# tencent-ailab/pika

Hardware: NVIDIA H100
Metric: utterances/sec RNN-T train step (T=1000,U=150,V=6k) (higher is better)
Workload: dtype bf16

## Files before the change

### include/pika_b200.h

```cpp
#ifndef PIKA_B200_H
#define PIKA_B200_H
#include <stdint.h>

#ifdef __cplusplus
extern "C" {
#endif

#define PK_F32 0
#define PK_BF16 1

const char* pk_last_error(void);
int pk_version(void);
long long pk_launch_count(void);

#define PK_GEMM_MAX_PAIRS 9
#define PK_SEL_ZERO 0
#define PK_SEL_ZB0 1
#define PK_SEL_ZB1 2
#define PK_SEL_KZ 3
#define PK_ACT_NONE 0
#define PK_ACT_RELU 1
#define PK_AUX_NONE 0
#define PK_AUX_ADD 1
#define PK_AUX_MASK_NZ 2

typedef struct {
    const void* ptr;
    int64_t dim[4];
    int64_t stride[3];
} pk_view4;

typedef struct {
    int n_pairs;
    pk_view4 a[PK_GEMM_MAX_PAIRS];
    pk_view4 b[PK_GEMM_MAX_PAIRS];
    int a_row_off[PK_GEMM_MAX_PAIRS];
    int b_row_off[PK_GEMM_MAX_PAIRS];
    int a_mn_major, b_mn_major;
    int a_sel2, a_sel3, b_sel2, b_sel3;
    int kz_count;
    pk_view4 c;
    int c_dtype;
    int c_accumulate;
    float alpha;
    const float* bias;
    int act;
    float drop_p;
    uint32_t drop_seed;
    int aux_mode;
    const void* aux;
    int aux_dtype;
    int64_t aux_stride[3];
    float aux_scale;
    int block_n;
    int k_splits;
    float* row_lse;
} pk_gemm_desc;

int pk_gemm_bf16(const pk_gemm_desc* desc, void* stream);
int pk_gemm_row_lse_parts(long long M, long long N, int block_n);

long long pk_rnnt_loss_workspace_bytes(int B, int T, int U1);
long long pk_rnnt_loss_colsum_workspace_bytes(int B, int T, int U1, int ldv);
int pk_rnnt_loss_fwd_bwd(const void* logits, int dtype, const int* labels, const int* frame_lens,
                         const int* label_lens, int B, int T, int U1, int V, int ldv, int ld_labels,
                         const float* grad_scale, float* costs, void* dlogits, float* dlogits_colsum, void* workspace,
                         long long workspace_bytes, void* stream);
int pk_rnnt_loss_fwd_bwd_lse(const void* logits, int dtype, const int* labels, const int* frame_lens,
                             const int* label_lens, int B, int T, int U1, int V, int ldv, int ld_labels,
                             const float* grad_scale, float* costs, void* dlogits, float* dlogits_colsum, void* workspace,
                             long long workspace_bytes, const float* row_lse, int n_parts, void* stream);

int pk_cast_split(const void* src, int src_dtype, long long ld_src, void* hi, void* lo, long long ld_dst,
                  long long rows, int cols, int cols_pad, float scale, void* stream);
int pk_attention_lse_stride(int T);
long long pk_attention_keep_bits_bytes(int B, int T, int heads);
int pk_attention_fwd(const void* q, const void* k, const void* v, long long ld_qkv, void* out, long long ld_out, float* lse,
                     int B, int T, int heads, int dh, float alpha, float drop_p, uint32_t seed, void* stream);
int pk_attention_bwd(const void* q, const void* k, const void* v, long long ld_qkv, const void* out, long long ld_out,
                     const void* dout, long long ld_dout, const float* lse, float* dsum_ws, void* dq, void* dk, void* dv,
                     long long ld_dqkv, int B, int T, int heads, int dh, float alpha, float drop_p, uint32_t seed, void* stream);
int pk_attention_fwd_bits(const void* q, const void* k, const void* v, long long ld_qkv, void* out, long long ld_out, float* lse,
                          int B, int T, int heads, int dh, float alpha, float drop_p, uint32_t seed, uint32_t* keep_bits, void* stream);
int pk_attention_bwd_bits(const void* q, const void* k, const void* v, long long ld_qkv, const void* out, long long ld_out,
                          const void* dout, long long ld_dout, const float* lse, float* dsum_ws, void* dq, void* dk, void* dv,
                          long long ld_dqkv, int B, int T, int heads, int dh, float alpha, float drop_p, const uint32_t* keep_bits,
                          void* stream);
long long pk_colstats_ws_floats(int C);
int pk_bn_fwd(const void* x, void* y, int dtype, long long rows, int C, const float* w, const float* b, float eps,
              int train, float momentum, float* run_mean, float* run_var, float* mean, float* rstd, float* stats_ws,
              void* stream);
int pk_bn_bwd(const void* dy, const void* x, void* dx, int dtype, long long rows, int C, const float* w,
              const float* mean, const float* rstd, int train, int relu_mask, float* dw, float* db, float* ws ,
              void* stream);
int pk_colsum(const void* x, int dtype, long long rows, int C, float* out, float* ws, void* stream);
int pk_layernorm_fwd(const void* x, void* y, int dtype, long long rows, int C, const float* w, const float* b, float eps,
                     float* mean, float* rstd, void* stream);
int pk_layernorm_bwd(const void* dy, const void* x, void* dx, int dtype, long long rows, int C, const float* w,
                     const float* mean, const float* rstd, float* dw, float* db, void* stream);
int pk_softmax_fwd(const float* S, long long ld_s, void* P, void* Pd, int dtype, long long ld_p, long long rows, int n,
                   float drop_p, uint32_t seed, void* stream);
int pk_softmax_masked_fwd(const float* S, long long ld_s, void* P, void* Pd, int dtype, long long ld_p, long long rows, int n,
                          int q_len, int heads, int causal, const uint8_t* key_pad, float drop_p, uint32_t seed, void* stream);
int pk_softmax_bwd(const float* dPd, long long ld_d, const void* P, long long ld_p, void* dS, int dtype, long long rows,
                   int n, float drop_p, uint32_t seed, void* stream);
#define PK_RELPOS_MAX 1024
int pk_softmax_masked_relpos_fwd(const float* S, long long ld_s, const float* QR, long long ld_r, void* P, void* Pd, int dtype,
                                 long long ld_p, long long rows, int n, int q_len, int heads, int causal, const uint8_t* key_pad,
                                 int max_rel, float* Pb, float drop_p, uint32_t seed, void* stream);
int pk_softmax_relpos_bwd(const float* dPd, long long ld_d, const float* G, long long ld_r, const void* P, long long ld_p, void* dS,
                          int dtype, long long rows, int n, int q_len, int heads, int max_rel, float* dSb, float drop_p,
                          uint32_t seed, void* stream);
int pk_dropout(const void* x, void* y, int dtype, long long n, float p, uint32_t seed, void* stream);
int pk_mask_nz(const void* dy, const void* y, void* dx, int dtype, long long n, float scale, void* stream);
int pk_add(const void* a, const void* b, void* o, int dtype, long long n, void* stream);
int pk_log_softmax(const void* x, int dtype, long long ld, float* y, long long rows, int n, float scale, void* stream);
int pk_joint_gate_fwd(const void* ex, const void* py, void* h, int dtype, int B, int T, int U1, int H, int ld_h, void* stream);
int pk_joint_gate_bwd(const void* ex, const void* py, const void* dh, void* dex, void* dpy, int dtype, int B, int T, int U1,
                      int H, void* stream);
int pk_lstm_cell_fwd(const float* gx, long long ld_gx, const float* gh, long long ld_gh, const float* c_prev, float* c_out,
                     void* h_out, int dtype, long long ld_h, float* gates_save, int B, int H, void* stream);
int pk_lstm_cell_bwd(const void* dh_out, long long ld_dho, const float* dh_rec, const float* dc_next, const float* gates,
                     const float* c, const float* c_prev, void* dgates, int dtype, float* dc_prev, int B, int H, void* stream);
int pk_embedding_fwd(const long long* idx, const float* table, int E, void* out, int dtype, int ld_out, long long n, void* stream);
int pk_embedding_bwd(const long long* idx, const void* dout, int dtype, int ld, int E, float* dtable, long long n,
                     long long padding_idx, void* stream);

int pk_absmax(const float* x, long long n, float* out, int* nan_flag, void* stream);
int pk_sgd_nesterov_clip(float* p, const float* g, float* buf, long long n, float lr, float momentum, float max_norm,
                         const float* absmax, const int* nan_flag, int first, void* stream);
int pk_bmuf_delta(const float* glob, const float* local, float* delta, long long n, void* stream);
int pk_bmuf_update(float* glob, float* local, float* delta_prev, const float* delta_sum, long long n, int world,
                   float block_momentum, float block_lr, void* stream);
int pk_adam_clip(float* p, const float* g, float* exp_avg, float* exp_avg_sq, float* p_out2, long long n, double lr,
                 double beta1, double beta2, double eps, double bias_correction1, double bias_correction2_sqrt,
                 float max_norm, const float* absmax, const int* nan_flag, void* stream);
int pk_bmuf_adam_update(float* glob, float* local, float* delta_prev, float* exp_avg_g, float* exp_avg_sq_g, float* msg,
                        long long n, int world, double block_momentum, double block_lr, double beta1_tau, double beta1_rho,
                        double beta2_tau, double beta2_rho, void* stream);

long long pk_frontend_workspace_bytes(int B, int n_max, int t_max, int n_mel, int D);
int pk_frontend_fwd(const short* pcm, long long ld_pcm, const int* n_samples, const float* rate, const int* new_len,
                    const float* target_db, const int* n_frames, int B, int n_max, int t_max, int n_mel, int lctx,
                    int rctx, const float* window, const float* twiddle, const float* mel_w, const int* mel_lo,
                    const int* mel_hi, float preemph, int cmn, const float* offset, const float* scale, int f0, int fs,
                    int t0, int ts, void* out, int out_dtype, short* wave_i16_out, void* workspace,
                    long long workspace_bytes, int* err_flag, float dither, unsigned int dither_seed, void* stream);
int pk_fbank(const float* wave, long long ld_wave, const int* n_frames, int B, int t_max, int n_mel, const float* window,
             const float* twiddle, const float* mel_w, const int* mel_lo, const int* mel_hi, float preemph, float* feats,
             float dither, unsigned int dither_seed, void* stream);

long long pk_frontend_noise_rir_workspace_bytes(int B, int n_max, int t_max, int n_mel, int D, int rir_max_len);
int pk_frontend_fwd_noise_rir(const short* pcm, long long ld_pcm, const int* n_samples, const float* rate, const int* new_len,
                              const float* target_db, const int* n_frames, int B, int n_max, int t_max, int n_mel, int lctx,
                              int rctx, const float* window, const float* twiddle, const float* mel_w, const int* mel_lo,
                              const int* mel_hi, float preemph, int cmn, const float* offset, const float* scale, int f0, int fs,
                              int t0, int ts, void* out, int out_dtype, short* wave_i16_out, void* workspace,
                              long long workspace_bytes, int* err_flag, float dither, unsigned int dither_seed, void* stream,
                              const short* noise, const int* noise_idx, const long long* noise_off, const double* snr,
                              const double* noise_rms_db, const short* rir, const long long* rir_off, const int* rir_len,
                              const int* rir_idx, int rir_max_len);

long long pk_conv_same_f64_workspace_bytes(int B, int n_max, int m_max);
int pk_conv_same_f64(const double* x, long long ld_x, const int* n_len, const double* h, long long ld_h, const int* m_len, int B,
                     int n_max, int m_max, double* y, long long ld_y, void* workspace, long long workspace_bytes, void* stream);

int pk_beam_prepare(const int* next_ys, const int* step_ctx, int* t_idx, const void* enc, int dtype, int Tenc, int H, void* enc_hid,
                    const float* embed, int E, void* x_emb, int ld_x, int K, int blk, int rows, void* stream);
int pk_beam_lstm_cell(const float* gates, const int* next_ys, const int* step_ctx, int blk, void* h, int dtype, float* c, int rows, int H,
                      void* stream);
int pk_beam_step_end(int* step_ctx, const int* not_done, int max_steps, void* stream);
int pk_beam_gate(const float* a, void* h, int dtype, int rows, int H, void* stream);
int pk_row_lse(const void* x, int dtype, long long ld, float* lse, long long rows, int n, float scale, void* stream);
int pk_beam_advance(const float* logits, int ldv, const float* row_lse, float sm_scale, const int* t_idx, const int* num_frames, const int* max_len, float* scores,
                    int* next_ys, int* prev_ks, int* hyp_tok, int* hyp_len, float* fin_score, int* fin_step, int* fin_k,
                    int* fin_count, int* eos_top, int* done, int* not_done_total, int B, int K, int V, int L, int cap,
                    const int* step_ctx, int blk, int n_best, int beam_prune, void* stream);
int pk_beam_reorder(const int* prev_ks, const int* step_ctx, const void* h_in, const float* c_in, const int* t_in, void* h_out, float* c_out,
                    int* t_out, int dtype, int K, int H, int layers, int rows, void* stream);
typedef struct {
    const int* arc_off;
    const int* arc_ilabel;
    const double* arc_weight;
    const int* arc_next;
    const double* finals;
    int backoff_id, n_disambig;
    int disambig_ids[4];
} pk_lm_fst;
int pk_beam_advance_lm(const float* logits, int ldv, const float* row_lse, float sm_scale, const int* t_idx, const int* num_frames, const int* max_len, float* scores,
                       int* next_ys, int* prev_ks, int* hyp_tok, int* hyp_len, float* fin_score, int* fin_step, int* fin_k,
                       int* fin_count, int* eos_top, int* done, int* not_done_total, int B, int K, int V, int L, int cap,
                       const int* step_ctx, int blk, int n_best, int beam_prune, const pk_lm_fst* fst, double lm_scale, double nonblk_reward,
                       int* set_state, double* set_cost, int* set_n, float* lm_scores, int max_states, int* err_flag, void* stream);

typedef struct {
    const int* next_ys;
    const int* step_ctx;
    const int* hyp_tok;
    const int* hyp_len;
    int* slot;
    void* pool;
    long long n_entries;
    int blk, rows, S1, layers, D, dtype, init;
} pk_beam_xf_state;
int pk_beam_xf_taps(const pk_beam_xf_state* st, int layer, const float* embed, int E, const void* x_cur, void* taps, int ldc, void* stream);
int pk_beam_xf_attn(const pk_beam_xf_state* st, int layer, const void* qkv, int heads, const float* rel, int max_rel, void* out, void* stream);
int pk_beam_xf_select(const pk_beam_xf_state* st, const void* x, void* h, int H, void* stream);
int pk_beam_xf_slots(const pk_beam_xf_state* st, const int* prev_ks, int K, void* stream);

long long pk_lstm_seq_workspace_bytes(int H);
int pk_lstm_seq_fwd_ex(const float* gx, const void* w_hh_bf16, void* out, int out_dtype, int ldo, float* gates_save, float* cs,
                       const int* lens, int B, int U, int H, int n_dir, int reverse, void* ws, void* stream);
int pk_lstm_seq_bwd_ex(const void* dout, int dtype, int ldo, const float* gates_save, const float* cs, const void* w_hh_bf16,
                       void* dG_bf16, const int* lens, int B, int U, int H, int n_dir, int reverse, void* ws, void* stream);

int pk_gather_rows(const void* src, const int* idx, void* dst, int dtype, long long rows, int C, void* stream);
int pk_scatter_add_rows(const void* src, const int* idx, float* dst, int dtype, long long rows, int C, void* stream);
int pk_ce_grad(const void* z, int dtype, long long ld, const int* tok, const float* coef, float scale, void* dz,
               long long rows, int n, void* stream);

#ifdef __cplusplus
}
#endif
#endif
```

### pika_b200/_lib.py

```python
import ctypes
import os
import re

_HERE = os.path.dirname(os.path.abspath(__file__))
LIB_PATH = os.path.join(_HERE, "libpika_b200.so")
HEADER_PATH = os.path.join(os.path.dirname(_HERE), "include", "pika_b200.h")


class PikaError(RuntimeError):
    pass


def _read_header(path):
    with open(path) as f:
        src = re.sub(r"/\*.*?\*/", " ", f.read(), flags=re.S)
    defines = {k: int(v) for k, v in re.findall(r"^\s*#define\s+(\w+)\s+(-?\d+)\s*$", src, flags=re.M)}
    src = re.sub(r"^\s*#.*$", " ", src, flags=re.M)
    src = re.sub(r"typedef\s+struct\s*\{.*?\}\s*\w+\s*;", " ", src, flags=re.S)
    src = re.sub(r'extern\s+"C"\s*\{|\}', " ", src)
    protos = []
    for decl in filter(None, (" ".join(d.split()) for d in src.split(";"))):
        m = re.fullmatch(r"(.+?)\s*\b(pk_\w+)\s*\((.*)\)", decl)
        if m is None:
            raise ImportError("pika_b200: %s: cannot read the declaration %r" % (path, decl))
        params = m.group(3).strip()
        protos.append((m.group(1), m.group(2), [] if params in ("", "void") else [p.strip() for p in params.split(",")]))
    return defines, protos


_DEFINES, _PROTOTYPES = _read_header(HEADER_PATH)
PK_F32, PK_BF16 = _DEFINES["PK_F32"], _DEFINES["PK_BF16"]
SEL_ZERO, SEL_ZB0, SEL_ZB1, SEL_KZ = (_DEFINES["PK_SEL_" + s] for s in ("ZERO", "ZB0", "ZB1", "KZ"))
ACT_NONE, ACT_RELU = _DEFINES["PK_ACT_NONE"], _DEFINES["PK_ACT_RELU"]
AUX_NONE, AUX_ADD, AUX_MASK_NZ = _DEFINES["PK_AUX_NONE"], _DEFINES["PK_AUX_ADD"], _DEFINES["PK_AUX_MASK_NZ"]
MAX_PAIRS = _DEFINES["PK_GEMM_MAX_PAIRS"]


class View4(ctypes.Structure):
    _fields_ = [("ptr", ctypes.c_void_p), ("dim", ctypes.c_int64 * 4), ("stride", ctypes.c_int64 * 3)]


class GemmDesc(ctypes.Structure):
    _fields_ = [
        ("n_pairs", ctypes.c_int),
        ("a", View4 * MAX_PAIRS),
        ("b", View4 * MAX_PAIRS),
        ("a_row_off", ctypes.c_int * MAX_PAIRS),
        ("b_row_off", ctypes.c_int * MAX_PAIRS),
        ("a_mn_major", ctypes.c_int), ("b_mn_major", ctypes.c_int),
        ("a_sel2", ctypes.c_int), ("a_sel3", ctypes.c_int), ("b_sel2", ctypes.c_int), ("b_sel3", ctypes.c_int),
        ("kz_count", ctypes.c_int),
        ("c", View4),
        ("c_dtype", ctypes.c_int),
        ("c_accumulate", ctypes.c_int),
        ("alpha", ctypes.c_float),
        ("bias", ctypes.c_void_p),
        ("act", ctypes.c_int),
        ("drop_p", ctypes.c_float),
        ("drop_seed", ctypes.c_uint32),
        ("aux_mode", ctypes.c_int),
        ("aux", ctypes.c_void_p),
        ("aux_dtype", ctypes.c_int),
        ("aux_stride", ctypes.c_int64 * 3),
        ("aux_scale", ctypes.c_float),
        ("block_n", ctypes.c_int),
        ("k_splits", ctypes.c_int),
        ("row_lse", ctypes.c_void_p),
    ]


class LmFst(ctypes.Structure):
    _fields_ = [("arc_off", ctypes.c_void_p), ("arc_ilabel", ctypes.c_void_p), ("arc_weight", ctypes.c_void_p),
                ("arc_next", ctypes.c_void_p), ("finals", ctypes.c_void_p), ("backoff_id", ctypes.c_int),
                ("n_disambig", ctypes.c_int), ("disambig_ids", ctypes.c_int * 4)]


class BeamXfState(ctypes.Structure):
    _fields_ = [("next_ys", ctypes.c_void_p), ("step_ctx", ctypes.c_void_p), ("hyp_tok", ctypes.c_void_p), ("hyp_len", ctypes.c_void_p),
                ("slot", ctypes.c_void_p), ("pool", ctypes.c_void_p), ("n_entries", ctypes.c_longlong), ("blk", ctypes.c_int),
                ("rows", ctypes.c_int), ("S1", ctypes.c_int), ("layers", ctypes.c_int), ("D", ctypes.c_int), ("dtype", ctypes.c_int),
                ("init", ctypes.c_int)]


STRUCTS = {"pk_view4": View4, "pk_gemm_desc": GemmDesc, "pk_lm_fst": LmFst, "pk_beam_xf_state": BeamXfState}
_SCALARS = {"int": ctypes.c_int, "long long": ctypes.c_longlong, "float": ctypes.c_float, "double": ctypes.c_double,
            "uint32_t": ctypes.c_uint32, "unsigned int": ctypes.c_uint32}
_RESULTS = {"int": ctypes.c_int, "long long": ctypes.c_longlong, "const char*": ctypes.c_char_p}


def _param_type(decl, fn):
    words = re.findall(r"\w+|\*", decl)[:-1]
    if "*" in words:
        base = " ".join(w for w in words if w not in ("const", "*"))
        if base in STRUCTS:
            return ctypes.POINTER(STRUCTS[base])
        if not base.startswith("pk_"):
            return ctypes.c_void_p
    elif " ".join(words) in _SCALARS:
        return _SCALARS[" ".join(words)]
    raise ImportError("pika_b200: %s: no ctypes type for the parameter %r of %s" % (HEADER_PATH, decl, fn))


class _CDLL(ctypes.CDLL):
    _func_flags_ = 0


def _bind(lib):
    for ret, name, params in _PROTOTYPES:
        if not hasattr(lib, name):
            raise ImportError("pika_b200: %s declares %s, which %s does not export" % (HEADER_PATH, name, LIB_PATH))
        ret = re.sub(r"\s*\*", "*", ret)
        if ret not in _RESULTS:
            raise ImportError("pika_b200: %s: no ctypes type for the return type %r of %s" % (HEADER_PATH, ret, name))
        fn = getattr(lib, name)
        fn.restype = _RESULTS[ret]
        fn.argtypes = [_param_type(p, name) for p in params]
    return lib


if not os.path.exists(LIB_PATH):
    raise ImportError(
        "pika_b200: %s is missing -- build it with `python -c 'import __graft_entry__ as g; g.build()'` "
        "(there is no CPU fallback)" % LIB_PATH)

lib = _bind(_CDLL(LIB_PATH))


def check(rc, what=""):
    if rc != 0:
        raise PikaError("%s failed (rc=%d): %s" % (what, rc, lib.pk_last_error().decode()))


def launch_count():
    return int(lib.pk_launch_count())
```

### pika_b200/csrc/elementwise.cu

```cuda
#include "../../include/pika_b200.h"
#include "common.cuh"

namespace pk {
void count_launch();

template <typename T> struct V8 {};
template <> struct V8<__nv_bfloat16> {
    struct Raw { uint4 q; };
    PK_DEVICE static Raw load_raw(const __nv_bfloat16* p) { return Raw{*reinterpret_cast<const uint4*>(p)}; }
    PK_DEVICE static void unpack(const Raw& r, float (&f)[8]) {
        f[0] = bf16lo(r.q.x); f[1] = bf16hi(r.q.x); f[2] = bf16lo(r.q.y); f[3] = bf16hi(r.q.y);
        f[4] = bf16lo(r.q.z); f[5] = bf16hi(r.q.z); f[6] = bf16lo(r.q.w); f[7] = bf16hi(r.q.w);
    }
    PK_DEVICE static void load(const __nv_bfloat16* p, float (&f)[8]) {
        const uint4 q = *reinterpret_cast<const uint4*>(p);
        f[0] = bf16lo(q.x); f[1] = bf16hi(q.x); f[2] = bf16lo(q.y); f[3] = bf16hi(q.y);
        f[4] = bf16lo(q.z); f[5] = bf16hi(q.z); f[6] = bf16lo(q.w); f[7] = bf16hi(q.w);
    }
    PK_DEVICE static void store(__nv_bfloat16* p, const float (&f)[8]) {
        *reinterpret_cast<uint4*>(p) =
            make_uint4(pack_bf16x2(f[0], f[1]), pack_bf16x2(f[2], f[3]), pack_bf16x2(f[4], f[5]), pack_bf16x2(f[6], f[7]));
    }
};
template <> struct V8<float> {
// ... 647 lines not shown
        V8<T>::load(x + i * 8, f);
#pragma unroll
        for (int e = 0; e < 8; ++e) f[e] = drop_keep((uint64_t)(i * 8 + e), seed, thresh) ? f[e] * scale : 0.f;
        V8<T>::store(y + i * 8, f);
    }
    for (long long i = nv * 8 + (long long)blockIdx.x * blockDim.x + threadIdx.x; i < n; i += (long long)gridDim.x * blockDim.x) {
        const float v = to_f32<T>(x[i]);
        y[i] = from_f32<T>(drop_keep((uint64_t)i, seed, thresh) ? v * scale : 0.f);
    }
}
template <typename T>
__global__ void __launch_bounds__(256) mask_nz_kernel(const T* __restrict__ dy, const T* __restrict__ y, T* __restrict__ dx, long long n, float scale) {
    const long long nv = n / 8;
    constexpr int UR = 2;
    for (long long i0 = ((long long)blockIdx.x * blockDim.x + threadIdx.x) * UR; i0 < nv; i0 += (long long)gridDim.x * blockDim.x * UR) {
        float g[UR][8], f[UR][8];
#pragma unroll
        for (int k = 0; k < UR; ++k)
            if (i0 + k < nv) { V8<T>::load(dy + (i0 + k) * 8, g[k]); V8<T>::load(y + (i0 + k) * 8, f[k]); }
#pragma unroll
        for (int k = 0; k < UR; ++k)
            if (i0 + k < nv) {
#pragma unroll
                for (int e = 0; e < 8; ++e) g[k][e] = f[k][e] != 0.f ? g[k][e] * scale : 0.f;
                V8<T>::store(dx + (i0 + k) * 8, g[k]);
            }
    }
    for (long long i = nv * 8 + (long long)blockIdx.x * blockDim.x + threadIdx.x; i < n; i += (long long)gridDim.x * blockDim.x)
        dx[i] = from_f32<T>(to_f32<T>(y[i]) != 0.f ? to_f32<T>(dy[i]) * scale : 0.f);
}
template <typename T>
__global__ void __launch_bounds__(256) add_kernel(const T* __restrict__ a, const T* __restrict__ b, T* __restrict__ o, long long n) {
    const long long nv = n / 8;
    for (long long i = (long long)blockIdx.x * blockDim.x + threadIdx.x; i < nv; i += (long long)gridDim.x * blockDim.x) {
        float f[8], g[8];
        V8<T>::load(a + i * 8, f);
        V8<T>::load(b + i * 8, g);
#pragma unroll
        for (int e = 0; e < 8; ++e) f[e] += g[e];
        V8<T>::store(o + i * 8, f);
    }
    for (long long i = nv * 8 + (long long)blockIdx.x * blockDim.x + threadIdx.x; i < n; i += (long long)gridDim.x * blockDim.x)
        o[i] = from_f32<T>(to_f32<T>(a[i]) + to_f32<T>(b[i]));
}
template <typename T>
__global__ void __launch_bounds__(256) log_softmax_kernel(const T* __restrict__ x, long long ld, float* __restrict__ y, long long rows,
                                                          int n, float scale, float* __restrict__ lse = nullptr) {
    const int lane = threadIdx.x & 31;
    const long long warp = (long long)blockIdx.x * (blockDim.x >> 5) + (threadIdx.x >> 5);
    const long long nw = (long long)gridDim.x * (blockDim.x >> 5);
    for (long long r = warp; r < rows; r += nw) {
        const T* xr = x + r * ld;
        float m = -INFINITY;
        for (int c = lane; c < n; c += 32) m = fmaxf(m, to_f32<T>(xr[c]) * scale);
        m = warp_max(m);
        float s = 0.f;
        for (int c = lane; c < n; c += 32) s += expf(to_f32<T>(xr[c]) * scale - m);
        const float l = m + logf(warp_sum(s));
        if (y) for (int c = lane; c < n; c += 32) y[r * n + c] = to_f32<T>(xr[c]) * scale - l;
        if (lse && lane == 0) lse[r] = l;
    }
}

PK_DEVICE float sigmoidf_(float x) { return 1.f / (1.f + __expf(-x)); }
template <typename T> PK_DEVICE float jt_tanh(float x);
template <> PK_DEVICE float jt_tanh<float>(float x) { return tanhf(x); }
template <> PK_DEVICE float jt_tanh<__nv_bfloat16>(float x) {
    float y;
    asm("tanh.approx.f32 %0, %1;" : "=f"(y) : "f"(x));
    return y;
}
template <typename T> PK_DEVICE float jt_sigmoid(float x);
template <> PK_DEVICE float jt_sigmoid<float>(float x) { return 1.f / (1.f + expf(-x)); }
template <> PK_DEVICE float jt_sigmoid<__nv_bfloat16>(float x) { return fmaf(jt_tanh<__nv_bfloat16>(0.5f * x), 0.5f, 0.5f); }

template <typename T>
__global__ void __launch_bounds__(128) joint_gate_fwd_kernel(const T* __restrict__ ex, const T* __restrict__ py, T* __restrict__ h,
                                                             int B, int Tt, int U1, int H, int ld_h) {
    const int bt = blockIdx.x;
    const int b = bt / Tt;
    for (int c0 = threadIdx.x * 8; c0 < H; c0 += blockDim.x * 8) {
        float e1[8], eg[8];
        V8<T>::load(ex + (long long)bt * 2 * H + c0, e1);
        V8<T>::load(ex + (long long)bt * 2 * H + H + c0, eg);
        for (int u = 0; u < U1; ++u) {
            float p1[8], pg[8], o[8];
            const T* pr = py + ((long long)b * U1 + u) * 2 * H;
            V8<T>::load(pr + c0, p1);
            V8<T>::load(pr + H + c0, pg);
#pragma unroll
            for (int e = 0; e < 8; ++e) o[e] = jt_tanh<T>(e1[e] + p1[e]) * jt_sigmoid<T>(eg[e] + pg[e]);
            V8<T>::store(h + ((long long)bt * U1 + u) * ld_h + c0, o);
        }
    }
    if (ld_h > H) {
        for (int u = threadIdx.x; u < U1; u += blockDim.x) {
            const float one[8] = {1.f, 0.f, 0.f, 0.f, 0.f, 0.f, 0.f, 0.f};
            V8<T>::store(h + ((long long)bt * U1 + u) * ld_h + H, one);
        }
    }
}
template <typename T, int UI>
__global__ void __launch_bounds__(128) joint_gate_fwd_sliced_kernel(const T* __restrict__ ex, const T* __restrict__ py, T* __restrict__ h,
                                                                    int B, int Tt, int U1, int H, int ld_h) {
    extern __shared__ __align__(16) uint8_t jg_smem[];
    T* s_py = reinterpret_cast<T*>(jg_smem);
    const int slices = H / 32;
    const int b = blockIdx.x / slices, cs = blockIdx.x - b * slices;
    const int tid = threadIdx.x, warp = tid >> 5, lane = tid & 31;
    const int ct = lane & 3, ul = (lane >> 2) + 8 * warp;
    const int c0 = cs * 32 + ct * 8;
    for (int i = tid; i < U1 * 8; i += 128) {
        const int u = i >> 3, v = i & 7;
        float f[8];
        V8<T>::load(py + ((long long)b * U1 + u) * 2 * H + (v >> 2) * H + cs * 32 + (v & 3) * 8, f);
        V8<T>::store(s_py + ((long long)(v * U1) + u) * 8, f);
    }
    __syncthreads();
    const T* s_p1 = s_py + (long long)(ct * U1) * 8;
    const T* s_pg = s_py + (long long)((4 + ct) * U1) * 8;
    const T* ex_b = ex + (long long)b * Tt * 2 * H + c0;
    typename V8<T>::Raw e1n = V8<T>::load_raw(ex_b), egn = V8<T>::load_raw(ex_b + H);
    for (int t = 0; t < Tt; ++t) {
        float e1[8], eg[8];
        V8<T>::unpack(e1n, e1);
        V8<T>::unpack(egn, eg);
        if (t + 1 < Tt) {
            e1n = V8<T>::load_raw(ex_b + (long long)(t + 1) * 2 * H);
            egn = V8<T>::load_raw(ex_b + (long long)(t + 1) * 2 * H + H);
        }
        T* hrow = h + ((long long)(b * Tt + t) * U1) * ld_h + c0;
#pragma unroll
        for (int i = 0; i < UI; ++i) {
            const int u = ul + 32 * i;
            if (u < U1) {
                float p1[8], pg[8], o[8];
                V8<T>::load(s_p1 + u * 8, p1);
                V8<T>::load(s_pg + u * 8, pg);
#pragma unroll
                for (int e = 0; e < 8; ++e) o[e] = jt_tanh<T>(e1[e] + p1[e]) * jt_sigmoid<T>(eg[e] + pg[e]);
                V8<T>::store(hrow + (long long)u * ld_h, o);
            }
        }
        if (ld_h > H && cs == 0 && ct == 0) {
            const float one[8] = {1.f, 0.f, 0.f, 0.f, 0.f, 0.f, 0.f, 0.f};
#pragma unroll
            for (int i = 0; i < UI; ++i) {
                const int u = ul + 32 * i;
                if (u < U1) V8<T>::store(h + ((long long)(b * Tt + t) * U1 + u) * ld_h + H, one);
            }
        }
    }
}
template <typename T>
__global__ void __launch_bounds__(128) joint_gate_bwd_ex_kernel(const T* __restrict__ ex, const T* __restrict__ py,
                                                                const T* __restrict__ dh, T* __restrict__ dex, int B, int Tt,
                                                                int U1, int H) {
    const int bt = blockIdx.x;
    const int b = bt / Tt;
    for (int c0 = threadIdx.x * 8; c0 < H; c0 += blockDim.x * 8) {
        float e1[8], eg[8], a1[8] = {0, 0, 0, 0, 0, 0, 0, 0}, ag[8] = {0, 0, 0, 0, 0, 0, 0, 0};
        V8<T>::load(ex + (long long)bt * 2 * H + c0, e1);
        V8<T>::load(ex + (long long)bt * 2 * H + H + c0, eg);
        for (int u = 0; u < U1; ++u) {
            float p1[8], pg[8], d[8];
            const T* pr = py + ((long long)b * U1 + u) * 2 * H;
            V8<T>::load(pr + c0, p1);
            V8<T>::load(pr + H + c0, pg);
            V8<T>::load(dh + ((long long)bt * U1 + u) * H + c0, d);
#pragma unroll
            for (int e = 0; e < 8; ++e) {
                const float a = jt_tanh<T>(e1[e] + p1[e]), g = jt_sigmoid<T>(eg[e] + pg[e]);
                a1[e] += d[e] * g * (1.f - a * a);
                ag[e] += d[e] * a * g * (1.f - g);
            }
        }
        V8<T>::store(dex + (long long)bt * 2 * H + c0, a1);
        V8<T>::store(dex + (long long)bt * 2 * H + H + c0, ag);
    }
}
template <typename T>
__global__ void __launch_bounds__(128) joint_gate_bwd_py_kernel(const T* __restrict__ ex, const T* __restrict__ py,
                                                                const T* __restrict__ dh, T* __restrict__ dpy, int B, int Tt,
                                                                int U1, int H) {
    const int bu = blockIdx.x;
    const int b = bu / U1, u = bu - b * U1;
    for (int c0 = threadIdx.x * 8; c0 < H; c0 += blockDim.x * 8) {
        float p1[8], pg[8], a1[8] = {0, 0, 0, 0, 0, 0, 0, 0}, ag[8] = {0, 0, 0, 0, 0, 0, 0, 0};
        V8<T>::load(py + (long long)bu * 2 * H + c0, p1);
        V8<T>::load(py + (long long)bu * 2 * H + H + c0, pg);
        for (int t = 0; t < Tt; ++t) {
            float e1[8], eg[8], d[8];
            const long long bt = (long long)b * Tt + t;
            V8<T>::load(ex + bt * 2 * H + c0, e1);
            V8<T>::load(ex + bt * 2 * H + H + c0, eg);
            V8<T>::load(dh + (bt * U1 + u) * H + c0, d);
#pragma unroll
            for (int e = 0; e < 8; ++e) {
                const float a = jt_tanh<T>(e1[e] + p1[e]), g = jt_sigmoid<T>(eg[e] + pg[e]);
                a1[e] += d[e] * g * (1.f - a * a);
                ag[e] += d[e] * a * g * (1.f - g);
            }
        }
        V8<T>::store(dpy + (long long)bu * 2 * H + c0, a1);
        V8<T>::store(dpy + (long long)bu * 2 * H + H + c0, ag);
    }
}

template <typename T, int UI>
__global__ void __launch_bounds__(128) joint_gate_bwd_fused_kernel(const T* __restrict__ ex, const T* __restrict__ py, const T* __restrict__ dh,
                                                                   T* __restrict__ dex, T* __restrict__ dpy, int B, int Tt, int U1, int H) {
    extern __shared__ __align__(16) uint8_t jg_smem[];
    T* s_py = reinterpret_cast<T*>(jg_smem);
    const int slices = H / 32;
    const int b = blockIdx.x / slices, cs = blockIdx.x - b * slices;
    const int tid = threadIdx.x, ct = tid >> 5, lane = tid & 31;
    const int c0 = cs * 32 + ct * 8;
    for (int i = tid; i < U1 * 8; i += 128) {
        const int u = i >> 3, v = i & 7;
        float f[8];
        V8<T>::load(py + ((long long)b * U1 + u) * 2 * H + (v >> 2) * H + cs * 32 + (v & 3) * 8, f);
        V8<T>::store(s_py + ((long long)(v * U1) + u) * 8, f);
    }
    float a1u[UI][8], agu[UI][8];
#pragma unroll
    for (int i = 0; i < UI; ++i)
#pragma unroll
        for (int e = 0; e < 8; ++e) { a1u[i][e] = 0.f; agu[i][e] = 0.f; }
    __syncthreads();
    const T* s_p1 = s_py + (long long)(ct * U1) * 8;
    const T* s_pg = s_py + (long long)((4 + ct) * U1) * 8;
    const T* dh_b = dh + (long long)b * Tt * U1 * H + c0;
    const T* ex_b = ex + (long long)b * Tt * 2 * H + c0;
    typename V8<T>::Raw dn[UI], e1n, egn;
#pragma unroll
    for (int i = 0; i < UI; ++i) {
        const int u = lane + 32 * i;
        if (u < U1) dn[i] = V8<T>::load_raw(dh_b + (long long)u * H);
    }
    e1n = V8<T>::load_raw(ex_b);
    egn = V8<T>::load_raw(ex_b + H);
    for (int t = 0; t < Tt; ++t) {
        float e1[8], eg[8];
        typename V8<T>::Raw dc[UI];
        V8<T>::unpack(e1n, e1);
        V8<T>::unpack(egn, eg);
#pragma unroll
        for (int i = 0; i < UI; ++i) dc[i] = dn[i];
        if (t + 1 < Tt) {
#pragma unroll
            for (int i = 0; i < UI; ++i) {
                const int u = lane + 32 * i;
                if (u < U1) dn[i] = V8<T>::load_raw(dh_b + ((long long)(t + 1) * U1 + u) * H);
            }
            e1n = V8<T>::load_raw(ex_b + (long long)(t + 1) * 2 * H);
            egn = V8<T>::load_raw(ex_b + (long long)(t + 1) * 2 * H + H);
        }
        float v[16];
#pragma unroll
        for (int e = 0; e < 16; ++e) v[e] = 0.f;
#pragma unroll
        for (int i = 0; i < UI; ++i) {
            const int u = lane + 32 * i;
            if (u < U1) {
                float p1[8], pg[8], d[8];
                V8<T>::unpack(dc[i], d);
                V8<T>::load(s_p1 + u * 8, p1);
                V8<T>::load(s_pg + u * 8, pg);
#pragma unroll
                for (int e = 0; e < 8; ++e) {
                    const float a = jt_tanh<T>(e1[e] + p1[e]), g = jt_sigmoid<T>(eg[e] + pg[e]);
                    const float dg = d[e] * g;
                    const float t1 = dg * (1.f - a * a), tg = dg * a * (1.f - g);
                    a1u[i][e] += t1; agu[i][e] += tg;
                    v[e] += t1; v[8 + e] += tg;
                }
            }
        }
        float w8[8], w4[4], w2[2];
        const bool h16 = lane & 16, h8 = lane & 8, h4 = lane & 4, h2 = lane & 2;
#pragma unroll
        for (int i = 0; i < 8; ++i) {
            const float keep = h16 ? v[i + 8] : v[i], send = h16 ? v[i] : v[i + 8];
            w8[i] = keep + __shfl_xor_sync(0xffffffffu, send, 16);
        }
#pragma unroll
        for (int i = 0; i < 4; ++i) {
            const float keep = h8 ? w8[i + 4] : w8[i], send = h8 ? w8[i] : w8[i + 4];
            w4[i] = keep + __shfl_xor_sync(0xffffffffu, send, 8);
        }
#pragma unroll
        for (int i = 0; i < 2; ++i) {
            const float keep = h4 ? w4[i + 2] : w4[i], send = h4 ? w4[i] : w4[i + 2];
            w2[i] = keep + __shfl_xor_sync(0xffffffffu, send, 4);
        }
        float w1 = (h2 ? w2[1] : w2[0]) + __shfl_xor_sync(0xffffffffu, h2 ? w2[0] : w2[1], 2);
        w1 += __shfl_xor_sync(0xffffffffu, w1, 1);
        if ((lane & 1) == 0) {
            const int j = lane >> 1;
            dex[((long long)b * Tt + t) * 2 * H + (j >> 3) * H + c0 + (j & 7)] = from_f32<T>(w1);
        }
    }
#pragma unroll
    for (int i = 0; i < UI; ++i) {
        const int u = lane + 32 * i;
        if (u < U1) {
            V8<T>::store(dpy + ((long long)b * U1 + u) * 2 * H + c0, a1u[i]);
            V8<T>::store(dpy + ((long long)b * U1 + u) * 2 * H + H + c0, agu[i]);
        }
    }
}

template <typename T>
__global__ void lstm_cell_fwd_kernel(const float* __restrict__ gx, long long ld_gx, const float* __restrict__ gh, long long ld_gh,
                                     const float* __restrict__ c_prev, float* __restrict__ c_out, T* __restrict__ h_out,
                                     long long ld_h, float* __restrict__ gates_save, int B, int H) {
    const int i = blockIdx.x * blockDim.x + threadIdx.x;
    if (i >= B * H) return;
    const int b = i / H, j = i - b * H;
    const float* a = gx + (long long)b * ld_gx;
    float gi = a[j], gf = a[H + j], gg = a[2 * H + j], go = a[3 * H + j];
    if (gh) {
        const float* r = gh + (long long)b * ld_gh;
        gi += r[j]; gf += r[H + j]; gg += r[2 * H + j]; go += r[3 * H + j];
    }
    gi = sigmoidf_(gi); gf = sigmoidf_(gf); gg = tanhf(gg); go = sigmoidf_(go);
    const float cp = c_prev ? c_prev[i] : 0.f;
    const float c = gf * cp + gi * gg;
    c_out[i] = c;
    h_out[(long long)b * ld_h + j] = from_f32<T>(go * tanhf(c));
    if (gates_save) {
        float* g = gates_save + (long long)b * 4 * H;
        g[j] = gi; g[H + j] = gf; g[2 * H + j] = gg; g[3 * H + j] = go;
    }
}
template <typename T>
__global__ void lstm_cell_bwd_kernel(const T* __restrict__ dh_out, long long ld_dho, const float* __restrict__ dh_rec,
                                     const float* __restrict__ dc_next, const float* __restrict__ gates, const float* __restrict__ c,
                                     const float* __restrict__ c_prev, T* __restrict__ dgates, float* __restrict__ dc_prev, int B,
                                     int H) {
    const int i = blockIdx.x * blockDim.x + threadIdx.x;
    if (i >= B * H) return;
    const int b = i / H, j = i - b * H;
    const float* g = gates + (long long)b * 4 * H;
    const float gi = g[j], gf = g[H + j], gg = g[2 * H + j], go = g[3 * H + j];
    float dh = dh_out ? to_f32<T>(dh_out[(long long)b * ld_dho + j]) : 0.f;
    if (dh_rec) dh += dh_rec[i];
    const float tc = tanhf(c[i]);
    float dc = dh * go * (1.f - tc * tc);
    if (dc_next) dc += dc_next[i];
    const float cp = c_prev ? c_prev[i] : 0.f;
    T* d = dgates + (long long)b * 4 * H;
    d[j] = from_f32<T>(dc * gg * gi * (1.f - gi));
    d[H + j] = from_f32<T>(dc * cp * gf * (1.f - gf));
    d[2 * H + j] = from_f32<T>(dc * gi * (1.f - gg * gg));
    d[3 * H + j] = from_f32<T>(dh * tc * go * (1.f - go));
    dc_prev[i] = dc * gf;
}

template <typename T>
__global__ void embedding_fwd_kernel(const long long* __restrict__ idx, const float* __restrict__ table, int E, T* __restrict__ out,
                                     int ld_out, long long n) {
    for (long long i = (long long)blockIdx.x * blockDim.x + threadIdx.x; i < n * ld_out; i += (long long)gridDim.x * blockDim.x) {
        const long long r = i / ld_out;
        const int c = (int)(i - r * ld_out);
        out[i] = from_f32<T>(c < E ? table[idx[r] * E + c] : 0.f);
    }
}
template <typename T>
__global__ void embedding_bwd_kernel(const long long* __restrict__ idx, const T* __restrict__ dout, int ld, int E,
                                     float* __restrict__ dtable, long long n, long long padding_idx) {
    for (long long i = (long long)blockIdx.x * blockDim.x + threadIdx.x; i < n * E; i += (long long)gridDim.x * blockDim.x) {
        const long long r = i / E;
        const int c = (int)(i - r * E);
        if (idx[r] != padding_idx) atomicAdd(&dtable[idx[r] * E + c], to_f32<T>(dout[r * ld + c]));
    }
}


template <typename T>
__global__ void gather_rows_kernel(const T* __restrict__ src, const int* __restrict__ idx, T* __restrict__ dst, long long rows, int C) {
    const long long r = blockIdx.x;
    if (r >= rows) return;
    const T* s = src + (long long)idx[r] * C;
    for (int c = threadIdx.x * 8; c < C; c += blockDim.x * 8) {
        float f[8];
        V8<T>::load(s + c, f);
        V8<T>::store(dst + r * C + c, f);
    }
}
template <typename T>
__global__ void scatter_add_rows_kernel(const T* __restrict__ src, const int* __restrict__ idx, float* __restrict__ dst, long long rows, int C) {
    const long long r = blockIdx.x;
    if (r >= rows) return;
    float* d = dst + (long long)idx[r] * C;
    for (int c = threadIdx.x; c < C; c += blockDim.x) atomicAdd(&d[c], to_f32<T>(src[r * C + c]));
}
template <typename T>
__global__ void __launch_bounds__(256) ce_grad_kernel(const T* __restrict__ z, long long ld, const int* __restrict__ tok,
                                                      const float* __restrict__ coef, float scale, T* __restrict__ dz, long long rows, int n) {
    const int lane = threadIdx.x & 31;
    const long long warp = (long long)blockIdx.x * (blockDim.x >> 5) + (threadIdx.x >> 5);
    const long long nw = (long long)gridDim.x * (blockDim.x >> 5);
    for (long long r = warp; r < rows; r += nw) {
        const T* zr = z + r * ld;
        T* dr = dz + r * ld;
// ... 86 lines not shown
                         const float* mean, const float* rstd, int train, int relu_mask, float* dw, float* db, float* ws,
                         void* stream) {
    PK_CHECK_ARG(C % 8 == 0 && rows > 0, "C must be a multiple of 8 and rows > 0");
    PK_CHECK_ARG(aligned16(dy) && aligned16(x) && aligned16(dx) && aligned16(ws), "pk_bn_bwd: dy, x, dx, ws must be 16-byte aligned");
    cudaStream_t st = STREAM(stream);
    PK_DISPATCH_T(dtype, { int rc = run_colstats<T, 1>((const T*)dy, (const T*)x, rows, C, mean, rstd, ws, db, dw, st); if (rc) return rc; });
    PK_DISPATCH_T(dtype, (bn_bwd_apply_kernel<T><<<col_grid(rows, C), 128, 0, st>>>((const T*)dy, (const T*)x, (T*)dx, rows, C, mean, rstd, w,
                                                                       train ? db : nullptr, train ? dw : nullptr, relu_mask)));
    DONE();
}

extern "C" int pk_colsum(const void* x, int dtype, long long rows, int C, float* out, float* ws, void* stream) {
    PK_CHECK_ARG(C % 8 == 0 && rows > 0, "C must be a multiple of 8 and rows > 0");
    PK_CHECK_ARG(aligned16(x) && aligned16(ws), "pk_colsum: x, ws must be 16-byte aligned");
    cudaStream_t st = STREAM(stream);
    PK_DISPATCH_T(dtype, { int rc = run_colstats<T, 0>((const T*)x, nullptr, rows, C, nullptr, nullptr, ws, out, nullptr, st); if (rc) return rc; });
    return 0;
}

extern "C" int pk_layernorm_fwd(const void* x, void* y, int dtype, long long rows, int C, const float* w, const float* b, float eps,
                                float* mean, float* rstd, void* stream) {
    PK_CHECK_ARG(C % 8 == 0 && rows > 0 && C <= 1024, "C must be a multiple of 8, <= 1024, and rows > 0");
    PK_CHECK_ARG(aligned16(x) && aligned16(y), "pk_layernorm_fwd: x, y must be 16-byte aligned");
    const int grid = grid_for(rows, 8);
    PK_DISPATCH_T(dtype, (ln_fwd_kernel<T><<<grid, 256, 0, STREAM(stream)>>>((const T*)x, (T*)y, rows, C, w, b, eps, mean, rstd)));
    DONE();
}
extern "C" int pk_layernorm_bwd(const void* dy, const void* x, void* dx, int dtype, long long rows, int C, const float* w,
                                const float* mean, const float* rstd, float* dw, float* db, void* stream) {
    PK_CHECK_ARG(C % 8 == 0 && rows > 0 && C <= 1024, "C must be a multiple of 8, <= 1024, and rows > 0");
    PK_CHECK_ARG(aligned16(dy) && aligned16(x) && aligned16(dx), "pk_layernorm_bwd: dy, x, dx must be 16-byte aligned");
    cudaStream_t st = STREAM(stream);
    PK_CHECK_CUDA(cudaMemsetAsync(dw, 0, sizeof(float) * C, st));
    PK_CHECK_CUDA(cudaMemsetAsync(db, 0, sizeof(float) * C, st));
    const int grid = grid_for(rows, 8, 2);
    PK_DISPATCH_T(dtype, (ln_bwd_kernel<T><<<grid, 256, 2 * C * sizeof(float), st>>>((const T*)dy, (const T*)x, (T*)dx, rows, C, w, mean,
                                                                                     rstd, dw, db)));
    DONE();
}

extern "C" int pk_softmax_fwd(const float* S, long long ld_s, void* P, void* Pd, int dtype, long long ld_p, long long rows, int n,
                              float drop_p, uint32_t seed, void* stream) {
    PK_CHECK_ARG(rows > 0 && n > 0 && ld_p >= n && ld_s >= ld_p && ld_p <= 2048 && ld_p % 8 == 0 && ld_s % 8 == 0, "softmax rows: ld % 8 == 0, <= 2048 wide");
    const int grid = grid_for(rows, 8);
    const uint32_t th = drop_thresh16_of(drop_p);
    const float sc = drop_scale16_of(th);
    if (ld_p <= 1024) { PK_DISPATCH_T(dtype, (softmax_fwd_kernel<T, 4><<<grid, 256, 0, STREAM(stream)>>>(S, ld_s, (T*)P, (T*)Pd, ld_p, rows, n, th, sc, seed))); }
    else { PK_DISPATCH_T(dtype, (softmax_fwd_kernel<T, 8><<<grid, 256, 0, STREAM(stream)>>>(S, ld_s, (T*)P, (T*)Pd, ld_p, rows, n, th, sc, seed))); }
    DONE();
}
extern "C" int pk_softmax_masked_fwd(const float* S, long long ld_s, void* P, void* Pd, int dtype, long long ld_p, long long rows, int n,
                                     int q_len, int heads, int causal, const uint8_t* key_pad, float drop_p, uint32_t seed, void* stream) {
    PK_CHECK_ARG(rows > 0 && n > 0 && ld_p >= n && ld_s >= ld_p && ld_p <= 2048 && ld_p % 8 == 0 && ld_s % 8 == 0, "softmax rows: ld % 8 == 0, <= 2048 wide");
    PK_CHECK_ARG(q_len > 0 && heads > 0 && rows % ((long long)heads * q_len) == 0, "masked softmax: rows = sequences * heads * q_len");
    PK_CHECK_ARG(causal || key_pad, "masked softmax without a mask: use pk_softmax_fwd");
    const int grid = grid_for(rows, 8);
    const uint32_t th = drop_thresh16_of(drop_p);
    const float sc = drop_scale16_of(th);
    if (ld_p <= 1024) { PK_DISPATCH_T(dtype, (softmax_fwd_kernel<T, 4><<<grid, 256, 0, STREAM(stream)>>>(S, ld_s, (T*)P, (T*)Pd, ld_p, rows, n, th, sc, seed, q_len, heads, causal, key_pad))); }
    else { PK_DISPATCH_T(dtype, (softmax_fwd_kernel<T, 8><<<grid, 256, 0, STREAM(stream)>>>(S, ld_s, (T*)P, (T*)Pd, ld_p, rows, n, th, sc, seed, q_len, heads, causal, key_pad))); }
    DONE();
}
extern "C" int pk_softmax_bwd(const float* dPd, long long ld_d, const void* P, long long ld_p, void* dS, int dtype, long long rows,
                              int n, float drop_p, uint32_t seed, void* stream) {
    PK_CHECK_ARG(rows > 0 && n > 0 && ld_p >= n && ld_d >= ld_p && ld_p <= 2048 && ld_p % 8 == 0 && ld_d % 8 == 0, "softmax rows: ld % 8 == 0, <= 2048 wide");
    const int grid = grid_for(rows, 8);
    const uint32_t th = drop_thresh16_of(drop_p);
    const float sc = drop_scale16_of(th);
    if (ld_p <= 1024) { PK_DISPATCH_T(dtype, (softmax_bwd_kernel<T, 4><<<grid, 256, 0, STREAM(stream)>>>(dPd, ld_d, (const T*)P, ld_p, (T*)dS, rows, n, th, sc, seed))); }
    else { PK_DISPATCH_T(dtype, (softmax_bwd_kernel<T, 8><<<grid, 256, 0, STREAM(stream)>>>(dPd, ld_d, (const T*)P, ld_p, (T*)dS, rows, n, th, sc, seed))); }
    DONE();
}
#define PK_RELPOS_CHECKS(ld_x, ld_p)                                                                                                  \
    PK_CHECK_ARG(rows > 0 && n > 0 && ld_p >= n && ld_x >= ld_p && ld_p <= 2048 && ld_p % 8 == 0 && ld_x % 8 == 0,                     \
                 "relative-position softmax rows: n <= ld_p <= 2048, pitches multiples of 8");                                         \
    PK_CHECK_ARG(q_len == n && heads > 0 && rows % ((long long)heads * q_len) == 0,                                                     \
                 "relative-position softmax: self-attention rows = sequences * heads * n");                                             \
    PK_CHECK_ARG(max_rel >= 1 && max_rel <= PK_RELPOS_MAX && ld_r >= 2 * max_rel + 1 && ld_r % 8 == 0,                               \
                 "relative positions: 1 <= max_rel <= 1024, ld_r >= 2*max_rel + 1 and a multiple of 8")
extern "C" int pk_softmax_masked_relpos_fwd(const float* S, long long ld_s, const float* QR, long long ld_r, void* P, void* Pd, int dtype,
                                            long long ld_p, long long rows, int n, int q_len, int heads, int causal, const uint8_t* key_pad,
                                            int max_rel, float* Pb, float drop_p, uint32_t seed, void* stream) {
    PK_RELPOS_CHECKS(ld_s, ld_p);
    const int grid = grid_for(rows, 8);
    const uint32_t th = drop_thresh16_of(drop_p);
    const float sc = drop_scale16_of(th);
    if (ld_p <= 1024) { PK_DISPATCH_T(dtype, (softmax_relpos_fwd_kernel<T, 4><<<grid, 256, 0, STREAM(stream)>>>(S, ld_s, QR, ld_r, (T*)P, (T*)Pd, ld_p, rows, n, th, sc, seed, q_len, heads, causal, key_pad, max_rel, Pb))); }
    else { PK_DISPATCH_T(dtype, (softmax_relpos_fwd_kernel<T, 8><<<grid, 256, 0, STREAM(stream)>>>(S, ld_s, QR, ld_r, (T*)P, (T*)Pd, ld_p, rows, n, th, sc, seed, q_len, heads, causal, key_pad, max_rel, Pb))); }
    DONE();
}
extern "C" int pk_softmax_relpos_bwd(const float* dPd, long long ld_d, const float* G, long long ld_r, const void* P, long long ld_p, void* dS,
                                     int dtype, long long rows, int n, int q_len, int heads, int max_rel, float* dSb, float drop_p,
                                     uint32_t seed, void* stream) {
    PK_RELPOS_CHECKS(ld_d, ld_p);
    const int grid = grid_for(rows, 8);
    const uint32_t th = drop_thresh16_of(drop_p);
    const float sc = drop_scale16_of(th);
    if (ld_p <= 1024) { PK_DISPATCH_T(dtype, (softmax_relpos_bwd_kernel<T, 4><<<grid, 256, 0, STREAM(stream)>>>(dPd, ld_d, G, ld_r, (const T*)P, ld_p, (T*)dS, rows, n, th, sc, seed, q_len, heads, max_rel, dSb))); }
    else { PK_DISPATCH_T(dtype, (softmax_relpos_bwd_kernel<T, 8><<<grid, 256, 0, STREAM(stream)>>>(dPd, ld_d, G, ld_r, (const T*)P, ld_p, (T*)dS, rows, n, th, sc, seed, q_len, heads, max_rel, dSb))); }
    DONE();
}
#undef PK_RELPOS_CHECKS

extern "C" int pk_dropout(const void* x, void* y, int dtype, long long n, float p, uint32_t seed, void* stream) {
    const int grid = grid_for(n, 256 * 8);
    const uint32_t th = drop_thresh_of(p);
    PK_CHECK_ARG(th != 0, "p must be > 0");
    PK_CHECK_ARG((reinterpret_cast<uintptr_t>(x) & 15) == 0 && (reinterpret_cast<uintptr_t>(y) & 15) == 0, "pk_dropout: pointers must be 16-byte aligned");
    PK_DISPATCH_T(dtype, (dropout_kernel<T><<<grid, 256, 0, STREAM(stream)>>>((const T*)x, (T*)y, n, th, 1.f / (1.f - p), seed)));
    DONE();
}
extern "C" int pk_mask_nz(const void* dy, const void* y, void* dx, int dtype, long long n, float scale, void* stream) {
    const int grid = grid_for(n, 256 * 16);
    PK_CHECK_ARG(((reinterpret_cast<uintptr_t>(dy) | reinterpret_cast<uintptr_t>(y) | reinterpret_cast<uintptr_t>(dx)) & 15) == 0, "pk_mask_nz: pointers must be 16-byte aligned");
    PK_DISPATCH_T(dtype, (mask_nz_kernel<T><<<grid, 256, 0, STREAM(stream)>>>((const T*)dy, (const T*)y, (T*)dx, n, scale)));
    DONE();
}
extern "C" int pk_add(const void* a, const void* b, void* o, int dtype, long long n, void* stream) {
    const int grid = grid_for(n, 256 * 8);
    PK_CHECK_ARG(((reinterpret_cast<uintptr_t>(a) | reinterpret_cast<uintptr_t>(b) | reinterpret_cast<uintptr_t>(o)) & 15) == 0, "pk_add: pointers must be 16-byte aligned");
    PK_DISPATCH_T(dtype, (add_kernel<T><<<grid, 256, 0, STREAM(stream)>>>((const T*)a, (const T*)b, (T*)o, n)));
    DONE();
}
extern "C" int pk_log_softmax(const void* x, int dtype, long long ld, float* y, long long rows, int n, float scale, void* stream) {
    const int grid = grid_for(rows, 8);
    PK_DISPATCH_T(dtype, (log_softmax_kernel<T><<<grid, 256, 0, STREAM(stream)>>>((const T*)x, ld, y, rows, n, scale)));
    DONE();
}
extern "C" int pk_row_lse(const void* x, int dtype, long long ld, float* lse, long long rows, int n, float scale, void* stream) {
    const int grid = grid_for(rows, 8);
    PK_DISPATCH_T(dtype, (log_softmax_kernel<T><<<grid, 256, 0, STREAM(stream)>>>((const T*)x, ld, nullptr, rows, n, scale, lse)));
    DONE();
}

template <typename T, int UI>
static void launch_gate_fwd_sliced(const void* ex, const void* py, void* h, int B, int T_, int U1, int H, int ld_h, cudaStream_t st) {
    joint_gate_fwd_sliced_kernel<T, UI><<<B * (H / 32), 128, U1 * 64 * (int)sizeof(T), st>>>((const T*)ex, (const T*)py, (T*)h, B, T_, U1, H, ld_h);
}
extern "C" int pk_joint_gate_fwd(const void* ex, const void* py, void* h, int dtype, int B, int T_, int U1, int H, int ld_h, void* stream) {
    PK_CHECK_ARG(H % 8 == 0 && ld_h % 8 == 0 && ld_h >= H, "H, ld_h must be multiples of 8");
    const int ui = (U1 + 31) / 32;
    if (H % 32 == 0 && ui <= 5 && T_ >= 8) {
        cudaStream_t st = STREAM(stream);
#define PK_GATE_CASE(N) case N: { PK_DISPATCH_T(dtype, (launch_gate_fwd_sliced<T, N>(ex, py, h, B, T_, U1, H, ld_h, st))); } break;
        switch (ui) { PK_GATE_CASE(1) PK_GATE_CASE(2) PK_GATE_CASE(3) PK_GATE_CASE(4) PK_GATE_CASE(5) }
#undef PK_GATE_CASE
        DONE();
    }
    PK_DISPATCH_T(dtype, (joint_gate_fwd_kernel<T><<<B * T_, 128, 0, STREAM(stream)>>>((const T*)ex, (const T*)py, (T*)h, B, T_, U1, H, ld_h)));
    DONE();
}

template <typename T, int UI>
static void launch_gate_bwd_fused(const void* ex, const void* py, const void* dh, void* dex, void* dpy, int B, int T_, int U1, int H, cudaStream_t st) {
    const int smem = U1 * 64 * (int)sizeof(T);
    joint_gate_bwd_fused_kernel<T, UI><<<B * (H / 32), 128, smem, st>>>((const T*)ex, (const T*)py, (const T*)dh, (T*)dex, (T*)dpy, B, T_, U1, H);
}
extern "C" int pk_joint_gate_bwd(const void* ex, const void* py, const void* dh, void* dex, void* dpy, int dtype, int B, int T_, int U1,
                                 int H, void* stream) {
    PK_CHECK_ARG(H % 8 == 0, "H must be a multiple of 8");
    const int ui = (U1 + 31) / 32;
    if (H % 32 == 0 && ui <= 5) {
        cudaStream_t st = STREAM(stream);
#define PK_GATE_CASE(N) case N: { PK_DISPATCH_T(dtype, (launch_gate_bwd_fused<T, N>(ex, py, dh, dex, dpy, B, T_, U1, H, st))); } break;
        switch (ui) { PK_GATE_CASE(1) PK_GATE_CASE(2) PK_GATE_CASE(3) PK_GATE_CASE(4) PK_GATE_CASE(5) }
#undef PK_GATE_CASE
        DONE();
    }
    PK_DISPATCH_T(dtype, (joint_gate_bwd_ex_kernel<T><<<B * T_, 128, 0, STREAM(stream)>>>((const T*)ex, (const T*)py, (const T*)dh, (T*)dex, B, T_, U1, H)));
    PK_CHECK_LAUNCH(); count_launch();
    PK_DISPATCH_T(dtype, (joint_gate_bwd_py_kernel<T><<<B * U1, 128, 0, STREAM(stream)>>>((const T*)ex, (const T*)py, (const T*)dh, (T*)dpy, B, T_, U1, H)));
    DONE();
}

extern "C" int pk_lstm_cell_fwd(const float* gx, long long ld_gx, const float* gh, long long ld_gh, const float* c_prev, float* c_out,
                                void* h_out, int dtype, long long ld_h, float* gates_save, int B, int H, void* stream) {
    PK_DISPATCH_T(dtype, (lstm_cell_fwd_kernel<T><<<(B * H + 255) / 256, 256, 0, STREAM(stream)>>>(gx, ld_gx, gh, ld_gh, c_prev, c_out,
                                                                                                (T*)h_out, ld_h, gates_save, B, H)));
    DONE();
}
extern "C" int pk_lstm_cell_bwd(const void* dh_out, long long ld_dho, const float* dh_rec, const float* dc_next, const float* gates,
                                const float* c, const float* c_prev, void* dgates, int dtype, float* dc_prev, int B, int H,
                                void* stream) {
    PK_DISPATCH_T(dtype, (lstm_cell_bwd_kernel<T><<<(B * H + 255) / 256, 256, 0, STREAM(stream)>>>((const T*)dh_out, ld_dho, dh_rec, dc_next,
                                                                                                gates, c, c_prev, (T*)dgates, dc_prev, B, H)));
    DONE();
}

extern "C" int pk_embedding_fwd(const long long* idx, const float* table, int E, void* out, int dtype, int ld_out, long long n,
                                void* stream) {
    const int grid = grid_for(n * ld_out, 256);
    PK_DISPATCH_T(dtype, (embedding_fwd_kernel<T><<<grid, 256, 0, STREAM(stream)>>>(idx, table, E, (T*)out, ld_out, n)));
    DONE();
}
extern "C" int pk_embedding_bwd(const long long* idx, const void* dout, int dtype, int ld, int E, float* dtable, long long n,
                                long long padding_idx, void* stream) {
    const int grid = grid_for(n * E, 256);
    PK_DISPATCH_T(dtype, (embedding_bwd_kernel<T><<<grid, 256, 0, STREAM(stream)>>>(idx, (const T*)dout, ld, E, dtable, n, padding_idx)));
    DONE();
}

extern "C" int pk_gather_rows(const void* src, const int* idx, void* dst, int dtype, long long rows, int C, void* stream) {
    PK_CHECK_ARG(C % 8 == 0 && rows > 0, "C must be a multiple of 8 and rows > 0");
    PK_CHECK_ARG(aligned16(src) && aligned16(dst), "pk_gather_rows: src, dst must be 16-byte aligned");
    PK_DISPATCH_T(dtype, (gather_rows_kernel<T><<<(unsigned)rows, 128, 0, STREAM(stream)>>>((const T*)src, idx, (T*)dst, rows, C)));
    DONE();
}
extern "C" int pk_scatter_add_rows(const void* src, const int* idx, float* dst, int dtype, long long rows, int C, void* stream) {
    PK_CHECK_ARG(rows > 0, "rows must be > 0");
    PK_DISPATCH_T(dtype, (scatter_add_rows_kernel<T><<<(unsigned)rows, 256, 0, STREAM(stream)>>>((const T*)src, idx, dst, rows, C)));
    DONE();
}
extern "C" int pk_ce_grad(const void* z, int dtype, long long ld, const int* tok, const float* coef, float scale, void* dz,
                          long long rows, int n, void* stream) {
    PK_CHECK_ARG(rows > 0 && n > 0 && ld >= n, "bad shape");
    const int grid = grid_for(rows, 8);
    PK_DISPATCH_T(dtype, (ce_grad_kernel<T><<<grid, 256, 0, STREAM(stream)>>>((const T*)z, ld, tok, coef, scale, (T*)dz, rows, n)));
    DONE();
}
```

### pika_b200/csrc/gemm.cu

```cuda
#include <cstdarg>
#include <cstdio>
#include <cstring>

#include "../../include/pika_b200.h"
#include "common.cuh"

namespace pk {

constexpr int BM = 128;
constexpr int BK = 64;
constexpr int A_STAGE_BYTES = BM * BK * 2;
constexpr int C_STAGE_BYTES = 64 * 128;
constexpr int CONSUMERS = 2;

struct GemmParams {
    CUtensorMap a[PK_GEMM_MAX_PAIRS];
    CUtensorMap b[PK_GEMM_MAX_PAIRS];
    CUtensorMap c;
    int a_off[PK_GEMM_MAX_PAIRS];
    int b_off[PK_GEMM_MAX_PAIRS];
    int n_pairs, kz_count, num_k_blocks;
    int k_splits, iters_per_split;
    int M, N, tiles_m, tiles_n, zb0, zb1;
    int a_sel2, a_sel3, b_sel2, b_sel3;
    int c_is_f32, c_accumulate;
    float alpha;
    const float* bias;
    int act;
    uint32_t drop_thresh;
    float drop_scale;
    uint32_t drop_seed;
    int aux_mode, aux_is_f32;
    const void* aux;
    long long aux_sm, aux_s0, aux_s1;
    float aux_scale;
    float* row_lse;
    uint64_t pol_a, pol_b, pol_c;
};

template <int BN, bool EPI_WARPS> struct GemmCfg {
    static constexpr int B_STAGE_BYTES = BN * BK * 2;
    static constexpr int STAGE_BYTES = A_STAGE_BYTES + B_STAGE_BYTES;
    static constexpr int STAGES = BN == 256 ? (EPI_WARPS ? 3 : 4) : (BN == 128 ? 6 : 8);
    static constexpr int C_OFF = STAGES * STAGE_BYTES;
    static constexpr int C_BYTES = EPI_WARPS ? BM * BN * 2 : CONSUMERS * 2 * C_STAGE_BYTES;
    static constexpr int BIAS_OFF = C_OFF + C_BYTES;
    static constexpr int BAR_OFF = BIAS_OFF + (EPI_WARPS ? BN * 4 : 0);
    static constexpr int SMEM_BYTES = BAR_OFF + 256 + 1024;
    static constexpr int THREADS = 128 + CONSUMERS * 128;
    static_assert(SMEM_BYTES <= 232448, "shared memory budget");
};

PK_DEVICE int pick_sel(int sel, int zb0, int zb1, int kz) {
    return sel == PK_SEL_ZB0 ? zb0 : (sel == PK_SEL_ZB1 ? zb1 : (sel == PK_SEL_KZ ? kz : 0));
}

struct UnitCoord { int mb, nb, zb0, zb1, split; };
PK_DEVICE UnitCoord decode_unit(const GemmParams& p, int unit) {
    UnitCoord u;
    const int tiles_per_z = p.tiles_m * p.tiles_n;
    const int out_tiles = tiles_per_z * p.zb0 * p.zb1;
    u.split = unit / out_tiles;
    const int tile = unit - u.split * out_tiles;
    const int z = tile / tiles_per_z;
    const int r = tile - z * tiles_per_z;
    u.mb = r / p.tiles_n; u.nb = r - u.mb * p.tiles_n;
    u.zb1 = z / p.zb0; u.zb0 = z - u.zb1 * p.zb0;
    return u;
}

template <int BN, bool A_MN, bool B_MN> PK_DEVICE void wgmma_tile(float (&acc)[BN / 2], uint64_t a, uint64_t b, uint32_t accumulate) {
    if constexpr (BN == 64) wgmma_ss_n64<A_MN, B_MN>(acc, a, b, accumulate);
    else if constexpr (BN == 128) wgmma_ss_n128<A_MN, B_MN>(acc, a, b, accumulate);
    else wgmma_ss_n256<A_MN, B_MN>(acc, a, b, accumulate);
}

enum { EPI_PLAIN = 0, EPI_LSE = 1, EPI_FULL = 2 };
template <bool CF32, int EPI> constexpr bool epi_warps() { return !CF32 && EPI != EPI_FULL; }

template <bool A_MN, bool B_MN, int BN, bool CF32, int EPI>
__global__ void __launch_bounds__(GemmCfg<BN, epi_warps<CF32, EPI>()>::THREADS, 1) gemm_wgmma_kernel(const __grid_constant__ GemmParams p) {
    constexpr bool EW = epi_warps<CF32, EPI>();
    static_assert(EPI != EPI_LSE || (EW && BN == 256), "the row log-sum-exp epilogue works on bf16 256-wide tiles");
    using Cfg = GemmCfg<BN, EW>;
    extern __shared__ uint8_t smem_raw[];
    uint8_t* smem = reinterpret_cast<uint8_t*>((reinterpret_cast<uintptr_t>(smem_raw) + 1023) & ~uintptr_t(1023));
    uint64_t* full_bar = reinterpret_cast<uint64_t*>(smem + Cfg::BAR_OFF);
    uint64_t* empty_bar = full_bar + Cfg::STAGES;
    uint64_t* c_full = empty_bar + Cfg::STAGES;
    uint64_t* c_empty = c_full + 1;
    const uint32_t ctile = smem_u32(smem + Cfg::C_OFF);
    const uint32_t sbias = smem_u32(smem + Cfg::BIAS_OFF);

    const int warp = threadIdx.x >> 5;
    const int lane = threadIdx.x & 31;
    const int worker = (int)blockIdx.x, n_workers = (int)gridDim.x;

    if (threadIdx.x == 0) {
        for (int i = 0; i < p.n_pairs; ++i) {
            tma_prefetch_desc(&p.a[i]);
            tma_prefetch_desc(&p.b[i]);
        }
        tma_prefetch_desc(&p.c);
        for (int s = 0; s < Cfg::STAGES; ++s) {
            mbar_init(&full_bar[s], 1);
            mbar_init(&empty_bar[s], CONSUMERS);
        }
        if (EW) {
            mbar_init(c_full, CONSUMERS * 4);
            mbar_init(c_empty, 3);
        }
        mbar_fence_init();
    }
    __syncthreads();

    const int out_tiles = p.tiles_m * p.tiles_n * p.zb0 * p.zb1;
    const int num_units = out_tiles * p.k_splits;
    const int k_iters_total = p.n_pairs * p.kz_count * p.num_k_blocks;

    if (warp < 4) {
        setmaxnreg_dec<40>();
    }
    if (warp == 0) {
        const uint32_t lead = elect_one_u32();
        int stage = 0;
        uint32_t phase = 0;
        const int kzb = p.kz_count * p.num_k_blocks;
        for (int unit = worker; unit < num_units; unit += n_workers) {
            const UnitCoord u = decode_unit(p, unit);
            const int m0 = u.mb * BM, n0 = u.nb * BN;
            const int i0 = u.split * p.iters_per_split, i1 = min(k_iters_total, i0 + p.iters_per_split);
            int pr = i0 / kzb;
            int rem = i0 - pr * kzb;
            int kz = rem / p.num_k_blocks, kb = rem - kz * p.num_k_blocks;
            int a2 = pick_sel(p.a_sel2, u.zb0, u.zb1, kz), a3 = pick_sel(p.a_sel3, u.zb0, u.zb1, kz);
            int b2 = pick_sel(p.b_sel2, u.zb0, u.zb1, kz), b3 = pick_sel(p.b_sel3, u.zb0, u.zb1, kz);
            const CUtensorMap* ma = &p.a[pr];
            const CUtensorMap* mbp = &p.b[pr];
            int a_off = p.a_off[pr], b_off = p.b_off[pr];
            for (int i = i0; i < i1; ++i) {
                mbar_wait(&empty_bar[stage], phase ^ 1);
                uint8_t* sa = smem + stage * Cfg::STAGE_BYTES;
                uint8_t* sb = sa + A_STAGE_BYTES;
                mbar_arrive_expect_tx_p(&full_bar[stage], Cfg::STAGE_BYTES, lead);
                const int k0 = kb * BK;
                if (A_MN) {
#pragma unroll
                    for (int c = 0; c < BM / 64; ++c)
                        tma_load_4d_hint_p(sa + c * (64 * BK * 2), ma, &full_bar[stage], m0 + c * 64, k0 + a_off, a2, a3, p.pol_a, lead);
                } else {
                    tma_load_4d_hint_p(sa, ma, &full_bar[stage], k0, m0 + a_off, a2, a3, p.pol_a, lead);
                }
                if (B_MN) {
#pragma unroll
                    for (int c = 0; c < BN / 64; ++c)
                        tma_load_4d_hint_p(sb + c * (64 * BK * 2), mbp, &full_bar[stage], n0 + c * 64, k0 + b_off, b2, b3, p.pol_b, lead);
                } else {
                    tma_load_4d_hint_p(sb, mbp, &full_bar[stage], k0, n0 + b_off, b2, b3, p.pol_b, lead);
                }
                if (++stage == Cfg::STAGES) { stage = 0; phase ^= 1; }
                if (++kb == p.num_k_blocks) {
                    kb = 0;
                    if (++kz == p.kz_count) {
                        kz = 0;
                        if (++pr < p.n_pairs) { ma = &p.a[pr]; mbp = &p.b[pr]; a_off = p.a_off[pr]; b_off = p.b_off[pr]; }
                    }
                    a2 = pick_sel(p.a_sel2, u.zb0, u.zb1, kz); a3 = pick_sel(p.a_sel3, u.zb0, u.zb1, kz);
                    b2 = pick_sel(p.b_sel2, u.zb0, u.zb1, kz); b3 = pick_sel(p.b_sel3, u.zb0, u.zb1, kz);
                }
            }
        }
    }
    if (EW && warp >= 1 && warp < 4) {
        const int et = threadIdx.x - 32;
        const uint32_t store_pred = (threadIdx.x == 32) ? 1u : 0u;
        uint32_t cph = 0;
        for (int unit = worker; unit < num_units; unit += n_workers, cph ^= 1) {
            const UnitCoord u = decode_unit(p, unit);
            const int m0 = u.mb * BM, n0 = u.nb * BN;
            for (int c = et; c < BN; c += 96) sts_f32(sbias + c * 4, (p.bias != nullptr && n0 + c < p.N) ? __ldg(p.bias + n0 + c) : 0.f);
            __syncwarp();
            if (lane == 0) mbar_arrive(c_empty);
            mbar_wait(c_full, cph);
#pragma unroll
            for (int ch = 0; ch < BN / 64; ++ch)
#pragma unroll
                for (int h = 0; h < 2; ++h)
                    if (n0 + ch * 64 < p.N && m0 + h * 64 < p.M)
                        tma_store_4d_hint_p(&p.c, smem + Cfg::C_OFF + ch * (BM * 128) + h * (64 * 128), n0 + ch * 64, m0 + h * 64, u.zb0, u.zb1,
                                            p.pol_c, store_pred);
            tma_store_commit_p(store_pred);
            tma_store_wait_read_p<0>(store_pred);
        }
        if (store_pred) tma_store_wait<0>();
    }
    if (warp >= 4) {
    setmaxnreg_inc<232>();
    const int wg = (threadIdx.x >> 7) - 1;
    const int et = threadIdx.x & 127;
    const int w4 = et >> 5;
    const uint32_t store_pred = (et == 0) ? 1u : 0u;
    const int bar_stage = 1 + wg;
    constexpr int GW = CF32 ? 4 : 8;
    constexpr int CH = 8 * GW;
    constexpr int ES = CF32 ? 4 : 2;
    uint8_t* cst = smem + Cfg::C_OFF + wg * 2 * C_STAGE_BYTES;
    const float relu_floor = (p.act == PK_ACT_RELU) ? 0.f : -INFINITY;
    const uint32_t base16 = (smem_u32(smem) >> 4) & 0x3FFF;
    const uint64_t a_desc0 = (A_MN ? make_smem_desc_sw128(0, 64 * BK * 2, 1024) : make_smem_desc_sw128(0, 16, 1024)) + base16 + ((wg * 8192) >> 4);
    const uint64_t b_desc0 = (B_MN ? make_smem_desc_sw128(0, 64 * BK * 2, 1024) : make_smem_desc_sw128(0, 16, 1024)) + base16 + (A_STAGE_BYTES >> 4);
    constexpr uint32_t A_K16 = (A_MN ? 2048 : 32) >> 4, B_K16 = (B_MN ? 2048 : 32) >> 4;
    const int r0 = w4 * 16 + (lane >> 2);
    const int cq = (lane & 3) * 2;

    float acc[BN / 2];
    int stage = 0;
    uint32_t phase = 0;
    uint32_t chunk_ctr = 0;
    uint32_t cph = 0;
    auto release = [&](int s) {
        if (et == 0) mbar_arrive(&empty_bar[s]);
    };
    constexpr float L2E = 1.4426950408889634f;
    constexpr int LSE_SLICES = BN / 16;
    bool lse_pending = false;
    float lse_m0 = 0.f, lse_m1 = 0.f, lse_s0 = 0.f, lse_s1 = 0.f;
    int lse_row = 0, lse_nb = 0, lse_nvalid = 0;
    const uint32_t lse_addr = ctile + (uint32_t)(wg * 64 + r0) * 128;
    auto lse_slice = [&](int t) {
        const int j = (t >> 1) & 3, g = (lane & 3) * 2 + (t & 1);
        if (j * 64 + g * 8 < lse_nvalid) {
            const bool hi = (t >> 3) != 0;
            const uint4 v = lds_u32x4(lse_addr + (hi ? 8 * 128 : 0) + j * (BM * 128) + ((g ^ (lane >> 2)) << 4));
            const float nm = hi ? -lse_m1 : -lse_m0;
            const uint32_t w[4] = {v.x, v.y, v.z, v.w};
            float s = 0.f;
#pragma unroll
            for (int q = 0; q < 4; ++q) s += ex2_approx(fmaf(bf16lo(w[q]), L2E, nm)) + ex2_approx(fmaf(bf16hi(w[q]), L2E, nm));
            if (hi) lse_s1 += s; else lse_s0 += s;
        }
    };
    auto lse_finish = [&]() {
        lse_s0 += __shfl_xor_sync(0xffffffffu, lse_s0, 1);
        lse_s1 += __shfl_xor_sync(0xffffffffu, lse_s1, 1);
        lse_s0 += __shfl_xor_sync(0xffffffffu, lse_s0, 2);
        lse_s1 += __shfl_xor_sync(0xffffffffu, lse_s1, 2);
        float* dst = p.row_lse + ((size_t)lse_nb * (size_t)p.M + (size_t)lse_row) * 2;
        if ((lane & 3) == 0 && lse_row < p.M) *reinterpret_cast<float2*>(dst) = make_float2(lse_m0, lse_m0 == -INFINITY ? 0.f : lse_s0);
        if ((lane & 3) == 0 && lse_row + 8 < p.M)
            *reinterpret_cast<float2*>(dst + 16) = make_float2(lse_m1, lse_m1 == -INFINITY ? 0.f : lse_s1);
        lse_pending = false;
    };
    for (int unit = worker; unit < num_units; unit += n_workers) {
        const UnitCoord u = decode_unit(p, unit);
        const int k_iters = min(k_iters_total, (u.split + 1) * p.iters_per_split) - u.split * p.iters_per_split;
        int prev = -1;
        for (int k = 0; k < k_iters; ++k) {
            mbar_wait(&full_bar[stage], phase);
            const uint32_t st16 = (uint32_t)(stage * Cfg::STAGE_BYTES) >> 4;
            wgmma_fence_acc(acc);
            wgmma_fence();
#pragma unroll
            for (int k4 = 0; k4 < BK / 16; ++k4)
                wgmma_tile<BN, A_MN, B_MN>(acc, a_desc0 + st16 + k4 * A_K16, b_desc0 + st16 + k4 * B_K16, (k > 0 || k4 > 0) ? 1u : 0u);
            wgmma_commit();
            wgmma_fence_acc(acc);
            wgmma_wait<1>();
            if (prev >= 0) release(prev);
            if constexpr (EPI == EPI_LSE) {
                if (lse_pending && k < LSE_SLICES) lse_slice(k);
            }
            prev = stage;
            if (++stage == Cfg::STAGES) { stage = 0; phase ^= 1; }
        }
        wgmma_wait<0>();
        wgmma_fence_acc(acc);
        if (prev >= 0) release(prev);

        if constexpr (EW) {
            if constexpr (EPI == EPI_LSE) {
                if (lse_pending) {
                    for (int t = k_iters; t < LSE_SLICES; ++t) lse_slice(t);
                    lse_finish();
                }
            }
            mbar_wait(c_empty, cph);
            if constexpr (EPI == EPI_LSE) __syncwarp();
            const int nvalid = p.N - u.nb * BN;
            uint32_t mx[2] = {0xFF80FF80u, 0xFF80FF80u};
            const int mi = lane >> 3;
            const uint32_t row_addr = ctile + (uint32_t)(wg * 64 + w4 * 16 + (lane & 7) + ((mi & 1) << 3)) * 128;
#pragma unroll
            for (int q = 0; q < BN / 16; ++q) {
                uint32_t r[4];
#pragma unroll
                for (int i = 0; i < 2; ++i) {
                    const int blk = 2 * q + i;
                    const float2 bs = lds_f32x2(sbias + (blk * 8 + cq) * 4);
#pragma unroll
                    for (int h = 0; h < 2; ++h)
                        r[2 * i + h] = pack_bf16x2(fmaxf(fmaf(acc[blk * 4 + 2 * h], p.alpha, bs.x), relu_floor),
                                                   fmaxf(fmaf(acc[blk * 4 + 2 * h + 1], p.alpha, bs.y), relu_floor));
                    if (EPI == EPI_LSE && blk * 8 < nvalid) { mx[0] = bf16x2_max(mx[0], r[2 * i]); mx[1] = bf16x2_max(mx[1], r[2 * i + 1]); }
                }
                const int blk = 2 * q + (mi >> 1);
                stmatrix_x4(row_addr + (blk >> 3) * (BM * 128) + (((blk & 7) ^ (lane & 7)) << 4), r[0], r[1], r[2], r[3]);
            }
            fence_proxy_async_smem();
            __syncwarp();
            if (lane == 0) mbar_arrive(c_full);
            cph ^= 1;
            if constexpr (EPI == EPI_LSE) {
                float x0 = fmaxf(bf16lo(mx[0]), bf16hi(mx[0])), x1 = fmaxf(bf16lo(mx[1]), bf16hi(mx[1]));
                x0 = fmaxf(x0, __shfl_xor_sync(0xffffffffu, x0, 1));
                x1 = fmaxf(x1, __shfl_xor_sync(0xffffffffu, x1, 1));
                x0 = fmaxf(x0, __shfl_xor_sync(0xffffffffu, x0, 2));
                x1 = fmaxf(x1, __shfl_xor_sync(0xffffffffu, x1, 2));
                lse_m0 = x0 * L2E; lse_m1 = x1 * L2E;
                lse_s0 = 0.f; lse_s1 = 0.f;
                lse_row = u.mb * BM + wg * 64 + r0;
                lse_nb = u.nb;
                lse_nvalid = nvalid;
                lse_pending = true;
            }
            continue;
        }

        const int zb0 = u.zb0, zb1 = u.zb1;
        const int m0 = u.mb * BM + wg * 64;
        const int n0 = u.nb * BN;
        if (m0 >= p.M) continue;
        const int mrow[2] = {m0 + r0, m0 + r0 + 8};
        const unsigned char* aux_row[2] = {nullptr, nullptr};
        uint64_t lin_row[2];
#pragma unroll
        for (int h = 0; h < 2; ++h) {
            if (EPI == EPI_FULL && p.aux_mode != PK_AUX_NONE && mrow[h] < p.M) {
                const long long off = (long long)mrow[h] * p.aux_sm + (long long)zb0 * p.aux_s0 + (long long)zb1 * p.aux_s1;
                aux_row[h] = reinterpret_cast<const unsigned char*>(p.aux) + off * (p.aux_is_f32 ? 4 : 2);
            }
            lin_row[h] = ((uint64_t)(zb1 * p.zb0 + zb0) * (uint64_t)p.M + (uint64_t)mrow[h]) * (uint64_t)p.N;
        }
        constexpr int n_chunks = BN / CH;
#pragma unroll
        for (int ch = 0; ch < n_chunks; ++ch) {
            const int nc0 = n0 + ch * CH;
            if (nc0 >= p.N) break;
            uint8_t* sbuf = cst + (chunk_ctr & 1) * C_STAGE_BYTES;
            tma_store_wait_read_p<1>(store_pred);
            named_bar_sync(bar_stage, 128);
#pragma unroll
            for (int nb = 0; nb < CH / 8; ++nb) {
                const int cl = nb * 8 + cq;
                const int ncol = nc0 + cl;
                float bs[2];
                if (p.bias != nullptr && ncol < p.N) { bs[0] = __ldg(p.bias + ncol); bs[1] = (ncol + 1 < p.N) ? __ldg(p.bias + ncol + 1) : 0.f; }
                else { bs[0] = 0.f; bs[1] = 0.f; }
#pragma unroll
                for (int h = 0; h < 2; ++h) {
                    const int ai = (ch * (CH / 8) + nb) * 4 + 2 * h;
                    float x[2];
#pragma unroll
                    for (int e = 0; e < 2; ++e) x[e] = fmaxf(fmaf(acc[ai + e], p.alpha, bs[e]), relu_floor);
                    if (EPI == EPI_FULL && p.drop_thresh != 0u) {
#pragma unroll
                        for (int e = 0; e < 2; ++e)
                            x[e] = drop_keep(lin_row[h] + (uint64_t)(ncol + e), p.drop_seed, p.drop_thresh) ? x[e] * p.drop_scale : 0.f;
                    }
                    if (EPI == EPI_FULL && aux_row[h] != nullptr && ncol < p.N) {
                        float a[2];
                        if (p.aux_is_f32) {
                            const float2 t2 = *reinterpret_cast<const float2*>(aux_row[h] + (size_t)ncol * 4);
                            a[0] = t2.x; a[1] = t2.y;
                        } else {
                            const uint32_t t1 = *reinterpret_cast<const uint32_t*>(aux_row[h] + (size_t)ncol * 2);
                            a[0] = bf16lo(t1); a[1] = bf16hi(t1);
                        }
                        if (p.aux_mode == PK_AUX_ADD) { x[0] += a[0]; x[1] += a[1]; }
                        else { x[0] = (a[0] != 0.f) ? x[0] * p.aux_scale : 0.f; x[1] = (a[1] != 0.f) ? x[1] * p.aux_scale : 0.f; }
                    }
                    const int row = r0 + 8 * h;
                    const int boff = cl * ES;
                    uint8_t* dst = sbuf + row * 128 + ((((boff >> 4) ^ (row & 7))) << 4) + (boff & 15);
                    if (CF32) {
                        *reinterpret_cast<float2*>(dst) = make_float2(x[0], x[1]);
                    } else {
                        *reinterpret_cast<uint32_t*>(dst) = pack_bf16x2(x[0], x[1]);
                    }
                }
            }
            fence_proxy_async_smem();
            named_bar_sync(bar_stage, 128);
            if (p.c_accumulate) tma_reduce_add_4d_p(&p.c, sbuf, nc0, m0, zb0, zb1, store_pred);
            else tma_store_4d_hint_p(&p.c, sbuf, nc0, m0, zb0, zb1, p.pol_c, store_pred);
            tma_store_commit_p(store_pred);
            ++chunk_ctr;
        }
    }
    if constexpr (EPI == EPI_LSE) {
        if (lse_pending) {
#pragma unroll
            for (int t = 0; t < LSE_SLICES; ++t) lse_slice(t);
            lse_finish();
        }
    }
    if (!EW && store_pred) tma_store_wait<0>();
    }
}
// ... 35 lines not shown
        }
        strides[i] = (cuuint64_t)sb;
    }
    if ((reinterpret_cast<uintptr_t>(v.ptr) & 15) != 0) { set_last_error("gemm %s: base pointer not 16B aligned", what); return -1; }
    if ((cuuint64_t)box[1] > 256) { set_last_error("gemm %s: box too large", what); return -1; }
    CUresult r = enc(out, is_f32 ? CU_TENSOR_MAP_DATA_TYPE_FLOAT32 : CU_TENSOR_MAP_DATA_TYPE_BFLOAT16, 4,
                     const_cast<void*>(v.ptr), dims, strides, box, estr, CU_TENSOR_MAP_INTERLEAVE_NONE,
                     CU_TENSOR_MAP_SWIZZLE_128B, CU_TENSOR_MAP_L2_PROMOTION_L2_256B, CU_TENSOR_MAP_FLOAT_OOB_FILL_NONE);
    if (r != CUDA_SUCCESS) { set_last_error("gemm %s: cuTensorMapEncodeTiled failed with CUresult %d", what, (int)r); return -3; }
    return 0;
}

void count_launch();

int encode_tiled_bf16_3d(CUtensorMap* out, const void* ptr, const unsigned long long (&dims)[3], const unsigned long long (&strides_bytes)[2],
                         const unsigned (&box)[3], const char* what) {
    EncodeTiledFn enc = get_encode_fn();
    if (!enc) { set_last_error("cuTensorMapEncodeTiled entry point not available"); return -3; }
    {
        static thread_local bool ctx_ready = false;
        if (!ctx_ready) { PK_CHECK_CUDA(cudaFree(nullptr)); ctx_ready = true; }
    }
    cuuint64_t d[3] = {dims[0], dims[1], dims[2]};
    cuuint64_t st[2] = {strides_bytes[0], strides_bytes[1]};
    cuuint32_t bx[3] = {box[0], box[1], box[2]};
    cuuint32_t es[3] = {1, 1, 1};
    if ((reinterpret_cast<uintptr_t>(ptr) & 15) != 0 || (st[0] % 16) != 0 || (st[1] % 16) != 0) {
        set_last_error("%s: base pointer / strides must be 16-byte aligned", what);
        return -1;
    }
    CUresult r = enc(out, CU_TENSOR_MAP_DATA_TYPE_BFLOAT16, 3, const_cast<void*>(ptr), d, st, bx, es, CU_TENSOR_MAP_INTERLEAVE_NONE,
                     CU_TENSOR_MAP_SWIZZLE_128B, CU_TENSOR_MAP_L2_PROMOTION_L2_256B, CU_TENSOR_MAP_FLOAT_OOB_FILL_NONE);
    if (r != CUDA_SUCCESS) { set_last_error("%s: cuTensorMapEncodeTiled failed with CUresult %d", what, (int)r); return -3; }
    return 0;
}

template <bool A_MN, bool B_MN, int BN, bool CF32, int EPI>
static int launch_gemm_e(const GemmParams& gp, int workers, cudaStream_t stream) {
    using Cfg = GemmCfg<BN, epi_warps<CF32, EPI>()>;
    auto kern = gemm_wgmma_kernel<A_MN, B_MN, BN, CF32, EPI>;
    static bool configured = false;
    if (!configured) {
        PK_CHECK_CUDA(cudaFuncSetAttribute(kern, cudaFuncAttributeMaxDynamicSharedMemorySize, Cfg::SMEM_BYTES));
        configured = true;
    }
    kern<<<workers, Cfg::THREADS, Cfg::SMEM_BYTES, stream>>>(gp);
    PK_CHECK_LAUNCH();
    count_launch();
    return 0;
}

template <bool A_MN, bool B_MN, int BN, bool CF32>
static int launch_gemm(const GemmParams& gp, int workers, cudaStream_t stream) {
    if (gp.row_lse != nullptr) {
        if constexpr (!A_MN && !B_MN && BN == 256 && !CF32) return launch_gemm_e<false, false, 256, false, EPI_LSE>(gp, workers, stream);
        set_last_error("gemm: row_lse needs K-major operands, a bf16 C and block_n = 256");
        return -1;
    }
    if (gp.drop_thresh != 0u || gp.aux_mode != PK_AUX_NONE) return launch_gemm_e<A_MN, B_MN, BN, CF32, EPI_FULL>(gp, workers, stream);
    return launch_gemm_e<A_MN, B_MN, BN, CF32, EPI_PLAIN>(gp, workers, stream);
}

template <int BN>
static int dispatch_major(const GemmParams& gp, int a_mn, int b_mn, int workers, cudaStream_t stream) {
    if (gp.c_is_f32) {
        if (!a_mn && !b_mn) return launch_gemm<false, false, BN, true>(gp, workers, stream);
        if (!a_mn && b_mn) return launch_gemm<false, true, BN, true>(gp, workers, stream);
        if (a_mn && !b_mn) return launch_gemm<true, false, BN, true>(gp, workers, stream);
        return launch_gemm<true, true, BN, true>(gp, workers, stream);
    }
    if (!a_mn && !b_mn) return launch_gemm<false, false, BN, false>(gp, workers, stream);
    if (!a_mn && b_mn) return launch_gemm<false, true, BN, false>(gp, workers, stream);
    if (a_mn && !b_mn) return launch_gemm<true, false, BN, false>(gp, workers, stream);
    return launch_gemm<true, true, BN, false>(gp, workers, stream);
}

static uint64_t policy_of(int code) { return code == 1 ? kL2EvictFirst : (code == 2 ? kL2EvictLast : kL2EvictNormal); }

static int plan_block_n(long long N, int block_n) { return block_n ? block_n : (N <= 64 ? 64 : (N <= 128 ? 128 : 256)); }

}

extern "C" int pk_gemm_row_lse_parts(long long M, long long N, int block_n) {
    (void)M;
    const int bn = pk::plan_block_n(N, block_n ? block_n : 256);
    return (int)((N + bn - 1) / bn);
}

extern "C" int pk_gemm_bf16(const pk_gemm_desc* d, void* stream_v) {
    using namespace pk;
    cudaStream_t stream = reinterpret_cast<cudaStream_t>(stream_v);
    PK_CHECK_ARG(d != nullptr, "null descriptor");
    PK_CHECK_ARG(d->n_pairs >= 1 && d->n_pairs <= PK_GEMM_MAX_PAIRS, "n_pairs out of range");
    PK_CHECK_ARG(d->kz_count >= 1, "kz_count must be >= 1");
    PK_CHECK_ARG(d->c_dtype == PK_F32 || d->c_dtype == PK_BF16, "bad c_dtype");
    PK_CHECK_ARG(!d->c_accumulate || d->c_dtype == PK_F32, "c_accumulate needs an f32 C");
    PK_CHECK_ARG(d->drop_p >= 0.f && d->drop_p < 1.f, "drop_p out of range");
    const long long N = d->c.dim[0], M = d->c.dim[1];
    PK_CHECK_ARG(M > 0 && N > 0, "empty C");
    PK_CHECK_ARG(d->aux == nullptr || d->aux_mode == PK_AUX_NONE || (N % 8 == 0), "aux epilogue needs N % 8 == 0");
    PK_CHECK_ARG(d->block_n == 0 || d->block_n == 64 || d->block_n == 128 || d->block_n == 256, "block_n must be 64, 128 or 256");
    const int bn = plan_block_n(N, d->row_lse ? (d->block_n ? d->block_n : 256) : d->block_n);

    {
        static thread_local bool ctx_ready = false;
        if (!ctx_ready) { PK_CHECK_CUDA(cudaFree(nullptr)); ctx_ready = true; }
    }
    static thread_local GemmParams gp;
    memset(&gp, 0, sizeof(gp));
    long long K = d->a_mn_major ? d->a[0].dim[1] : d->a[0].dim[0];
    for (int i = 0; i < d->n_pairs; ++i) {
        const long long ka = d->a_mn_major ? d->a[i].dim[1] : d->a[i].dim[0];
        const long long kb = d->b_mn_major ? d->b[i].dim[1] : d->b[i].dim[0];
        PK_CHECK_ARG(ka == K && kb == K, "all pairs must share the reduction extent K");
        int rc = make_map(&gp.a[i], d->a[i], 0, 64, d->a_mn_major ? 64 : BM, "A");
        if (rc) return rc;
        rc = make_map(&gp.b[i], d->b[i], 0, 64, d->b_mn_major ? 64 : bn, "B");
        if (rc) return rc;
        gp.a_off[i] = d->a_row_off[i];
        gp.b_off[i] = d->b_row_off[i];
    }
    {
        int rc = make_map(&gp.c, d->c, d->c_dtype == PK_F32, d->c_dtype == PK_F32 ? 32 : 64, 64, "C");
        if (rc) return rc;
    }
    gp.n_pairs = d->n_pairs;
    gp.kz_count = d->kz_count;
    gp.num_k_blocks = (int)((K + BK - 1) / BK);
    gp.M = (int)M;
    gp.N = (int)N;
    gp.tiles_m = (int)((M + BM - 1) / BM);
    gp.tiles_n = (int)((N + bn - 1) / bn);
    gp.zb0 = (int)d->c.dim[2];
    gp.zb1 = (int)d->c.dim[3];
    gp.a_sel2 = d->a_sel2; gp.a_sel3 = d->a_sel3; gp.b_sel2 = d->b_sel2; gp.b_sel3 = d->b_sel3;
    gp.c_is_f32 = d->c_dtype == PK_F32;
    gp.c_accumulate = d->c_accumulate;
    gp.alpha = d->alpha;
    gp.bias = d->bias;
    gp.act = d->act;
    if (d->drop_p > 0.f) {
        double t = (double)d->drop_p * 4294967296.0;
        gp.drop_thresh = t >= 4294967295.0 ? 4294967295u : (uint32_t)t;
        if (gp.drop_thresh == 0) gp.drop_thresh = 1;
        gp.drop_scale = 1.f / (1.f - d->drop_p);
    }
    gp.drop_seed = d->drop_seed;
    gp.aux_mode = d->aux ? d->aux_mode : PK_AUX_NONE;
    gp.aux_is_f32 = d->aux_dtype == PK_F32;
    gp.aux = d->aux;
    gp.aux_sm = d->aux_stride[0]; gp.aux_s0 = d->aux_stride[1]; gp.aux_s1 = d->aux_stride[2];
    gp.aux_scale = d->aux_scale;
    gp.row_lse = d->row_lse;
    PK_CHECK_ARG(d->row_lse == nullptr || (d->c_dtype == PK_BF16 && N % 8 == 0 && gp.zb0 == 1 && gp.zb1 == 1 && bn == 256 &&
                                           gp.drop_thresh == 0u && gp.aux_mode == PK_AUX_NONE),
                 "row_lse needs a 2-D bf16 C with N % 8 == 0, block_n = 256, no dropout / aux");
    {
        const long long K_ = (long long)gp.num_k_blocks * BK * gp.kz_count;
        const long long a_bytes = M * K_ * 2 * gp.n_pairs, b_bytes = N * K_ * 2 * gp.n_pairs;
        const long long c_bytes = M * N * (gp.c_is_f32 ? 4 : 2) * gp.zb0 * gp.zb1;
        const long long small = 32ll << 20, big = 256ll << 20;
        gp.pol_a = policy_of(a_bytes <= small && gp.zb0 * gp.zb1 == 1 ? 2 : 0);
        gp.pol_b = policy_of(b_bytes <= small && gp.zb0 * gp.zb1 == 1 ? 2 : 0);
        gp.pol_c = policy_of(c_bytes >= big ? 1 : 0);
    }

    const long long out_tiles = (long long)gp.tiles_m * gp.tiles_n * gp.zb0 * gp.zb1;
    const int workers_max = num_sms();
    const int k_iters_total = gp.n_pairs * gp.kz_count * gp.num_k_blocks;
    int splits = 1;
    const bool plain_epi = d->bias == nullptr && d->act == PK_ACT_NONE && d->drop_p == 0.f && gp.aux_mode == PK_AUX_NONE;
    if (d->k_splits > 0) splits = d->k_splits;
    else if (gp.c_is_f32 && plain_epi && gp.zb0 == 1 && gp.zb1 == 1 && k_iters_total >= 16 && out_tiles < 6 * workers_max) {
        const int w = workers_max;
        double best = 0.0;
        for (int sp = 1; sp <= 16 && sp <= k_iters_total / 8; ++sp) {
            const long long units = out_tiles * sp;
            const double eff = (double)units / (double)(((units + w - 1) / w) * w);
            if (eff > best + 0.02) { best = eff; splits = sp; }
        }
    }
    PK_CHECK_ARG(splits == 1 || (gp.c_is_f32 && plain_epi && gp.zb0 == 1 && gp.zb1 == 1), "split-K needs a plain f32 2-D C");
    gp.iters_per_split = (k_iters_total + splits - 1) / splits;
    gp.k_splits = (k_iters_total + gp.iters_per_split - 1) / gp.iters_per_split;
    if (gp.k_splits > 1) {
        if (!gp.c_accumulate)
            PK_CHECK_CUDA(cudaMemset2DAsync(const_cast<void*>(d->c.ptr), (size_t)d->c.stride[0] * 4, 0, (size_t)N * 4, (size_t)M, stream));
        gp.c_accumulate = 1;
    }
    const long long num_tiles = out_tiles * gp.k_splits;
    PK_CHECK_ARG(num_tiles < (1ll << 31), "too many tiles");
    int grid = workers_max;
    if (num_tiles < grid) grid = (int)num_tiles;
    if (bn == 64) return dispatch_major<64>(gp, d->a_mn_major, d->b_mn_major, grid, stream);
    if (bn == 128) return dispatch_major<128>(gp, d->a_mn_major, d->b_mn_major, grid, stream);
    return dispatch_major<256>(gp, d->a_mn_major, d->b_mn_major, grid, stream);
}
```

### pika_b200/csrc/rnnt_loss.cu

```cuda
#include <cstdlib>

#include "../../include/pika_b200.h"
#include "common.cuh"

namespace pk {
void count_launch();

constexpr float kLog2e = 1.4426950408889634f;
constexpr float kLn2 = 0.6931471805599453f;

template <typename T> struct Vec16;
template <> struct Vec16<__nv_bfloat16> {
    static constexpr int N = 8;
    PK_DEVICE static void unpack(const uint4& q, float (&f)[8]) {
        f[0] = bf16lo(q.x); f[1] = bf16hi(q.x); f[2] = bf16lo(q.y); f[3] = bf16hi(q.y);
        f[4] = bf16lo(q.z); f[5] = bf16hi(q.z); f[6] = bf16lo(q.w); f[7] = bf16hi(q.w);
    }
    PK_DEVICE static uint4 pack(const float (&f)[8]) {
        return make_uint4(pack_bf16x2(f[0], f[1]), pack_bf16x2(f[2], f[3]), pack_bf16x2(f[4], f[5]), pack_bf16x2(f[6], f[7]));
    }
    PK_DEVICE static float vmax(const uint4& q) {
        const __nv_bfloat162 a = __hmax2(*reinterpret_cast<const __nv_bfloat162*>(&q.x), *reinterpret_cast<const __nv_bfloat162*>(&q.y));
        const __nv_bfloat162 b = __hmax2(*reinterpret_cast<const __nv_bfloat162*>(&q.z), *reinterpret_cast<const __nv_bfloat162*>(&q.w));
        const __nv_bfloat162 c = __hmax2(a, b);
// ... 129 lines not shown
            lpl_skew[sk] = to_f32<T>(rp[y]) - lse;
        }
    }
}

typedef double lat_t;
#define LAT_NEG_INF (-(double)INFINITY)
PK_DEVICE lat_t lse2(lat_t a, lat_t b) {
    const lat_t mx = fmax(a, b), mn = fmin(a, b);
    if (mx == LAT_NEG_INF) return LAT_NEG_INF;
    return mx + log1p(exp(mn - mx));
}

constexpr int LAT_MAX_G = 512;
constexpr int LAT_MAX_CPT = 4;

__global__ void __launch_bounds__(2 * LAT_MAX_G) rnnt_lattice_kernel(
    const int* __restrict__ frame_lens, const int* __restrict__ label_lens, RnntDims d, int G, int cpt,
    const float* __restrict__ lpb_skew, const float* __restrict__ lpl_skew, lat_t* __restrict__ alpha_skew,
    lat_t* __restrict__ beta_skew, const float* __restrict__ grad_scale, float* __restrict__ costs,
    float* __restrict__ gb_out, float* __restrict__ gl_out) {
    extern __shared__ lat_t sm[];
    const int b = blockIdx.x;
    const int grp = threadIdx.x >= G ? 1 : 0;
    const int j = threadIdx.x - grp * G;
    const int T = frame_lens[b], U = label_lens[b];
    const int W = d.U1 + 2;
    lat_t* buf0 = sm + grp * 2 * W + 1;
    lat_t* buf1 = buf0 + W;
    __shared__ lat_t s_ll;
    const size_t base = (size_t)b * d.ND * d.U1;
    const bool valid = (T > 0 && T <= d.T && U >= 0 && U < d.U1);
    if (valid) {
        for (int i = j - 1; i <= d.U1; i += G) { buf0[i] = LAT_NEG_INF; buf1[i] = LAT_NEG_INF; }
        named_bar_sync(1 + grp, G);
        const int last = T - 1 + U;
        if (grp == 0) {
            lat_t* prev = buf0;
            lat_t* cur = buf1;
            if (j == 0) { cur[0] = 0.0; alpha_skew[base] = 0.0; }
            float nb[LAT_MAX_CPT], nl[LAT_MAX_CPT];
#pragma unroll
            for (int c = 0; c < LAT_MAX_CPT; ++c) {
                const int u = j + c * G;
                nb[c] = (c < cpt && u <= U && last >= 1) ? lpb_skew[base + u] : 0.f;
                nl[c] = (c < cpt && u >= 1 && u <= U && last >= 1) ? lpl_skew[base + u - 1] : 0.f;
            }
            named_bar_sync(1, G);
            for (int dg = 1; dg <= last; ++dg) {
                lat_t* tsw = prev; prev = cur; cur = tsw;
                const int lo = max(0, dg - (T - 1)), hi = min(U, dg);
                float pb[LAT_MAX_CPT], pl[LAT_MAX_CPT];
#pragma unroll
                for (int c = 0; c < LAT_MAX_CPT; ++c) { pb[c] = nb[c]; pl[c] = nl[c]; }
                if (dg < last) {
                    const size_t nbase = base + (size_t)dg * d.U1;
#pragma unroll
                    for (int c = 0; c < LAT_MAX_CPT; ++c) {
                        const int u = j + c * G;
                        if (c < cpt && u <= U) {
                            nb[c] = lpb_skew[nbase + u];
                            nl[c] = (u >= 1) ? lpl_skew[nbase + u - 1] : 0.f;
                        }
                    }
                }
#pragma unroll
                for (int c = 0; c < LAT_MAX_CPT; ++c) {
                    const int u = j + c * G;
                    if (c < cpt && u >= lo && u <= hi) {
                        lat_t a = LAT_NEG_INF, cc = LAT_NEG_INF;
                        if (u <= dg - 1) a = prev[u] + pb[c];
                        if (u >= 1) cc = prev[u - 1] + pl[c];
                        const lat_t v = lse2(a, cc);
                        cur[u] = v;
                        alpha_skew[base + (size_t)dg * d.U1 + u] = v;
                    }
                }
                named_bar_sync(1, G);
            }
        } else {
            lat_t* prev = buf0;
            lat_t* cur = buf1;
            if (j == 0) {
                const lat_t v = lpb_skew[base + (size_t)last * d.U1 + U];
                cur[U] = v;
                beta_skew[base + (size_t)last * d.U1 + U] = v;
            }
            float nb[LAT_MAX_CPT], nl[LAT_MAX_CPT];
#pragma unroll
            for (int c = 0; c < LAT_MAX_CPT; ++c) {
                const int u = j + c * G;
                const bool ok = c < cpt && u <= U && last >= 1;
                nb[c] = ok ? lpb_skew[base + (size_t)(last - 1) * d.U1 + u] : 0.f;
                nl[c] = ok ? lpl_skew[base + (size_t)(last - 1) * d.U1 + u] : 0.f;
            }
            named_bar_sync(2, G);
            for (int dg = last - 1; dg >= 0; --dg) {
                lat_t* tsw = prev; prev = cur; cur = tsw;
                const int lo = max(0, dg - (T - 1)), hi = min(U, dg);
                float pb[LAT_MAX_CPT], pl[LAT_MAX_CPT];
#pragma unroll
                for (int c = 0; c < LAT_MAX_CPT; ++c) { pb[c] = nb[c]; pl[c] = nl[c]; }
                if (dg > 0) {
                    const size_t nbase = base + (size_t)(dg - 1) * d.U1;
#pragma unroll
                    for (int c = 0; c < LAT_MAX_CPT; ++c) {
                        const int u = j + c * G;
                        if (c < cpt && u <= U) { nb[c] = lpb_skew[nbase + u]; nl[c] = lpl_skew[nbase + u]; }
                    }
                }
#pragma unroll
                for (int c = 0; c < LAT_MAX_CPT; ++c) {
                    const int u = j + c * G;
                    if (c < cpt && u >= lo && u <= hi) {
                        const int t = dg - u;
                        lat_t a = LAT_NEG_INF, cc = LAT_NEG_INF;
                        if (t + 1 <= T - 1) a = prev[u] + pb[c];
                        if (u + 1 <= U) cc = prev[u + 1] + pl[c];
                        const lat_t v = lse2(a, cc);
                        cur[u] = v;
                        beta_skew[base + (size_t)dg * d.U1 + u] = v;
                    }
                }
                named_bar_sync(2, G);
            }
            if (j == 0) { s_ll = cur[0]; costs[b] = (float)(-cur[0]); }
        }
    } else if (threadIdx.x == 0) {
        costs[b] = 0.f;
    }
    __syncthreads();
    const float gs = grad_scale ? grad_scale[b] : 1.f;
    const lat_t ll = valid ? s_ll : 0.0;
    const int nodes = d.T * d.U1;
    for (int i = threadIdx.x; i < nodes; i += blockDim.x) {
        const int t = i / d.U1, u = i - t * d.U1;
        float gb = 0.f, gl = 0.f;
        if (valid && t < T && u <= U) {
            const size_t sk = skew_index(d, b, t, u);
            const lat_t a = alpha_skew[sk];
            lat_t bn;
            if (t < T - 1) bn = beta_skew[skew_index(d, b, t + 1, u)];
            else bn = (u == U) ? 0.0 : LAT_NEG_INF;
            gb = (float)(-exp(a + bn + (lat_t)lpb_skew[sk] - ll)) * gs;
            if (u < U) gl = (float)(-exp(a + beta_skew[skew_index(d, b, t, u + 1)] + (lat_t)lpl_skew[sk] - ll)) * gs;
            if (!(gb == gb)) gb = 0.f;
            if (!(gl == gl)) gl = 0.f;
        }
        gb_out[(size_t)b * nodes + i] = gb;
        gl_out[(size_t)b * nodes + i] = gl;
    }
}

constexpr int GRAD_THREADS = 256;
template <typename T> struct GradCfg { static constexpr int MAXG = 32 / Vec16<T>::N; };
template <typename T, int GRAD_RU, int MINB>
__global__ void __launch_bounds__(GRAD_THREADS, MINB) rnnt_grad_kernel(const T* logits, const int* __restrict__ labels,
                                                                    const int* __restrict__ label_lens, RnntDims d,
                                                                    const float* __restrict__ lse_in, const float* __restrict__ gb_in,
                                                                    const float* __restrict__ gl_in, T* dlogits, float* __restrict__ colsum,
                                                                    long long rows_per_cta) {
    constexpr int VN = Vec16<T>::N;
    constexpr int GRAD_MAXG = GradCfg<T>::MAXG;
    extern __shared__ float gsm[];
    float* s_gb = gsm;
    float* s_gl = gsm + rows_per_cta;
    float* s_l2 = gsm + 2 * rows_per_cta;
    int* s_y = reinterpret_cast<int*>(gsm + 3 * rows_per_cta);
    const long long rows = (long long)d.B * d.T * d.U1;
    const long long r0 = (long long)blockIdx.x * rows_per_cta;
    const long long r1 = min(rows, r0 + rows_per_cta);
    const int nvec_ld = d.ldv / VN;
    const int tid = threadIdx.x;
    for (long long row = r0 + tid; row < r1; row += GRAD_THREADS) {
        const int i = (int)(row - r0);
        s_gb[i] = gb_in[row];
        s_gl[i] = gl_in[row];
        s_l2[i] = lse_in[row] * kLog2e;
        const int u = (int)(row % d.U1);
        const int b = (int)(row / ((long long)d.T * d.U1));
        s_y[i] = (u < label_lens[b]) ? labels[(size_t)b * d.ld_labels + u] : -1;
    }
    __syncthreads();
    float cs[GRAD_MAXG][VN];
#pragma unroll
    for (int gq = 0; gq < GRAD_MAXG; ++gq)
#pragma unroll
        for (int e = 0; e < VN; ++e) cs[gq][e] = 0.f;
    for (long long rb = r0; rb < r1; rb += GRAD_RU) {
        uint4 q[GRAD_RU][GRAD_MAXG];
#pragma unroll
        for (int k = 0; k < GRAD_RU; ++k) {
            const long long row = rb + k;
            if (row < r1 && (s_gb[row - r0] != 0.f || s_gl[row - r0] != 0.f)) {
                const uint4* vp = reinterpret_cast<const uint4*>(logits + row * (long long)d.ldv);
#pragma unroll
                for (int gq = 0; gq < GRAD_MAXG; ++gq) {
                    const int i = tid + gq * GRAD_THREADS;
                    if (i < nvec_ld) q[k][gq] = ld_plain(vp + i);
                }
            }
        }
#pragma unroll
        for (int k = 0; k < GRAD_RU; ++k) {
            const long long row = rb + k;
            if (row >= r1) continue;
            const float gb = s_gb[row - r0], gl = s_gl[row - r0];
            uint4* op = reinterpret_cast<uint4*>(dlogits + row * (long long)d.ldv);
            if (gb == 0.f && gl == 0.f) {
#pragma unroll
                for (int gq = 0; gq < GRAD_MAXG; ++gq) {
                    const int i = tid + gq * GRAD_THREADS;
                    if (i < nvec_ld) st_stream(op + i, make_uint4(0, 0, 0, 0));
                }
                continue;
            }
            const int y = s_y[row - r0];
            const float l2 = s_l2[row - r0];
            const float gsum = -(gb + gl);
#pragma unroll
            for (int gq = 0; gq < GRAD_MAXG; ++gq) {
                const int i = tid + gq * GRAD_THREADS;
                if (i < nvec_ld) {
                    float f[VN];
                    Vec16<T>::unpack(q[k][gq], f);
#pragma unroll
                    for (int e = 0; e < VN; ++e) f[e] = ex2_approx(fmaf(f[e], kLog2e, -l2)) * gsum;
                    const int v0 = i * VN;
                    if (v0 == 0) f[0] += gb;
                    if (y >= v0 && y < v0 + VN) {
#pragma unroll
                        for (int e = 0; e < VN; ++e) if (v0 + e == y) f[e] += gl;
                    }
                    if (v0 + VN > d.V) {
#pragma unroll
                        for (int e = 0; e < VN; ++e) if (v0 + e >= d.V) f[e] = 0.f;
                    }
                    const uint4 packed = Vec16<T>::pack(f);
                    st_stream(op + i, packed);
                    if (colsum) {
                        float w[VN];
                        Vec16<T>::unpack(packed, w);
#pragma unroll
                        for (int e = 0; e < VN; ++e) cs[gq][e] += w[e];
                    }
                }
            }
        }
    }
    if (colsum) {
        float* part = colsum + (size_t)blockIdx.x * d.ldv;
#pragma unroll
        for (int gq = 0; gq < GRAD_MAXG; ++gq) {
            const int i = tid + gq * GRAD_THREADS;
            if (i < nvec_ld) {
#pragma unroll
                for (int e = 0; e < VN; ++e) part[i * VN + e] = cs[gq][e];
            }
        }
    }
}

__global__ void __launch_bounds__(256) colsum_partials_kernel(const float* __restrict__ part, int n_part, int ld, float* __restrict__ out) {
    __shared__ float sm[8][33];
    const int tx = threadIdx.x & 31, ty = threadIdx.x >> 5;
    const int c = blockIdx.x * 32 + tx;
    float a = 0.f;
    if (c < ld) {
        const int per = (n_part + 7) / 8;
        const int i0 = ty * per, i1 = min(n_part, i0 + per);
        float a0 = 0.f, a1 = 0.f, a2 = 0.f, a3 = 0.f;
        int i = i0;
        for (; i + 4 <= i1; i += 4) {
            a0 += part[(size_t)(i + 0) * ld + c]; a1 += part[(size_t)(i + 1) * ld + c];
            a2 += part[(size_t)(i + 2) * ld + c]; a3 += part[(size_t)(i + 3) * ld + c];
        }
        for (; i < i1; ++i) a0 += part[(size_t)i * ld + c];
        a = (a0 + a1) + (a2 + a3);
    }
    sm[ty][tx] = a;
    __syncthreads();
    if (ty == 0 && c < ld) {
        float t = sm[0][tx];
#pragma unroll
        for (int k = 1; k < 8; ++k) t += sm[k][tx];
        out[c] = t;
    }
}

}

extern "C" long long pk_rnnt_loss_workspace_bytes(int B, int T, int U1) {
    const long long nd = (long long)T + U1 - 1;
    const long long skew = (long long)B * nd * U1;
    const long long nodes = (long long)B * T * U1;
    return (2 * skew + 3 * nodes) * 4 + 2 * skew * 8 + 256;
}
static void rnnt_grad_grid(long long rows, long long* rpc_out, int* ggrid_out) {
    const int ru = 2;
    const int gcta = pk::num_sms() * 3 * 4;
    long long rpc = (rows + gcta - 1) / gcta;
    rpc = (rpc + ru - 1) / ru * ru;
    if (rpc > 2048) rpc = 2048;
    *rpc_out = rpc; *ggrid_out = (int)((rows + rpc - 1) / rpc);
}
extern "C" long long pk_rnnt_loss_colsum_workspace_bytes(int B, int T, int U1, int ldv) {
    int ggrid; long long rpc;
    rnnt_grad_grid((long long)B * T * U1, &rpc, &ggrid);
    return (long long)ggrid * ldv * 4;
}

static int rnnt_loss_impl(const void* logits, int dtype, const int* labels, const int* frame_lens,
                          const int* label_lens, int B, int T, int U1, int V, int ldv, int ld_labels,
                          const float* grad_scale, float* costs, void* dlogits, float* dlogits_colsum, void* workspace,
                          long long workspace_bytes, const float* row_lse, int n_parts, void* stream_v) {
    using namespace pk;
    cudaStream_t stream = reinterpret_cast<cudaStream_t>(stream_v);
    PK_CHECK_ARG(dtype == PK_F32 || dtype == PK_BF16, "bad dtype");
    PK_CHECK_ARG(B > 0 && T > 0 && U1 > 0 && V > 1, "bad dims");
    const int vn = dtype == PK_F32 ? 4 : 8;
    PK_CHECK_ARG(ldv >= V && ldv % vn == 0, "ldv must be >= V and a multiple of 16 bytes");
    PK_CHECK_ARG((reinterpret_cast<uintptr_t>(logits) & 15) == 0, "logits not 16B aligned");
    PK_CHECK_ARG(dlogits == nullptr || (reinterpret_cast<uintptr_t>(dlogits) & 15) == 0, "dlogits not 16B aligned");
    PK_CHECK_ARG(workspace_bytes >= pk_rnnt_loss_workspace_bytes(B, T, U1), "workspace too small");
    RnntDims d{B, T, U1, V, ldv, ld_labels, T + U1 - 1};
    const size_t skew = (size_t)B * d.ND * U1, nodes = (size_t)B * T * U1;
    double* wsd = reinterpret_cast<double*>(workspace);
    double* alpha = wsd; double* beta = alpha + skew;
    float* lpb = reinterpret_cast<float*>(beta + skew); float* lpl = lpb + skew;
    float* lse = lpl + skew; float* gb = lse + nodes; float* gl = gb + nodes;

    const long long rows = (long long)nodes;
    const int warps_per_cta = 8;
    long long want = (rows + warps_per_cta - 1) / warps_per_cta;
    const long long cap = (long long)num_sms() * 8 * 4;
    const int grid = (int)(want < cap ? want : cap);
    if (row_lse != nullptr) {
        PK_CHECK_ARG(n_parts >= 1, "n_parts must be >= 1");
        const int fgrid = (int)((rows + 255) / 256 < (long long)num_sms() * 8 ? (rows + 255) / 256 : (long long)num_sms() * 8);
        if (dtype == PK_BF16)
            rnnt_rowfinish_kernel<__nv_bfloat16><<<fgrid, 256, 0, stream>>>(reinterpret_cast<const __nv_bfloat16*>(logits), labels, frame_lens,
                                                                           label_lens, d, reinterpret_cast<const float2*>(row_lse), n_parts,
                                                                           lse, lpb, lpl);
        else
            rnnt_rowfinish_kernel<float><<<fgrid, 256, 0, stream>>>(reinterpret_cast<const float*>(logits), labels, frame_lens, label_lens, d,
                                                                   reinterpret_cast<const float2*>(row_lse), n_parts, lse, lpb, lpl);
    } else if (dtype == PK_BF16)
        rnnt_rowstats_kernel<__nv_bfloat16><<<grid, 256, 0, stream>>>(reinterpret_cast<const __nv_bfloat16*>(logits), labels,
                                                                     frame_lens, label_lens, d, lse, lpb, lpl);
    else
        rnnt_rowstats_kernel<float><<<grid, 256, 0, stream>>>(reinterpret_cast<const float*>(logits), labels, frame_lens,
                                                              label_lens, d, lse, lpb, lpl);
    PK_CHECK_LAUNCH(); count_launch();
    const int lat_smem = 2 * 2 * (U1 + 2) * 8;
    int G = ((U1 + 31) / 32) * 32;
    if (G > LAT_MAX_G) G = LAT_MAX_G;
    const int cpt = (U1 + G - 1) / G;
    PK_CHECK_ARG(cpt <= LAT_MAX_CPT, "U too large for the lattice kernel (U+1 <= 2048)");
    static bool configured = false;
    if (!configured) {
        PK_CHECK_CUDA(cudaFuncSetAttribute(rnnt_lattice_kernel, cudaFuncAttributeMaxDynamicSharedMemorySize,
                                           2 * 2 * (LAT_MAX_G * LAT_MAX_CPT + 2) * (int)sizeof(lat_t)));
        configured = true;
    }
    rnnt_lattice_kernel<<<B, 2 * G, lat_smem, stream>>>(frame_lens, label_lens, d, G, cpt, lpb, lpl, alpha, beta, grad_scale,
                                                     costs, gb, gl);
    PK_CHECK_LAUNCH(); count_launch();
    if (dlogits != nullptr) {
        PK_CHECK_ARG(ldv <= 8192, "V too large for the gradient kernel (V <= 8192)");
        int ggrid; long long rpc;
        rnnt_grad_grid(rows, &rpc, &ggrid);
        float* cs_part = nullptr;
        if (dlogits_colsum) {
            const long long base_bytes = pk_rnnt_loss_workspace_bytes(B, T, U1);
            PK_CHECK_ARG(workspace_bytes >= base_bytes + (long long)ggrid * ldv * 4,
                         "workspace too small for the column sums (add pk_rnnt_loss_colsum_workspace_bytes)");
            cs_part = reinterpret_cast<float*>(reinterpret_cast<unsigned char*>(workspace) + base_bytes);
        }
        const size_t gsmem = (size_t)rpc * 16;
#define PK_GRAD_LAUNCH(TT, RU, MB)                                                                                         \
        rnnt_grad_kernel<TT, RU, MB><<<ggrid, GRAD_THREADS, gsmem, stream>>>(reinterpret_cast<const TT*>(logits), labels, label_lens, d, lse, \
                                                                            gb, gl, reinterpret_cast<TT*>(dlogits), cs_part, rpc)
        if (dtype == PK_BF16) PK_GRAD_LAUNCH(__nv_bfloat16, 2, 3);
        else PK_GRAD_LAUNCH(float, 2, 2);
#undef PK_GRAD_LAUNCH
        PK_CHECK_LAUNCH(); count_launch();
        if (dlogits_colsum) {
            colsum_partials_kernel<<<(ldv + 31) / 32, 256, 0, stream>>>(cs_part, ggrid, ldv, dlogits_colsum);
            PK_CHECK_LAUNCH(); count_launch();
        }
    }
    return 0;
}

extern "C" int pk_rnnt_loss_fwd_bwd(const void* logits, int dtype, const int* labels, const int* frame_lens,
                                    const int* label_lens, int B, int T, int U1, int V, int ldv, int ld_labels,
                                    const float* grad_scale, float* costs, void* dlogits, float* dlogits_colsum, void* workspace,
                                    long long workspace_bytes, void* stream) {
    return rnnt_loss_impl(logits, dtype, labels, frame_lens, label_lens, B, T, U1, V, ldv, ld_labels, grad_scale, costs, dlogits,
                          dlogits_colsum, workspace, workspace_bytes, nullptr, 0, stream);
}

extern "C" int pk_rnnt_loss_fwd_bwd_lse(const void* logits, int dtype, const int* labels, const int* frame_lens,
                                        const int* label_lens, int B, int T, int U1, int V, int ldv, int ld_labels,
                                        const float* grad_scale, float* costs, void* dlogits, float* dlogits_colsum, void* workspace,
                                        long long workspace_bytes, const float* row_lse, int n_parts, void* stream) {
    PK_CHECK_ARG(row_lse != nullptr, "row_lse is null");
    return rnnt_loss_impl(logits, dtype, labels, frame_lens, label_lens, B, T, U1, V, ldv, ld_labels, grad_scale, costs, dlogits,
                          dlogits_colsum, workspace, workspace_bytes, row_lse, n_parts, stream);
}
```

### pika_b200/engine.py

```python
import math
import weakref

import torch

from . import kernels as K

_PRECISION = "bf16"
_WEIGHT_EPOCH = 0
_SEED = [0x5EED]
_DROPOUT_ENABLED = True


def set_precision(p):
    global _PRECISION
    assert p in ("bf16", "fp32")
    _PRECISION = p


def get_precision():
    return _PRECISION


def act_dtype():
    return torch.bfloat16 if _PRECISION == "bf16" else torch.float32
# ... 489 lines not shown
    other = (L - 1 - r) if rev else r.expand(U, B)
    live = r < L
    src = b * U + torch.where(live, other, torch.zeros_like(other))
    dsrc = torch.where(live, b * U + other, torch.full_like(other, B * U))
    to_time = torch.where(live, other * B + b, torch.full_like(other, U * B))
    return src, dsrc, to_time


class LstmLayerFn(torch.autograd.Function):

    @staticmethod
    def forward(ctx, x, lens, *params):
        B, U, E = x.shape
        n_dir = len(params) // 4
        dirs = [params[4 * d:4 * d + 4] for d in range(n_dir)]
        H = dirs[0][1].shape[1]
        G4 = 4 * H
        wih_parts = [stage_weight(p[0], cols_pad=E if E != p[0].shape[1] else None) for p in dirs]
        whh_parts = stage_weight([p[1] for p in dirs])
        x_parts = stage_act(x)
        gx = torch.empty(n_dir, B, U, G4, dtype=torch.float32, device=x.device)
        for d, (w_ih, w_hh, b_ih, b_hh) in enumerate(dirs):
            bsum = torch.empty(G4, dtype=torch.float32, device=x.device)
            K.add(b_ih.detach(), b_hh.detach(), bsum)
            gemm_parts([[p.view(B * U, E) for p in x_parts]], [wih_parts[d]], gx[d].view(B * U, G4), bias=bsum)
        out = _new((B, U, n_dir * H), like=x)
        gates = torch.empty(n_dir, U, B, G4, dtype=torch.float32, device=x.device)
        cs = torch.empty(n_dir, U, B, H, dtype=torch.float32, device=x.device)
        ctx.persistent = (x.dtype == torch.bfloat16 and H % 64 == 0 and
                          n_dir * H // 8 <= torch.cuda.get_device_properties(x.device).multi_processor_count)
        if ctx.persistent:
            K.lstm_seq_fwd_ex(gx, whh_parts[0], out, gates, cs, lens)
        else:
            for d in range(n_dir):
                whh = [p[d * G4:(d + 1) * G4] for p in whh_parts]
                out_d = out[:, :, d * H:(d + 1) * H]
                if lens is None and d == 0:
                    gx_s, h_s = (lambda t: gx[d][:, t, :]), (lambda t: out_d[:, t, :])
                else:
                    src, _, _ = _lstm_step_maps(lens if lens is not None else _full_lens(B, U, x.device), B, U, d == 1)
                    gxs = torch.empty(U * B, G4, dtype=torch.float32, device=x.device)
                    K.gather_rows(gx[d].view(B * U, G4), src.view(-1), gxs)
                    hs = _new((U * B + 1, H), like=x, zero=True)
                    gx_s, h_s = (lambda t: gxs[t * B:(t + 1) * B]), (lambda t: hs[t * B:(t + 1) * B])
                gh = torch.empty(B, G4, dtype=torch.float32, device=x.device)
                for t in range(U):
                    if t > 0:
                        gemm_parts([stage_act_view(h_s(t - 1))], [whh], gh, block_n=64)
                    K.lstm_cell_fwd(gx_s(t), gh if t > 0 else None, cs[d][t - 1] if t > 0 else None, cs[d][t], h_s(t), gates[d][t], B, H)
                if not (lens is None and d == 0):
                    _, _, to_time = _lstm_step_maps(lens if lens is not None else _full_lens(B, U, x.device), B, U, d == 1)
                    ho = _new((B * U, H), like=x)
                    K.gather_rows(hs, to_time.t().contiguous().view(-1), ho)
                    out_d.copy_(ho.view(B, U, H))
        ctx.save_for_backward(x, out, gates, cs)
        ctx.x_parts, ctx.wih_parts, ctx.whh_parts = x_parts, wih_parts, whh_parts
        ctx.dirs, ctx.lens = dirs, lens
        return out

    @staticmethod
    def backward(ctx, dout):
        x, out, gates, cs = ctx.saved_tensors
        lens, dirs = ctx.lens, ctx.dirs
        n_dir = len(dirs)
        B, U, E = x.shape
        H = dirs[0][1].shape[1]
        G4 = 4 * H
        dout = dout.contiguous()
        dG = _new((n_dir, U, B, G4), like=out)
        if ctx.persistent:
            K.lstm_seq_bwd_ex(dout, gates, cs, ctx.whh_parts[0], dG, lens)
        else:
            dh_rec = torch.empty(B, H, dtype=torch.float32, device=x.device)
            dc = [torch.empty(B, H, dtype=torch.float32, device=x.device) for _ in range(2)]
            for d in range(n_dir):
                whh = [p[d * G4:(d + 1) * G4] for p in ctx.whh_parts]
                dout_d = dout[:, :, d * H:(d + 1) * H]
                if lens is None and d == 0:
                    do_s, dg_s = (lambda t: dout_d[:, t, :]), (lambda t: dG[d][t])
                else:
                    _, dsrc, to_time = _lstm_step_maps(lens if lens is not None else _full_lens(B, U, x.device), B, U, d == 1)
                    dz = torch.zeros(B * U + 1, H, dtype=dout.dtype, device=x.device)
                    dz[:B * U].view(B, U, H).copy_(dout_d)
                    dos = torch.empty(U * B, H, dtype=dout.dtype, device=x.device)
                    K.gather_rows(dz, dsrc.view(-1), dos)
                    dgs = _new((U * B + 1, G4), like=out, zero=True)
                    do_s, dg_s = (lambda t: dos[t * B:(t + 1) * B]), (lambda t: dgs[t * B:(t + 1) * B])
                for t in range(U - 1, -1, -1):
                    last = (t == U - 1)
                    K.lstm_cell_bwd(do_s(t), None if last else dh_rec, None if last else dc[(t + 1) & 1], gates[d][t], cs[d][t],
                                    cs[d][t - 1] if t > 0 else None, dg_s(t), dc[t & 1], B, H)
                    if t > 0:
                        gemm_parts([stage_act_view(dg_s(t))], [whh], dh_rec, b_mn=True, block_n=64)
                if not (lens is None and d == 0):
                    K.gather_rows(dgs, to_time.view(-1), dG[d].view(U * B, G4))
        dg_all = stage_act(dG)
        out_parts = stage_act(out)
        sel = dict(a_sel=(K.SEL_KZ, K.SEL_ZERO), b_sel=(K.SEL_KZ, K.SEL_ZERO))
        for d, (w_ih, w_hh, b_ih, b_hh) in enumerate(dirs):
            dg_parts = [p[d] for p in dg_all]
            h_parts = [p[:, :, d * H:(d + 1) * H].permute(1, 0, 2) for p in out_parts]
            if U > 1:
                a, b = ([p[1:] for p in dg_parts], [p[:-1] for p in h_parts]) if d == 0 else \
                       ([p[:-1] for p in dg_parts], [p[1:] for p in h_parts])
                gemm_parts([a], [b], grad_of(w_hh), a_mn=True, b_mn=True, kz_count=U - 1, **sel)
            else:
                grad_of(w_hh).zero_()
            gemm_parts([dg_parts], [[p.permute(1, 0, 2) for p in ctx.x_parts]], grad_of(w_ih), a_mn=True, b_mn=True, kz_count=U, **sel)
            K.colsum(dG[d].view(U * B, G4), grad_of(b_ih))
            grad_of(b_hh).copy_(b_ih.grad)
        dx = None
        if ctx.needs_input_grad[0]:
            dx = torch.empty_like(x)
            taps = [[p[d] for p in dg_all] for d in range(n_dir)]
            gemm_parts(taps, ctx.wih_parts, dx.permute(1, 0, 2), b_mn=True, a_sel=(K.SEL_ZB0, K.SEL_ZERO), b_sel=(K.SEL_ZERO, K.SEL_ZERO))
        return (dx, None) + (None,) * (4 * n_dir)


def _full_lens(B, U, device):
    return torch.full((B,), U, dtype=torch.int32, device=device)


def stage_act_view(v):
    if v.dtype == torch.bfloat16:
        return [v]
    hi = torch.empty(v.shape, dtype=torch.bfloat16, device=v.device)
    lo = torch.empty_like(hi)
    K.cast_split(v, hi, lo)
    return [hi, lo]


class DropoutFn(torch.autograd.Function):
    @staticmethod
    def forward(ctx, x, p, seed):
        y = torch.empty_like(x)
        K.dropout(x.contiguous(), y, p, seed)
        ctx.p, ctx.seed = p, seed
        return y

    @staticmethod
    def backward(ctx, dy):
        dx = torch.empty_like(dy)
        K.dropout(dy.contiguous(), dx, ctx.p, ctx.seed)
        return dx, None, None


def _ldv(V):
    return (V + 7) // 8 * 8


_FUSED_LSE = True


EVENT_TAPS = None


class _Tap:
    def __init__(self, name):
        self.name = name

    def __enter__(self):
        if EVENT_TAPS is not None:
            self.s = torch.cuda.Event(enable_timing=True)
            self.s.record()

    def __exit__(self, *exc):
        if EVENT_TAPS is not None:
            e = torch.cuda.Event(enable_timing=True)
            e.record()
            EVENT_TAPS.setdefault(self.name, []).append((self.s, e))


def _joint_forward(enc, pred, model, want_lse=False):
    B, T, H = enc.shape
    U1 = pred.shape[1]
    V = model.fc2.weight.shape[0]
    ldv = _ldv(V)
    fc1, fcg, fc2 = model.fc1, model.fc_gate, model.fc2
    wx = stage_weight([fc1.weight, fcg.weight])
    enc_parts = stage_act(enc.reshape(B * T, H))
    pred_parts = stage_act(pred.reshape(B * U1, H))
    ex = _new((B * T, 2 * H), like=enc)
    py = _new((B * U1, 2 * H), like=enc)
    gemm_parts([enc_parts], [[p[:, :H] for p in wx]], ex, bias=_cat_bias([fc1.bias, fcg.bias]))
    gemm_parts([pred_parts], [[p[:, H:] for p in wx]], py)
    R = B * T * U1
    h = _new((R, H), like=enc)
    K.joint_gate_fwd(ex, py, h, B, T, U1, H)
    w2 = stage_weight(fc2.weight)
    logits = _new((B, T, U1, ldv), like=enc, zero=(ldv != V))
    h_parts = stage_act(h)
    row_lse = None
    if want_lse and _FUSED_LSE and logits.dtype == torch.bfloat16 and V % 8 == 0:
        row_lse = torch.empty(K.row_lse_parts(R, V, 256), R, 2, dtype=torch.float32, device=enc.device)
    with _Tap("fc2_fwd"):
        gemm_parts([h_parts], [w2], logits.view(R, ldv)[:, :V], bias=fc2.bias.detach(), row_lse=row_lse,
                   **({"block_n": 256} if row_lse is not None else {}))
    state = dict(row_lse=row_lse, ex=ex, py=py, h_parts=h_parts, enc_parts=enc_parts, pred_parts=pred_parts, wx=wx, w2=w2, dims=(B, T, U1, H, V, ldv))
    return logits, state


def _joint_backward(dlogits, st, model, need_enc=True, need_pred=True, db2=None):
    B, T, U1, H, V, ldv = st["dims"]
    R = B * T * U1
    fc1, fcg, fc2 = model.fc1, model.fc_gate, model.fc2
    dl_parts = [p.view(R, ldv) for p in stage_act(dlogits)]
    dl_v = [p[:, :V] for p in dl_parts]
    dh = _new((R, H), like=dlogits)
    gemm_parts([dl_v], [st["w2"]], dh, b_mn=True)
    gemm_parts([dl_v], [st["h_parts"]], grad_of(fc2.weight), a_mn=True, b_mn=True)
    if db2 is None:
        db2 = torch.empty(ldv, dtype=torch.float32, device=dlogits.device)
        K.colsum(dlogits.view(R, ldv), db2)
    grad_of(fc2.bias).copy_(db2[:V])
    dex = _new((B * T, 2 * H), like=dlogits)
    dpy = _new((B * U1, 2 * H), like=dlogits)
    K.joint_gate_bwd(st["ex"], st["py"], dh, dex, dpy, B, T, U1, H)
    del dh
    dex_parts, dpy_parts = stage_act(dex), stage_act(dpy)
    g1, gg = grad_of(fc1.weight), grad_of(fcg.weight)
    for (dparts, xparts, lo) in ((dex_parts, st["enc_parts"], 0), (dpy_parts, st["pred_parts"], H)):
        gemm_parts([[p[:, :H] for p in dparts]], [xparts], g1[:, lo:lo + H], a_mn=True, b_mn=True)
        gemm_parts([[p[:, H:] for p in dparts]], [xparts], gg[:, lo:lo + H], a_mn=True, b_mn=True)
    dbx = torch.empty(2 * H, dtype=torch.float32, device=dlogits.device)
    K.colsum(dex, dbx)
    grad_of(fc1.bias).copy_(dbx[:H])
    grad_of(fcg.bias).copy_(dbx[H:])
    d_enc = d_pred = None
    if need_enc:
        d_enc = _new((B * T, H), like=dlogits)
        gemm_parts([dex_parts], [[p[:, :H] for p in st["wx"]]], d_enc, b_mn=True)
        d_enc = d_enc.view(B, T, H)
    if need_pred:
        d_pred = _new((B * U1, H), like=dlogits)
        gemm_parts([dpy_parts], [[p[:, H:] for p in st["wx"]]], d_pred, b_mn=True)
        d_pred = d_pred.view(B, U1, H)
    return d_enc, d_pred


class JointFn(torch.autograd.Function):

    @staticmethod
    def forward(ctx, enc, pred, model):
        logits, st = _joint_forward(enc, pred, model)
        ctx.st, ctx.model = st, model
        return logits

    @staticmethod
    def backward(ctx, dlogits):
        d_enc, d_pred = _joint_backward(dlogits.contiguous(), ctx.st, ctx.model, ctx.needs_input_grad[0], ctx.needs_input_grad[1])
        return d_enc, d_pred, None


_UNIT_LOSS_GRAD = False


def assume_unit_loss_grad(flag):
    global _UNIT_LOSS_GRAD
    _UNIT_LOSS_GRAD = bool(flag)


class JointLossFn(torch.autograd.Function):

    @staticmethod
    def forward(ctx, enc, pred, model, labels, frame_lens, label_lens, need_grad=True):
        logits, st = _joint_forward(enc, pred, model, want_lse=True)
        V = st["dims"][4]
        ctx.need_grad = need_grad
        if not need_grad:
            costs, _ = K.rnnt_loss_fwd_bwd(logits, labels, frame_lens, label_lens, V=V, want_grad=False, row_lse=st.pop("row_lse"))
            return costs
        db2 = torch.empty(logits.shape[-1], dtype=torch.float32, device=logits.device)
        with _Tap("rnnt_loss"):
            costs, _ = K.rnnt_loss_fwd_bwd(logits, labels, frame_lens, label_lens, V=V, dlogits=logits, colsum=db2,
                                           row_lse=st.pop("row_lse"))
        d_enc, d_pred = _joint_backward(logits, st, model, db2=db2)
        del logits, st
        ctx.save_for_backward(d_enc, d_pred)
        ctx.model = model
        return costs

    @staticmethod
    def backward(ctx, dcosts):
        if not ctx.need_grad:
            raise RuntimeError("JointLossFn: forward ran with grad mode off; there is nothing to back-propagate")
        d_enc, d_pred = ctx.saved_tensors
        if not _UNIT_LOSS_GRAD:
            w = dcosts.detach().float()
            if not bool((w == w[0]).all()):
                raise RuntimeError("JointLossFn: per-utterance loss weights are not supported by the fused joint backward "
                                   "(its parameter gradients were formed for a uniform upstream gradient)")
            if float(w[0]) != 1.0:
                m = ctx.model
                for p in (m.fc1.weight, m.fc1.bias, m.fc_gate.weight, m.fc_gate.bias, m.fc2.weight, m.fc2.bias):
                    p.grad.mul_(w[0])
                d_enc = d_enc * w[0].to(d_enc.dtype)
                d_pred = d_pred * w[0].to(d_pred.dtype)
        return d_enc, d_pred, None, None, None, None, None


class RNNTLossFn(torch.autograd.Function):

    @staticmethod
    def forward(ctx, log_probs, labels, frame_lens, label_lens):
        lp = log_probs.contiguous()
        B, T, U1, V = lp.shape
        ldv = V if (V % (8 if lp.dtype == torch.bfloat16 else 4) == 0) else None
        if ldv is None:
            ldv = _ldv(V)
            buf = torch.zeros(B, T, U1, ldv, dtype=lp.dtype, device=lp.device)
            buf[..., :V].copy_(lp)
            lp = buf
        costs, grads = K.rnnt_loss_fwd_bwd(lp, labels.int().contiguous(), frame_lens.int().contiguous(),
                                           label_lens.int().contiguous(), V=V)
        ctx.save_for_backward(grads[..., :V])
        return costs

    @staticmethod
    def backward(ctx, dcosts):
        (g,) = ctx.saved_tensors
        return g * dcosts.view(-1, 1, 1, 1).to(g.dtype), None, None, None


def _to_act(x):
    x = x.contiguous()
    if x.dtype == act_dtype():
        return x
    if act_dtype() == torch.bfloat16:
        x2 = x.reshape(-1, x.shape[-1]).float()
        out = torch.empty(x2.shape, dtype=torch.bfloat16, device=x.device)
        K.cast_split(x2, out)
        return out.view(x.shape)
    return x.float()


def transformer_layer(layer, x2, B, T, training, causal=False, key_pad=None):
    att, ff = layer.self_attn, layer.feed_forward
    p = _drop(layer.dropout_p, training)
    ln = LayerNormFn.apply(x2, layer.layer_norm, layer.layer_norm.weight, layer.layer_norm.bias)
    qkv = linear(ln, [att.linear_query.weight, att.linear_keys.weight, att.linear_values.weight],
                 [att.linear_query.bias, att.linear_keys.bias, att.linear_values.bias])
    rel = att.relative_positions_embeddings.weight if getattr(att, "max_relative_positions", 0) > 0 else None
    ctxv = AttentionFn.apply(qkv.view(B, T, -1), att.head_count, p, _next_seed() if p > 0 else 0, causal, key_pad, rel)
    h1 = linear(ctxv.view(B * T, -1), att.final_linear.weight, att.final_linear.bias, drop_p=p, residual=x2)
    ln2 = LayerNormFn.apply(h1, ff.layer_norm, ff.layer_norm.weight, ff.layer_norm.bias)
    fold = ln2.dtype == torch.bfloat16
    inter = linear(ln2, ff.w_1.weight, ff.w_1.bias, act=True, drop_p=p, premasked=fold)
    return linear(inter, ff.w_2.weight, ff.w_2.bias, drop_p=p, residual=h1,
                  mask_input_scale=(1.0 / (1.0 - p) if p > 0 else 1.0) if fold else 0.0)


def encoder_forward_act(enc, x, x_len=None, t_out=None):
    if isinstance(enc, torch.nn.LSTM):
        return lstm_encoder_forward_act(enc, x, x_len, t_out)
    training = enc.training
    B, T, D = x.shape
    C = enc.tdnn_nhid
    if T < 43:
        raise ValueError("encoder input has %d frames; the TDNN stack needs at least 43 (receptive field 21+1+21)" % T)
    h = linear(_to_act(x).view(B * T, D), enc.fc_in.weight, enc.fc_in.bias, act=True, premasked=True)
    h = BatchNormFn.apply(h, enc.bn_in, training, enc.bn_in.weight, enc.bn_in.bias, True)
    for l, (conv, bn) in enumerate(zip(enc.hidden_conv, enc.hidden_bn)):
        dil, stride = enc.TDNN_DIL_STRIDE[l]
        h3 = TdnnFn.apply(h.view(B, T, C), conv.weight, conv.bias, dil, stride, True)
        T = h3.shape[1]
        h = BatchNormFn.apply(h3.view(B * T, C), bn, training, bn.weight, bn.bias, True)
        if (l + 1) % 3 == 0:
            h = transformer_layer(enc.transformer[l // 3], h, B, T, training)
    h = BatchNormFn.apply(h, enc.bn_final, training, enc.bn_final.weight, enc.bn_final.bias)
    h = linear(h, enc.fc_out.weight, enc.fc_out.bias)
    return h.view(B, T, -1)


def encoder_forward(enc, x):
    return encoder_forward_act(enc, x).float()


def _lstm_layer_params(lstm, l):
    names = ["weight_ih_l%d", "weight_hh_l%d", "bias_ih_l%d", "bias_hh_l%d"]
    sfx = ["", "_reverse"] if lstm.bidirectional else [""]
    return [getattr(lstm, n % l + x) for x in sfx for n in names]


def lstm_encoder_forward_act(lstm, x, x_len=None, t_out=None):
    if lstm.batch_first is not True or not lstm.bias or lstm.proj_size:
        raise NotImplementedError("pika_b200: the LSTM encoder expects nn.LSTM(batch_first=True, bias=True, proj_size=0)")
    B, T, D = x.shape
    lens = None
    if x_len is None:
        t_out = T
    else:
        x_len = torch.as_tensor(x_len)
        if x_len.shape != (B,):
            raise ValueError("x_len must hold one length per sequence (%d), got shape %s" % (B, tuple(x_len.shape)))
        if t_out is None or not x_len.is_cuda:
            lo, hi = (int(v) for v in torch.stack((x_len.min(), x_len.max())).tolist())
            if lo < 1 or hi > T:
                raise ValueError("x_len must lie in [1, %d] (the frames of x); got [%d, %d]" % (T, lo, hi))
            t_out = hi if t_out is None else t_out
        if not 1 <= t_out <= T:
            raise ValueError("t_out = %d must lie in [1, %d]" % (t_out, T))
        lens = x_len.to(device=x.device, dtype=torch.int32).contiguous()
    ld = (D + 7) // 8 * 8
    h = _to_act(x[:, :t_out])
    if ld != D:
        hp = _new((B, t_out, ld), like=h, zero=True)
        hp[:, :, :D] = h
        h = hp
    p = _drop(lstm.dropout, lstm.training)
    for l in range(lstm.num_layers):
        h = LstmLayerFn.apply(h, lens, *_lstm_layer_params(lstm, l))
        if p > 0 and l < lstm.num_layers - 1:
            h = DropoutFn.apply(h, p, _next_seed())
    return h


def prednet_forward_act(model, y):
    B, U = y.shape
    sos = torch.zeros(B, 1, dtype=torch.long, device=y.device)
    yy = torch.cat((sos, y.long()), dim=1).contiguous()
    if getattr(model, "decoder_type", "rnn") != "rnn":
        return conv_transformer_lm_forward_act(model.decoder, yy)
    E = model.embed.weight.shape[1]
    ld = (E + 7) // 8 * 8
    h = EmbeddingFn.apply(yy, model.embed, ld, model.embed.weight).view(B, U + 1, ld)
    lstm = model.decoder
    p = _drop(lstm.dropout, lstm.training)
    for l in range(lstm.num_layers):
        h = LstmLayerFn.apply(h, None, *_lstm_layer_params(lstm, l))
# ... 61 lines not shown
```

### pika_b200/kernels.py

```python
import torch

from . import _lib
from ._lib import (ACT_NONE, ACT_RELU, AUX_ADD, AUX_MASK_NZ, AUX_NONE, PK_BF16, PK_F32, SEL_KZ, SEL_ZB0, SEL_ZB1,
                   SEL_ZERO, GemmDesc, View4, check, lib)


def _stream():
    return torch.cuda.current_stream().cuda_stream


def _dt(t):
    if t.dtype == torch.bfloat16:
        return PK_BF16
    if t.dtype == torch.float32:
        return PK_F32
    raise TypeError("unsupported dtype %s" % t.dtype)


def _P(t):
    return t.data_ptr() if t is not None else None


def _fill_view(v, t):
    assert t.is_cuda and t.dim() >= 1 and t.dim() <= 4, "views must be CUDA tensors with 1..4 dims"
    assert t.stride(-1) == 1 or t.shape[-1] == 1, "innermost dimension must be contiguous"
    shape = list(t.shape)[::-1]
    strides = list(t.stride())[::-1]
    v.ptr = t.data_ptr()
    for i in range(4):
        v.dim[i] = shape[i] if i < len(shape) else 1
    for i in range(3):
        v.stride[i] = strides[i + 1] if i + 1 < len(strides) else 0
    return v


def gemm(a, b, c, a_mn=False, b_mn=False, a_sel=(SEL_ZB0, SEL_ZB1), b_sel=(SEL_ZB0, SEL_ZB1), kz_count=1,
         a_row_off=None, b_row_off=None, alpha=1.0, bias=None, act=ACT_NONE, drop_p=0.0, drop_seed=0,
         aux=None, aux_mode=AUX_NONE, aux_scale=1.0, accumulate=False, block_n=0, k_splits=0, row_lse=None):
    a = a if isinstance(a, (list, tuple)) else [a]
    b = b if isinstance(b, (list, tuple)) else [b]
    assert len(a) == len(b) and 1 <= len(a) <= _lib.MAX_PAIRS
    d = GemmDesc()
    d.n_pairs = len(a)
    for i, (ai, bi) in enumerate(zip(a, b)):
        assert ai.dtype == torch.bfloat16 and bi.dtype == torch.bfloat16, "GEMM operands must be bf16"
        _fill_view(d.a[i], ai)
        _fill_view(d.b[i], bi)
        d.a_row_off[i] = a_row_off[i] if a_row_off else 0
        d.b_row_off[i] = b_row_off[i] if b_row_off else 0
    d.a_mn_major, d.b_mn_major = int(a_mn), int(b_mn)
    d.a_sel2, d.a_sel3 = a_sel
    d.b_sel2, d.b_sel3 = b_sel
    d.kz_count = kz_count
    _fill_view(d.c, c)
    d.c_dtype = _dt(c)
    d.c_accumulate = int(accumulate)
    d.alpha = alpha
    if bias is not None:
        assert bias.dtype == torch.float32 and bias.is_contiguous()
        d.bias = bias.data_ptr()
    d.act = act
    d.drop_p = drop_p
    d.drop_seed = drop_seed & 0xFFFFFFFF
    if aux is not None:
        assert aux.dim() == c.dim() and aux.stride(-1) == 1
        d.aux_mode = aux_mode
        d.aux = aux.data_ptr()
        d.aux_dtype = _dt(aux)
        st = list(aux.stride())[::-1]
        for i in range(3):
            d.aux_stride[i] = st[i + 1] if i + 1 < len(st) else 0
        d.aux_scale = aux_scale
    d.block_n = block_n
    d.k_splits = k_splits
    if row_lse is not None:
        assert row_lse.dtype == torch.float32 and row_lse.is_contiguous() and c.dim() == 2
        assert tuple(row_lse.shape) == (row_lse_parts(c.shape[-2], c.shape[-1], block_n), c.shape[-2], 2)
        d.row_lse = row_lse.data_ptr()
    check(lib.pk_gemm_bf16(d, _stream()), "pk_gemm_bf16")
    return c


def row_lse_parts(M, N, block_n=0):
    return int(lib.pk_gemm_row_lse_parts(M, N, block_n))


def rnnt_loss_fwd_bwd(logits, labels, frame_lens, label_lens, V=None, grad_scale=None, dlogits=None, want_grad=True, colsum=None,
                      row_lse=None):
    B, T, U1, ldv = logits.shape
    V = ldv if V is None else V
    assert logits.is_contiguous() and labels.dtype == torch.int32 and labels.dim() == 2
    assert frame_lens.dtype == torch.int32 and label_lens.dtype == torch.int32
    ws_bytes = int(lib.pk_rnnt_loss_workspace_bytes(B, T, U1))
    if colsum is not None:
        ws_bytes += int(lib.pk_rnnt_loss_colsum_workspace_bytes(B, T, U1, ldv))
    ws = torch.empty(ws_bytes, dtype=torch.uint8, device=logits.device)
    costs = torch.empty(B, dtype=torch.float32, device=logits.device)
    if want_grad and dlogits is None:
        dlogits = torch.empty_like(logits)
    if row_lse is not None:
        assert row_lse.dtype == torch.float32 and row_lse.is_contiguous() and tuple(row_lse.shape[1:]) == (B * T * U1, 2)
        check(lib.pk_rnnt_loss_fwd_bwd_lse(_P(logits), _dt(logits), _P(labels), _P(frame_lens), _P(label_lens),
                                           B, T, U1, V, ldv, max(labels.stride(0), 1), _P(grad_scale), _P(costs),
                                           _P(dlogits if want_grad else None), _P(colsum), _P(ws), ws_bytes,
                                           _P(row_lse), int(row_lse.shape[0]), _stream()), "pk_rnnt_loss_fwd_bwd_lse")
        return costs, dlogits
    check(lib.pk_rnnt_loss_fwd_bwd(_P(logits), _dt(logits), _P(labels), _P(frame_lens), _P(label_lens),
                                   B, T, U1, V, ldv, max(labels.stride(0), 1), _P(grad_scale), _P(costs),
                                   _P(dlogits if want_grad else None), _P(colsum), _P(ws), ws_bytes, _stream()),
          "pk_rnnt_loss_fwd_bwd")
    return costs, dlogits




def cast_split(src, hi, lo=None, cols_pad=None, scale=1.0):
    rows, cols = src.shape
    cols_pad = cols_pad or cols
    assert hi.shape[-1] == cols_pad and hi.stride(-1) == 1 and src.stride(-1) == 1
    check(lib.pk_cast_split(_P(src), _dt(src), src.stride(0), _P(hi), _P(lo), hi.stride(0), rows, cols, cols_pad, scale, _stream()),
          "pk_cast_split")


def attention_lse_stride(T):
    return int(lib.pk_attention_lse_stride(T))


def attention_keep_bits(B, T, heads, drop_p, device):
    if drop_p <= 0:
        return None
    return torch.empty(int(lib.pk_attention_keep_bits_bytes(B, T, heads)) // 4, dtype=torch.int32, device=device)


def attention_fwd(qkv, out, lse, heads, alpha, drop_p=0.0, seed=0, keep_bits=None):
    B, T, D3 = qkv.shape
    D = D3 // 3
    assert qkv.dtype == torch.bfloat16 and qkv.is_contiguous() and out.is_contiguous() and out.shape == (B, T, D)
    assert lse.dtype == torch.float32 and lse.numel() == B * heads * attention_lse_stride(T)
    base, es = qkv.data_ptr(), 2
    args = (base, base + D * es, base + 2 * D * es, D3, _P(out), D, _P(lse), B, T, heads, D // heads, alpha, drop_p, seed & 0xFFFFFFFF)
    if keep_bits is None:
        check(lib.pk_attention_fwd(*args, _stream()), "pk_attention_fwd")
        return
    assert keep_bits.is_contiguous() and keep_bits.numel() * keep_bits.element_size() >= lib.pk_attention_keep_bits_bytes(B, T, heads)
    check(lib.pk_attention_fwd_bits(*args, _P(keep_bits), _stream()), "pk_attention_fwd_bits")


def attention_bwd(qkv, out, dout, lse, dqkv, heads, alpha, drop_p=0.0, seed=0, keep_bits=None):
    B, T, D3 = qkv.shape
    D = D3 // 3
    assert dout.is_contiguous() and dqkv.is_contiguous() and dqkv.shape == qkv.shape and dout.dtype == torch.bfloat16
    ws = torch.zeros(B * heads * attention_lse_stride(T), dtype=torch.float32, device=qkv.device)
    base, gb, es = qkv.data_ptr(), dqkv.data_ptr(), 2
    args = (base, base + D * es, base + 2 * D * es, D3, _P(out), D, _P(dout), D, _P(lse), _P(ws),
            gb, gb + D * es, gb + 2 * D * es, D3, B, T, heads, D // heads, alpha, drop_p)
    if keep_bits is None:
        check(lib.pk_attention_bwd(*args, seed & 0xFFFFFFFF, _stream()), "pk_attention_bwd")
    else:
        check(lib.pk_attention_bwd_bits(*args, _P(keep_bits), _stream()), "pk_attention_bwd_bits")


_col_ws = {}


def col_ws(C, device):
    key = (C, str(device))
    if key not in _col_ws:
        _col_ws[key] = torch.empty(int(lib.pk_colstats_ws_floats(C)) + 2 * C, dtype=torch.float32, device=device)
    return _col_ws[key]


def bn_fwd(x, y, w, b, eps, train, momentum, run_mean, run_var, mean, rstd, ws=None):
    rows, C = x.shape
    ws = col_ws(C, x.device)
    check(lib.pk_bn_fwd(_P(x), _P(y), _dt(x), rows, C, _P(w), _P(b), eps, int(train), momentum,
                        _P(run_mean), _P(run_var), _P(mean), _P(rstd), _P(ws), _stream()), "pk_bn_fwd")


def bn_bwd(dy, x, dx, w, mean, rstd, train, relu_mask, dw, db):
    rows, C = x.shape
    check(lib.pk_bn_bwd(_P(dy), _P(x), _P(dx), _dt(x), rows, C, _P(w), _P(mean), _P(rstd), int(train),
                        int(relu_mask), _P(dw), _P(db), _P(col_ws(C, x.device)), _stream()), "pk_bn_bwd")


def colsum(x, out):
    rows, C = x.shape
    assert x.is_contiguous()
    check(lib.pk_colsum(_P(x), _dt(x), rows, C, _P(out), _P(col_ws(C, x.device)), _stream()), "pk_colsum")


def layernorm_fwd(x, y, w, b, eps, mean, rstd):
    rows, C = x.shape
    check(lib.pk_layernorm_fwd(_P(x), _P(y), _dt(x), rows, C, _P(w), _P(b), eps, _P(mean), _P(rstd), _stream()), "pk_layernorm_fwd")


def layernorm_bwd(dy, x, dx, w, mean, rstd, dw, db):
    rows, C = x.shape
    check(lib.pk_layernorm_bwd(_P(dy), _P(x), _P(dx), _dt(x), rows, C, _P(w), _P(mean), _P(rstd), _P(dw), _P(db), _stream()),
          "pk_layernorm_bwd")


def softmax_fwd(S, P, Pd, n, drop_p, seed):
    rows = S.numel() // S.shape[-1]
    check(lib.pk_softmax_fwd(_P(S), S.shape[-1], _P(P), _P(Pd), _dt(P), P.shape[-1], rows, n, drop_p, seed & 0xFFFFFFFF, _stream()),
          "pk_softmax_fwd")


def softmax_masked_fwd(S, P, Pd, n, q_len, heads, causal, key_pad, drop_p, seed):
    rows = S.numel() // S.shape[-1]
    if key_pad is not None:
        assert key_pad.dtype == torch.uint8 and key_pad.is_contiguous() and key_pad.shape[-1] == n
    check(lib.pk_softmax_masked_fwd(_P(S), S.shape[-1], _P(P), _P(Pd), _dt(P), P.shape[-1], rows, n, q_len, heads, int(bool(causal)),
                                    _P(key_pad), drop_p, seed & 0xFFFFFFFF, _stream()), "pk_softmax_masked_fwd")


def softmax_bwd(dPd, P, dS, n, drop_p, seed):
    rows = P.numel() // P.shape[-1]
    check(lib.pk_softmax_bwd(_P(dPd), dPd.shape[-1], _P(P), P.shape[-1], _P(dS), _dt(P), rows, n, drop_p, seed & 0xFFFFFFFF, _stream()),
          "pk_softmax_bwd")


def softmax_masked_relpos_fwd(S, QR, P, Pd, Pb, n, heads, causal, key_pad, max_rel, drop_p, seed):
    rows = S.numel() // S.shape[-1]
    if key_pad is not None:
        assert key_pad.dtype == torch.uint8 and key_pad.is_contiguous() and key_pad.shape[-1] == n
    assert QR.dtype == torch.float32 and Pb.dtype == torch.float32 and QR.stride(-1) == 1 and Pb.stride() == QR.stride()
    check(lib.pk_softmax_masked_relpos_fwd(_P(S), S.shape[-1], _P(QR), QR.stride(0), _P(P), _P(Pd), _dt(P), P.shape[-1],
                                           rows, n, n, heads, int(bool(causal)), _P(key_pad), max_rel, _P(Pb),
                                           drop_p, seed & 0xFFFFFFFF, _stream()), "pk_softmax_masked_relpos_fwd")


def softmax_relpos_bwd(dPd, G, P, dS, dSb, n, heads, max_rel, drop_p, seed):
    rows = P.numel() // P.shape[-1]
    assert G.dtype == torch.float32 and dSb.dtype == torch.float32 and G.stride(-1) == 1 and dSb.stride() == G.stride()
    check(lib.pk_softmax_relpos_bwd(_P(dPd), dPd.shape[-1], _P(G), G.stride(0), _P(P), P.shape[-1], _P(dS), _dt(P),
                                    rows, n, n, heads, max_rel, _P(dSb), drop_p, seed & 0xFFFFFFFF, _stream()),
          "pk_softmax_relpos_bwd")


def dropout(x, y, p, seed):
    check(lib.pk_dropout(_P(x), _P(y), _dt(x), x.numel(), p, seed & 0xFFFFFFFF, _stream()), "pk_dropout")


def mask_nz(dy, y, dx, scale):
    check(lib.pk_mask_nz(_P(dy), _P(y), _P(dx), _dt(y), y.numel(), scale, _stream()), "pk_mask_nz")


def add(a, b, o):
    check(lib.pk_add(_P(a), _P(b), _P(o), _dt(a), a.numel(), _stream()), "pk_add")


def log_softmax(x, y, n, scale=1.0):
    rows = x.numel() // x.shape[-1]
    check(lib.pk_log_softmax(_P(x), _dt(x), x.shape[-1], _P(y), rows, n, scale, _stream()), "pk_log_softmax")


def joint_gate_fwd(ex, py, h, B, T, U1, H):
    check(lib.pk_joint_gate_fwd(_P(ex), _P(py), _P(h), _dt(ex), B, T, U1, H, h.stride(0), _stream()), "pk_joint_gate_fwd")


def joint_gate_bwd(ex, py, dh, dex, dpy, B, T, U1, H):
    check(lib.pk_joint_gate_bwd(_P(ex), _P(py), _P(dh), _P(dex), _P(dpy), _dt(ex), B, T, U1, H, _stream()), "pk_joint_gate_bwd")


def lstm_cell_fwd(gx, gh, c_prev, c_out, h_out, gates_save, B, H):
    check(lib.pk_lstm_cell_fwd(_P(gx), gx.stride(0), _P(gh), gh.stride(0) if gh is not None else 0, _P(c_prev), _P(c_out), _P(h_out),
                               _dt(h_out), h_out.stride(0), _P(gates_save), B, H, _stream()), "pk_lstm_cell_fwd")


def lstm_cell_bwd(dh_out, dh_rec, dc_next, gates, c, c_prev, dgates, dc_prev, B, H):
    check(lib.pk_lstm_cell_bwd(_P(dh_out), dh_out.stride(0) if dh_out is not None else 0, _P(dh_rec), _P(dc_next), _P(gates), _P(c),
                               _P(c_prev), _P(dgates), _dt(dgates), _P(dc_prev), B, H, _stream()), "pk_lstm_cell_bwd")


def embedding_fwd(idx, table, out):
    n, ld = out.shape
    check(lib.pk_embedding_fwd(_P(idx), _P(table), table.shape[1], _P(out), _dt(out), ld, n, _stream()), "pk_embedding_fwd")


def embedding_bwd(idx, dout, dtable, padding_idx):
    n, ld = dout.shape
    check(lib.pk_embedding_bwd(_P(idx), _P(dout), _dt(dout), ld, dtable.shape[1], _P(dtable), n,
                               padding_idx if padding_idx is not None else -1, _stream()), "pk_embedding_bwd")


def absmax(x, out, nan_flag=None):
    check(lib.pk_absmax(_P(x), x.numel(), _P(out), _P(nan_flag), _stream()), "pk_absmax")


def sgd_nesterov_clip(p, g, buf, lr, momentum, max_norm, absmax_t, first, nan_flag=None):
    check(lib.pk_sgd_nesterov_clip(_P(p), _P(g), _P(buf), p.numel(), lr, momentum, max_norm, _P(absmax_t), _P(nan_flag), int(first),
                                   _stream()), "pk_sgd_nesterov_clip")


def bmuf_delta(glob, local, delta):
    check(lib.pk_bmuf_delta(_P(glob), _P(local), _P(delta), glob.numel(), _stream()), "pk_bmuf_delta")


def bmuf_update(glob, local, delta_prev, delta_sum, world, bm, blr):
    check(lib.pk_bmuf_update(_P(glob), _P(local), _P(delta_prev), _P(delta_sum), glob.numel(), world, bm, blr, _stream()),
          "pk_bmuf_update")


def adam_clip(p, g, exp_avg, exp_avg_sq, lr, betas, eps, step, max_norm=-1.0, absmax_t=None, nan_flag=None, p_out2=None):
    for t in (g, exp_avg, exp_avg_sq) + ((p_out2,) if p_out2 is not None else ()):
        assert t.numel() == p.numel() and t.dtype == torch.float32 and t.is_contiguous()
    beta1, beta2 = betas
    bc1 = 1 - beta1 ** step
    bc2_sqrt = (1 - beta2 ** step) ** 0.5
    on = max_norm > 0
    check(lib.pk_adam_clip(_P(p), _P(g), _P(exp_avg), _P(exp_avg_sq), _P(p_out2), p.numel(), lr, beta1, beta2, eps, bc1, bc2_sqrt,
                           max_norm, _P(absmax_t if on else None), _P(nan_flag if on else None), _stream()), "pk_adam_clip")


def bmuf_adam_update(glob, local, delta_prev, exp_avg_g, exp_avg_sq_g, msg, world, bm, blr, beta1_tau, beta1_rho, beta2_tau,
                     beta2_rho):
    n = glob.numel()
    assert msg.numel() == 3 * n and all(t.numel() == n for t in (local, delta_prev, exp_avg_g, exp_avg_sq_g))
    check(lib.pk_bmuf_adam_update(_P(glob), _P(local), _P(delta_prev), _P(exp_avg_g), _P(exp_avg_sq_g), _P(msg), n, world, bm, blr,
                                  beta1_tau, beta1_rho, beta2_tau, beta2_rho, _stream()), "pk_bmuf_adam_update")


_lstm_ws = {}


def _lstm_scratch(H, device):
    key = (H, str(device))
    if key not in _lstm_ws:
        _lstm_ws[key] = torch.zeros(int(lib.pk_lstm_seq_workspace_bytes(H)), dtype=torch.uint8, device=device)
    return _lstm_ws[key]


def _lens_arg(lens, B):
    assert lens is None or (lens.dtype == torch.int32 and lens.is_contiguous() and lens.numel() == B)
    return _P(lens)


def lstm_seq_fwd_ex(gx, w_hh, out, gates_save, cs, lens=None, reverse=False):
    n_dir, B, U, G4 = gx.shape
    H = G4 // 4
    assert gx.is_contiguous() and w_hh.dtype == torch.bfloat16 and w_hh.is_contiguous() and w_hh.shape[0] == n_dir * G4
    assert out.stride(2) == 1 and out.stride(0) == U * out.stride(1) and out.shape[-1] == n_dir * H
    check(lib.pk_lstm_seq_fwd_ex(_P(gx), _P(w_hh), _P(out), _dt(out), out.stride(1), _P(gates_save), _P(cs), _lens_arg(lens, B),
                                 B, U, H, n_dir, int(reverse), _P(_lstm_scratch(n_dir * H, gx.device)), _stream()),
          "pk_lstm_seq_fwd_ex")


def lstm_seq_bwd_ex(dout, gates_save, cs, w_hh, dG, lens=None, reverse=False):
    n_dir, U, B, G4 = dG.shape
    H = G4 // 4
    assert dout.stride(2) == 1 and dout.stride(0) == U * dout.stride(1) and dout.shape[-1] == n_dir * H
    assert dG.dtype == torch.bfloat16 and dG.is_contiguous() and w_hh.shape[0] == n_dir * G4
    check(lib.pk_lstm_seq_bwd_ex(_P(dout), _dt(dout), dout.stride(1), _P(gates_save), _P(cs), _P(w_hh), _P(dG), _lens_arg(lens, B),
                                 B, U, H, n_dir, int(reverse), _P(_lstm_scratch(n_dir * H, dout.device)), _stream()),
          "pk_lstm_seq_bwd_ex")


def gather_rows(src, idx, dst):
    rows, C = dst.shape
    check(lib.pk_gather_rows(_P(src), _P(idx), _P(dst), _dt(src), rows, C, _stream()), "pk_gather_rows")


def scatter_add_rows(src, idx, dst):
    rows, C = src.shape
    assert dst.dtype == torch.float32
    check(lib.pk_scatter_add_rows(_P(src), _P(idx), _P(dst), _dt(src), rows, C, _stream()), "pk_scatter_add_rows")


def beam_xf_taps(st, layer, embed, x_cur, taps):
    assert embed.dtype == torch.float32 and embed.is_contiguous() and taps.is_contiguous()
    check(lib.pk_beam_xf_taps(st, layer, _P(embed), embed.shape[1], _P(x_cur), _P(taps), taps.shape[1] // 5,
                              _stream()), "pk_beam_xf_taps")


def beam_xf_attn(st, layer, qkv, heads, rel, out):
    assert qkv.is_contiguous() and out.is_contiguous() and (rel is None or (rel.dtype == torch.float32 and rel.is_contiguous()))
    check(lib.pk_beam_xf_attn(st, layer, _P(qkv), heads, _P(rel), 0 if rel is None else rel.shape[0] // 2, _P(out),
                              _stream()), "pk_beam_xf_attn")


def beam_xf_select(st, x, h):
    check(lib.pk_beam_xf_select(st, _P(x), _P(h), h.shape[-1], _stream()), "pk_beam_xf_select")


def beam_xf_slots(st, prev_ks, K):
    check(lib.pk_beam_xf_slots(st, _P(prev_ks), K, _stream()), "pk_beam_xf_slots")


def ce_grad(z, tok, coef, scale, dz, n):
    rows, ld = z.shape
    check(lib.pk_ce_grad(_P(z), _dt(z), ld, _P(tok), _P(coef), scale, _P(dz), rows, n, _stream()), "pk_ce_grad")


def conv_same_f64(x, n_len, h, m_len, y=None):
    assert x.dtype == torch.float64 and h.dtype == torch.float64 and x.stride(1) == 1 and h.stride(1) == 1
    B, n = x.shape
    m = h.shape[1]
    if y is None:
        y = torch.zeros_like(x)
    need = int(lib.pk_conv_same_f64_workspace_bytes(B, n, m))
    if need < 0:
        raise ValueError("pk_conv_same_f64: RIR width %d outside [1, 65536]" % m)
    ws = torch.empty(need, dtype=torch.uint8, device=x.device)
    check(lib.pk_conv_same_f64(_P(x), x.stride(0), _P(n_len), _P(h), h.stride(0), _P(m_len), B, n, m, _P(y), y.stride(0), _P(ws), need,
                               _stream()), "pk_conv_same_f64")
    return y
```

Measured before the change: 273.5.

## Compact RNN-T gradient rows and skip negligible rows in joint backward GEMMs

The RNN-T loss backward now keeps only the (b,t,u) lattice rows whose blank and label gradient mass exceeds a tiny threshold. It writes a compacted dlogits and the matching hidden rows, plus a row map and a device-side row count. The joint backward GEMMs read that count to limit M tiles or K iterations, and the gate backward gathers dh through the row map. The aim is to avoid GEMM work and memory traffic on the many lattice cells with negligible occupancy. In exchange it adds scan/compaction kernels and extra copies, and it drops gradient contributions below the threshold, which is a mild approximation.

```diff
diff --git a/include/pika_b200.h b/include/pika_b200.h
--- a/include/pika_b200.h
+++ b/include/pika_b200.h
@@ -55,6 +55,7 @@
     int block_n;
     int k_splits;
     float* row_lse;
+    const int* a_rows_dev;
 } pk_gemm_desc;
 
 int pk_gemm_bf16(const pk_gemm_desc* desc, void* stream);
@@ -70,6 +71,11 @@
                              const int* label_lens, int B, int T, int U1, int V, int ldv, int ld_labels,
                              const float* grad_scale, float* costs, void* dlogits, float* dlogits_colsum, void* workspace,
                              long long workspace_bytes, const float* row_lse, int n_parts, void* stream);
+int pk_rnnt_loss_fwd_bwd_compact(const void* logits, int dtype, const int* labels, const int* frame_lens,
+                                 const int* label_lens, int B, int T, int U1, int V, int ldv, int ld_labels,
+                                 const float* grad_scale, float* costs, void* dz_c, float* dlogits_colsum, void* workspace,
+                                 long long workspace_bytes, const float* row_lse, int n_parts, const void* h, int H,
+                                 void* h_c, int* row_map, int* row_count, void* stream);
 
 int pk_cast_split(const void* src, int src_dtype, long long ld_src, void* hi, void* lo, long long ld_dst,
                   long long rows, int cols, int cols_pad, float scale, void* stream);
@@ -116,8 +122,8 @@
 int pk_add(const void* a, const void* b, void* o, int dtype, long long n, void* stream);
 int pk_log_softmax(const void* x, int dtype, long long ld, float* y, long long rows, int n, float scale, void* stream);
 int pk_joint_gate_fwd(const void* ex, const void* py, void* h, int dtype, int B, int T, int U1, int H, int ld_h, void* stream);
-int pk_joint_gate_bwd(const void* ex, const void* py, const void* dh, void* dex, void* dpy, int dtype, int B, int T, int U1,
-                      int H, void* stream);
+int pk_joint_gate_bwd(const void* ex, const void* py, const void* dh, const int* dh_map, void* dex, void* dpy, int dtype, int B, int T,
+                      int U1, int H, void* stream);
 int pk_lstm_cell_fwd(const float* gx, long long ld_gx, const float* gh, long long ld_gh, const float* c_prev, float* c_out,
                      void* h_out, int dtype, long long ld_h, float* gates_save, int B, int H, void* stream);
 int pk_lstm_cell_bwd(const void* dh_out, long long ld_dho, const float* dh_rec, const float* dc_next, const float* gates,
diff --git a/pika_b200/_lib.py b/pika_b200/_lib.py
--- a/pika_b200/_lib.py
+++ b/pika_b200/_lib.py
@@ -66,6 +66,7 @@
         ("block_n", ctypes.c_int),
         ("k_splits", ctypes.c_int),
         ("row_lse", ctypes.c_void_p),
+        ("a_rows_dev", ctypes.c_void_p),
     ]
 
 
diff --git a/pika_b200/csrc/elementwise.cu b/pika_b200/csrc/elementwise.cu
--- a/pika_b200/csrc/elementwise.cu
+++ b/pika_b200/csrc/elementwise.cu
@@ -823,10 +823,19 @@
         }
     }
 }
+template <typename T> PK_DEVICE typename V8<T>::Raw load_dh_mapped(const T* dh, int m, int H, int c0) {
+    if (m >= 0) return V8<T>::load_raw(dh + (long long)m * H + c0);
+    return typename V8<T>::Raw{};
+}
+template <typename T> PK_DEVICE typename V8<T>::Raw load_dh_row(const T* dh, const int* map, long long r, int H, int c0) {
+    if (map == nullptr) return V8<T>::load_raw(dh + r * H + c0);
+    return load_dh_mapped<T>(dh, __ldg(map + r), H, c0);
+}
+
 template <typename T>
 __global__ void __launch_bounds__(128) joint_gate_bwd_ex_kernel(const T* __restrict__ ex, const T* __restrict__ py,
-                                                                const T* __restrict__ dh, T* __restrict__ dex, int B, int Tt,
-                                                                int U1, int H) {
+                                                                const T* __restrict__ dh, const int* __restrict__ dh_map,
+                                                                T* __restrict__ dex, int B, int Tt, int U1, int H) {
     const int bt = blockIdx.x;
     const int b = bt / Tt;
     for (int c0 = threadIdx.x * 8; c0 < H; c0 += blockDim.x * 8) {
@@ -838,7 +847,7 @@
             const T* pr = py + ((long long)b * U1 + u) * 2 * H;
             V8<T>::load(pr + c0, p1);
             V8<T>::load(pr + H + c0, pg);
-            V8<T>::load(dh + ((long long)bt * U1 + u) * H + c0, d);
+            V8<T>::unpack(load_dh_row<T>(dh, dh_map, (long long)bt * U1 + u, H, c0), d);
 #pragma unroll
             for (int e = 0; e < 8; ++e) {
                 const float a = jt_tanh<T>(e1[e] + p1[e]), g = jt_sigmoid<T>(eg[e] + pg[e]);
@@ -852,8 +861,8 @@
 }
 template <typename T>
 __global__ void __launch_bounds__(128) joint_gate_bwd_py_kernel(const T* __restrict__ ex, const T* __restrict__ py,
-                                                                const T* __restrict__ dh, T* __restrict__ dpy, int B, int Tt,
-                                                                int U1, int H) {
+                                                                const T* __restrict__ dh, const int* __restrict__ dh_map,
+                                                                T* __restrict__ dpy, int B, int Tt, int U1, int H) {
     const int bu = blockIdx.x;
     const int b = bu / U1, u = bu - b * U1;
     for (int c0 = threadIdx.x * 8; c0 < H; c0 += blockDim.x * 8) {
@@ -865,7 +874,7 @@
             const long long bt = (long long)b * Tt + t;
             V8<T>::load(ex + bt * 2 * H + c0, e1);
             V8<T>::load(ex + bt * 2 * H + H + c0, eg);
-            V8<T>::load(dh + (bt * U1 + u) * H + c0, d);
+            V8<T>::unpack(load_dh_row<T>(dh, dh_map, bt * U1 + u, H, c0), d);
 #pragma unroll
             for (int e = 0; e < 8; ++e) {
                 const float a = jt_tanh<T>(e1[e] + p1[e]), g = jt_sigmoid<T>(eg[e] + pg[e]);
@@ -880,7 +889,8 @@
 
 template <typename T, int UI>
 __global__ void __launch_bounds__(128) joint_gate_bwd_fused_kernel(const T* __restrict__ ex, const T* __restrict__ py, const T* __restrict__ dh,
-                                                                   T* __restrict__ dex, T* __restrict__ dpy, int B, int Tt, int U1, int H) {
+                                                                   const int* __restrict__ dh_map, T* __restrict__ dex, T* __restrict__ dpy,
+                                                                   int B, int Tt, int U1, int H) {
     extern __shared__ __align__(16) uint8_t jg_smem[];
     T* s_py = reinterpret_cast<T*>(jg_smem);
     const int slices = H / 32;
@@ -901,13 +911,15 @@
     __syncthreads();
     const T* s_p1 = s_py + (long long)(ct * U1) * 8;
     const T* s_pg = s_py + (long long)((4 + ct) * U1) * 8;
-    const T* dh_b = dh + (long long)b * Tt * U1 * H + c0;
+    const long long row_b = (long long)b * Tt * U1;
     const T* ex_b = ex + (long long)b * Tt * 2 * H + c0;
     typename V8<T>::Raw dn[UI], e1n, egn;
+    int mn[UI];
 #pragma unroll
     for (int i = 0; i < UI; ++i) {
         const int u = lane + 32 * i;
-        if (u < U1) dn[i] = V8<T>::load_raw(dh_b + (long long)u * H);
+        if (u < U1) dn[i] = load_dh_row<T>(dh, dh_map, row_b + u, H, c0);
+        mn[i] = (dh_map != nullptr && u < U1 && Tt > 1) ? __ldg(dh_map + row_b + U1 + u) : -1;
     }
     e1n = V8<T>::load_raw(ex_b);
     egn = V8<T>::load_raw(ex_b + H);
@@ -922,7 +934,14 @@
 #pragma unroll
             for (int i = 0; i < UI; ++i) {
                 const int u = lane + 32 * i;
-                if (u < U1) dn[i] = V8<T>::load_raw(dh_b + ((long long)(t + 1) * U1 + u) * H);
+                if (u < U1) {
+                    if (dh_map == nullptr) {
+                        dn[i] = V8<T>::load_raw(dh + (row_b + (long long)(t + 1) * U1 + u) * H + c0);
+                    } else {
+                        dn[i] = load_dh_mapped<T>(dh, mn[i], H, c0);
+                        if (t + 2 < Tt) mn[i] = __ldg(dh_map + row_b + (long long)(t + 2) * U1 + u);
+                    }
+                }
             }
             e1n = V8<T>::load_raw(ex_b + (long long)(t + 1) * 2 * H);
             egn = V8<T>::load_raw(ex_b + (long long)(t + 1) * 2 * H + H);
@@ -1315,24 +1334,26 @@
 }
 
 template <typename T, int UI>
-static void launch_gate_bwd_fused(const void* ex, const void* py, const void* dh, void* dex, void* dpy, int B, int T_, int U1, int H, cudaStream_t st) {
+static void launch_gate_bwd_fused(const void* ex, const void* py, const void* dh, const int* dh_map, void* dex, void* dpy, int B, int T_, int U1, int H,
+                                  cudaStream_t st) {
     const int smem = U1 * 64 * (int)sizeof(T);
-    joint_gate_bwd_fused_kernel<T, UI><<<B * (H / 32), 128, smem, st>>>((const T*)ex, (const T*)py, (const T*)dh, (T*)dex, (T*)dpy, B, T_, U1, H);
-}
-extern "C" int pk_joint_gate_bwd(const void* ex, const void* py, const void* dh, void* dex, void* dpy, int dtype, int B, int T_, int U1,
-                                 int H, void* stream) {
+    joint_gate_bwd_fused_kernel<T, UI><<<B * (H / 32), 128, smem, st>>>((const T*)ex, (const T*)py, (const T*)dh, dh_map, (T*)dex, (T*)dpy, B, T_, U1,
+                                                                     H);
+}
+extern "C" int pk_joint_gate_bwd(const void* ex, const void* py, const void* dh, const int* dh_map, void* dex, void* dpy, int dtype, int B,
+                                 int T_, int U1, int H, void* stream) {
     PK_CHECK_ARG(H % 8 == 0, "H must be a multiple of 8");
     const int ui = (U1 + 31) / 32;
     if (H % 32 == 0 && ui <= 5) {
         cudaStream_t st = STREAM(stream);
-#define PK_GATE_CASE(N) case N: { PK_DISPATCH_T(dtype, (launch_gate_bwd_fused<T, N>(ex, py, dh, dex, dpy, B, T_, U1, H, st))); } break;
+#define PK_GATE_CASE(N) case N: { PK_DISPATCH_T(dtype, (launch_gate_bwd_fused<T, N>(ex, py, dh, dh_map, dex, dpy, B, T_, U1, H, st))); } break;
         switch (ui) { PK_GATE_CASE(1) PK_GATE_CASE(2) PK_GATE_CASE(3) PK_GATE_CASE(4) PK_GATE_CASE(5) }
 #undef PK_GATE_CASE
         DONE();
     }
-    PK_DISPATCH_T(dtype, (joint_gate_bwd_ex_kernel<T><<<B * T_, 128, 0, STREAM(stream)>>>((const T*)ex, (const T*)py, (const T*)dh, (T*)dex, B, T_, U1, H)));
+    PK_DISPATCH_T(dtype, (joint_gate_bwd_ex_kernel<T><<<B * T_, 128, 0, STREAM(stream)>>>((const T*)ex, (const T*)py, (const T*)dh, dh_map, (T*)dex, B, T_, U1, H)));
     PK_CHECK_LAUNCH(); count_launch();
-    PK_DISPATCH_T(dtype, (joint_gate_bwd_py_kernel<T><<<B * U1, 128, 0, STREAM(stream)>>>((const T*)ex, (const T*)py, (const T*)dh, (T*)dpy, B, T_, U1, H)));
+    PK_DISPATCH_T(dtype, (joint_gate_bwd_py_kernel<T><<<B * U1, 128, 0, STREAM(stream)>>>((const T*)ex, (const T*)py, (const T*)dh, dh_map, (T*)dpy, B, T_, U1, H)));
     DONE();
 }
 
diff --git a/pika_b200/csrc/gemm.cu b/pika_b200/csrc/gemm.cu
--- a/pika_b200/csrc/gemm.cu
+++ b/pika_b200/csrc/gemm.cu
@@ -36,6 +36,7 @@
     float aux_scale;
     float* row_lse;
     uint64_t pol_a, pol_b, pol_c;
+    const int* a_rows_dev;
 };
 
 template <int BN, bool EPI_WARPS> struct GemmCfg {
@@ -115,8 +116,18 @@
     __syncthreads();
 
     const int out_tiles = p.tiles_m * p.tiles_n * p.zb0 * p.zb1;
-    const int num_units = out_tiles * p.k_splits;
-    const int k_iters_total = p.n_pairs * p.kz_count * p.num_k_blocks;
+    int num_units = out_tiles * p.k_splits;
+    int k_iters_total = p.n_pairs * p.kz_count * p.num_k_blocks;
+    int ips = p.iters_per_split;
+    if (p.a_rows_dev != nullptr) {
+        const int rows = *p.a_rows_dev;
+        if (A_MN) {
+            k_iters_total = min(k_iters_total, (rows + BK - 1) / BK);
+            ips = max(1, (k_iters_total + p.k_splits - 1) / p.k_splits);
+        } else {
+            num_units = min(num_units, (rows + BM - 1) / BM * p.tiles_n);
+        }
+    }
 
     if (warp < 4) {
         setmaxnreg_dec<40>();
@@ -129,7 +140,7 @@
         for (int unit = worker; unit < num_units; unit += n_workers) {
             const UnitCoord u = decode_unit(p, unit);
             const int m0 = u.mb * BM, n0 = u.nb * BN;
-            const int i0 = u.split * p.iters_per_split, i1 = min(k_iters_total, i0 + p.iters_per_split);
+            const int i0 = u.split * ips, i1 = min(k_iters_total, i0 + ips);
             int pr = i0 / kzb;
             int rem = i0 - pr * kzb;
             int kz = rem / p.num_k_blocks, kb = rem - kz * p.num_k_blocks;
@@ -253,7 +264,11 @@
     };
     for (int unit = worker; unit < num_units; unit += n_workers) {
         const UnitCoord u = decode_unit(p, unit);
-        const int k_iters = min(k_iters_total, (u.split + 1) * p.iters_per_split) - u.split * p.iters_per_split;
+        const int k_iters = max(0, min(k_iters_total, (u.split + 1) * ips) - u.split * ips);
+        if (k_iters == 0) {
+#pragma unroll
+            for (int i = 0; i < BN / 2; ++i) acc[i] = 0.f;
+        }
         int prev = -1;
         for (int k = 0; k < k_iters; ++k) {
             mbar_wait(&full_bar[stage], phase);
@@ -595,6 +610,10 @@
     gp.aux_sm = d->aux_stride[0]; gp.aux_s0 = d->aux_stride[1]; gp.aux_s1 = d->aux_stride[2];
     gp.aux_scale = d->aux_scale;
     gp.row_lse = d->row_lse;
+    gp.a_rows_dev = d->a_rows_dev;
+    PK_CHECK_ARG(d->a_rows_dev == nullptr || (d->n_pairs == 1 && d->kz_count == 1 && gp.zb0 == 1 && gp.zb1 == 1 &&
+                                              (d->a_mn_major || d->k_splits <= 1)),
+                 "a_rows_dev needs one pair, kz_count 1, a 2-D C and, for a K-major A, no split-K");
     PK_CHECK_ARG(d->row_lse == nullptr || (d->c_dtype == PK_BF16 && N % 8 == 0 && gp.zb0 == 1 && gp.zb1 == 1 && bn == 256 &&
                                            gp.drop_thresh == 0u && gp.aux_mode == PK_AUX_NONE),
                  "row_lse needs a 2-D bf16 C with N % 8 == 0, block_n = 256, no dropout / aux");
@@ -614,7 +633,8 @@
     int splits = 1;
     const bool plain_epi = d->bias == nullptr && d->act == PK_ACT_NONE && d->drop_p == 0.f && gp.aux_mode == PK_AUX_NONE;
     if (d->k_splits > 0) splits = d->k_splits;
-    else if (gp.c_is_f32 && plain_epi && gp.zb0 == 1 && gp.zb1 == 1 && k_iters_total >= 16 && out_tiles < 6 * workers_max) {
+    else if (gp.c_is_f32 && plain_epi && gp.zb0 == 1 && gp.zb1 == 1 && k_iters_total >= 16 && out_tiles < 6 * workers_max &&
+             (d->a_rows_dev == nullptr || d->a_mn_major)) {
         const int w = workers_max;
         double best = 0.0;
         for (int sp = 1; sp <= 16 && sp <= k_iters_total / 8; ++sp) {
diff --git a/pika_b200/csrc/rnnt_loss.cu b/pika_b200/csrc/rnnt_loss.cu
--- a/pika_b200/csrc/rnnt_loss.cu
+++ b/pika_b200/csrc/rnnt_loss.cu
@@ -305,14 +305,109 @@
     }
 }
 
+PK_DEVICE bool grad_row_kept(float gb, float gl) {
+    return (__float_as_uint(gb) & 0x7fffffffu) + (__float_as_uint(gl) & 0x7fffffffu) >= 0x2000u;
+}
+
+constexpr int SCAN_THREADS = 1024;
+constexpr int SCAN_PER_THREAD = 4;
+constexpr int SCAN_TILE = SCAN_THREADS * SCAN_PER_THREAD;
+
+PK_DEVICE int block_exclusive_scan(int v, int* s_warp, int* total) {
+    const int lane = threadIdx.x & 31, w = threadIdx.x >> 5;
+    int x = v;
+#pragma unroll
+    for (int o = 1; o < 32; o <<= 1) {
+        const int y = __shfl_up_sync(0xffffffffu, x, o);
+        if (lane >= o) x += y;
+    }
+    if (lane == 31) s_warp[w] = x;
+    __syncthreads();
+    if (w == 0) {
+        int s = s_warp[lane];
+#pragma unroll
+        for (int o = 1; o < 32; o <<= 1) {
+            const int y = __shfl_up_sync(0xffffffffu, s, o);
+            if (lane >= o) s += y;
+        }
+        s_warp[lane] = s;
+    }
+    __syncthreads();
+    const int r = x - v + (w > 0 ? s_warp[w - 1] : 0);
+    *total = s_warp[31];
+    __syncthreads();
+    return r;
+}
+
+PK_DEVICE int tile_kept(const float* gb, const float* gl, long long rows, long long r0, bool (&keep)[SCAN_PER_THREAD]) {
+    int n = 0;
+#pragma unroll
+    for (int k = 0; k < SCAN_PER_THREAD; ++k) {
+        const long long r = r0 + (long long)threadIdx.x * SCAN_PER_THREAD + k;
+        keep[k] = r < rows && grad_row_kept(gb[r], gl[r]);
+        n += keep[k];
+    }
+    return n;
+}
+
+__global__ void __launch_bounds__(SCAN_THREADS) grad_rows_count_kernel(const float* __restrict__ gb, const float* __restrict__ gl,
+                                                                       long long rows, int* __restrict__ tile_count) {
+    __shared__ int s_warp[32];
+    bool keep[SCAN_PER_THREAD];
+    int total;
+    block_exclusive_scan(tile_kept(gb, gl, rows, (long long)blockIdx.x * SCAN_TILE, keep), s_warp, &total);
+    if (threadIdx.x == 0) tile_count[blockIdx.x] = total;
+}
+
+template <typename T>
+__global__ void __launch_bounds__(SCAN_THREADS) grad_rows_scan_kernel(int* __restrict__ tile_count, int n_tiles, int* __restrict__ count,
+                                                                      long long rows, T* dz_c, int ldv, T* h_c, int H) {
+    __shared__ int s_warp[32];
+    __shared__ int s_carry;
+    if (threadIdx.x == 0) s_carry = 0;
+    __syncthreads();
+    for (int i0 = 0; i0 < n_tiles; i0 += SCAN_THREADS) {
+        const int i = i0 + threadIdx.x;
+        const int v = i < n_tiles ? tile_count[i] : 0;
+        int total;
+        const int ex = block_exclusive_scan(v, s_warp, &total);
+        if (i < n_tiles) tile_count[i] = s_carry + ex;
+        __syncthreads();
+        if (threadIdx.x == 0) s_carry += total;
+        __syncthreads();
+    }
+    const long long kept = s_carry;
+    if (threadIdx.x == 0) *count = (int)kept;
+    const long long tail = min(rows, (kept + 63) / 64 * 64);
+    for (long long r = kept; r < tail; ++r) {
+        for (int c = threadIdx.x; c < ldv; c += SCAN_THREADS) dz_c[r * ldv + c] = from_f32<T>(0.f);
+        for (int c = threadIdx.x; c < H; c += SCAN_THREADS) h_c[r * H + c] = from_f32<T>(0.f);
+    }
+}
+
+__global__ void __launch_bounds__(SCAN_THREADS) grad_rows_map_kernel(const float* __restrict__ gb, const float* __restrict__ gl,
+                                                                     long long rows, const int* __restrict__ tile_off, int* __restrict__ map) {
+    __shared__ int s_warp[32];
+    bool keep[SCAN_PER_THREAD];
+    const long long r0 = (long long)blockIdx.x * SCAN_TILE;
+    int total;
+    int idx = tile_off[blockIdx.x] + block_exclusive_scan(tile_kept(gb, gl, rows, r0, keep), s_warp, &total);
+#pragma unroll
+    for (int k = 0; k < SCAN_PER_THREAD; ++k) {
+        const long long r = r0 + (long long)threadIdx.x * SCAN_PER_THREAD + k;
+        if (r < rows) map[r] = keep[k] ? idx++ : -1;
+    }
+}
+
 constexpr int GRAD_THREADS = 256;
 template <typename T> struct GradCfg { static constexpr int MAXG = 32 / Vec16<T>::N; };
-template <typename T, int GRAD_RU, int MINB>
+template <typename T, int GRAD_RU, int MINB, bool COMPACT>
 __global__ void __launch_bounds__(GRAD_THREADS, MINB) rnnt_grad_kernel(const T* logits, const int* __restrict__ labels,
                                                                     const int* __restrict__ label_lens, RnntDims d,
                                                                     const float* __restrict__ lse_in, const float* __restrict__ gb_in,
                                                                     const float* __restrict__ gl_in, T* dlogits, float* __restrict__ colsum,
-                                                                    long long rows_per_cta) {
+                                                                    long long rows_per_cta, const int* __restrict__ row_map,
+                                                                    const T* __restrict__ h, T* __restrict__ h_c, int H) {
     constexpr int VN = Vec16<T>::N;
     constexpr int GRAD_MAXG = GradCfg<T>::MAXG;
     extern __shared__ float gsm[];
@@ -320,6 +415,7 @@
     float* s_gl = gsm + rows_per_cta;
     float* s_l2 = gsm + 2 * rows_per_cta;
     int* s_y = reinterpret_cast<int*>(gsm + 3 * rows_per_cta);
+    int* s_map = reinterpret_cast<int*>(gsm + 4 * rows_per_cta);
     const long long rows = (long long)d.B * d.T * d.U1;
     const long long r0 = (long long)blockIdx.x * rows_per_cta;
     const long long r1 = min(rows, r0 + rows_per_cta);
@@ -333,8 +429,10 @@
         const int u = (int)(row % d.U1);
         const int b = (int)(row / ((long long)d.T * d.U1));
         s_y[i] = (u < label_lens[b]) ? labels[(size_t)b * d.ld_labels + u] : -1;
+        if (COMPACT) s_map[i] = row_map[row];
     }
     __syncthreads();
+    const int h_vec = COMPACT ? H / 8 : 0;
     float cs[GRAD_MAXG][VN];
 #pragma unroll
     for (int gq = 0; gq < GRAD_MAXG; ++gq)
@@ -342,16 +440,18 @@
         for (int e = 0; e < VN; ++e) cs[gq][e] = 0.f;
     for (long long rb = r0; rb < r1; rb += GRAD_RU) {
         uint4 q[GRAD_RU][GRAD_MAXG];
+        uint4 hq[GRAD_RU];
 #pragma unroll
         for (int k = 0; k < GRAD_RU; ++k) {
             const long long row = rb + k;
-            if (row < r1 && (s_gb[row - r0] != 0.f || s_gl[row - r0] != 0.f)) {
+            if (row < r1 && (COMPACT ? s_map[row - r0] >= 0 : (s_gb[row - r0] != 0.f || s_gl[row - r0] != 0.f))) {
                 const uint4* vp = reinterpret_cast<const uint4*>(logits + row * (long long)d.ldv);
 #pragma unroll
                 for (int gq = 0; gq < GRAD_MAXG; ++gq) {
                     const int i = tid + gq * GRAD_THREADS;
                     if (i < nvec_ld) q[k][gq] = ld_plain(vp + i);
                 }
+                if (COMPACT && tid < h_vec) hq[k] = ld_stream(reinterpret_cast<const uint4*>(h + row * (long long)H) + tid);
             }
         }
 #pragma unroll
@@ -359,7 +459,13 @@
             const long long row = rb + k;
             if (row >= r1) continue;
             const float gb = s_gb[row - r0], gl = s_gl[row - r0];
-            uint4* op = reinterpret_cast<uint4*>(dlogits + row * (long long)d.ldv);
+            long long orow = row;
+            if (COMPACT) {
+                orow = s_map[row - r0];
+                if (orow < 0) continue;
+                if (tid < h_vec) st_stream(reinterpret_cast<uint4*>(h_c + orow * H) + tid, hq[k]);
+            }
+            uint4* op = reinterpret_cast<uint4*>(dlogits + orow * (long long)d.ldv);
             if (gb == 0.f && gl == 0.f) {
 #pragma unroll
                 for (int gq = 0; gq < GRAD_MAXG; ++gq) {
@@ -466,7 +572,8 @@
 static int rnnt_loss_impl(const void* logits, int dtype, const int* labels, const int* frame_lens,
                           const int* label_lens, int B, int T, int U1, int V, int ldv, int ld_labels,
                           const float* grad_scale, float* costs, void* dlogits, float* dlogits_colsum, void* workspace,
-                          long long workspace_bytes, const float* row_lse, int n_parts, void* stream_v) {
+                          long long workspace_bytes, const float* row_lse, int n_parts, int* row_map, int* row_count,
+                          const void* h, int H, void* h_c, void* stream_v) {
     using namespace pk;
     cudaStream_t stream = reinterpret_cast<cudaStream_t>(stream_v);
     PK_CHECK_ARG(dtype == PK_F32 || dtype == PK_BF16, "bad dtype");
@@ -530,12 +637,27 @@
                          "workspace too small for the column sums (add pk_rnnt_loss_colsum_workspace_bytes)");
             cs_part = reinterpret_cast<float*>(reinterpret_cast<unsigned char*>(workspace) + base_bytes);
         }
-        const size_t gsmem = (size_t)rpc * 16;
-#define PK_GRAD_LAUNCH(TT, RU, MB)                                                                                         \
-        rnnt_grad_kernel<TT, RU, MB><<<ggrid, GRAD_THREADS, gsmem, stream>>>(reinterpret_cast<const TT*>(logits), labels, label_lens, d, lse, \
-                                                                            gb, gl, reinterpret_cast<TT*>(dlogits), cs_part, rpc)
-        if (dtype == PK_BF16) PK_GRAD_LAUNCH(__nv_bfloat16, 2, 3);
-        else PK_GRAD_LAUNCH(float, 2, 2);
+        if (row_map != nullptr) {
+            const int n_tiles = (int)((rows + SCAN_TILE - 1) / SCAN_TILE);
+            int* tile_count = reinterpret_cast<int*>(alpha);
+            grad_rows_count_kernel<<<n_tiles, SCAN_THREADS, 0, stream>>>(gb, gl, rows, tile_count);
+            PK_CHECK_LAUNCH(); count_launch();
+            grad_rows_scan_kernel<__nv_bfloat16><<<1, SCAN_THREADS, 0, stream>>>(tile_count, n_tiles, row_count, rows,
+                                                                                 reinterpret_cast<__nv_bfloat16*>(dlogits), ldv,
+                                                                                 reinterpret_cast<__nv_bfloat16*>(h_c), H);
+            PK_CHECK_LAUNCH(); count_launch();
+            grad_rows_map_kernel<<<n_tiles, SCAN_THREADS, 0, stream>>>(gb, gl, rows, tile_count, row_map);
+            PK_CHECK_LAUNCH(); count_launch();
+        }
+        const size_t gsmem = (size_t)rpc * (row_map != nullptr ? 20 : 16);
+#define PK_GRAD_LAUNCH(TT, RU, MB, CP)                                                                                     \
+        rnnt_grad_kernel<TT, RU, MB, CP><<<ggrid, GRAD_THREADS, gsmem, stream>>>(reinterpret_cast<const TT*>(logits), labels, label_lens, d, \
+                                                                                lse, gb, gl, reinterpret_cast<TT*>(dlogits), cs_part, rpc,  \
+                                                                                row_map, reinterpret_cast<const TT*>(h),                    \
+                                                                                reinterpret_cast<TT*>(h_c), H)
+        if (row_map != nullptr) PK_GRAD_LAUNCH(__nv_bfloat16, 2, 3, true);
+        else if (dtype == PK_BF16) PK_GRAD_LAUNCH(__nv_bfloat16, 2, 3, false);
+        else PK_GRAD_LAUNCH(float, 2, 2, false);
 #undef PK_GRAD_LAUNCH
         PK_CHECK_LAUNCH(); count_launch();
         if (dlogits_colsum) {
@@ -551,7 +673,7 @@
                                     const float* grad_scale, float* costs, void* dlogits, float* dlogits_colsum, void* workspace,
                                     long long workspace_bytes, void* stream) {
     return rnnt_loss_impl(logits, dtype, labels, frame_lens, label_lens, B, T, U1, V, ldv, ld_labels, grad_scale, costs, dlogits,
-                          dlogits_colsum, workspace, workspace_bytes, nullptr, 0, stream);
+                          dlogits_colsum, workspace, workspace_bytes, nullptr, 0, nullptr, nullptr, nullptr, 0, nullptr, stream);
 }
 
 extern "C" int pk_rnnt_loss_fwd_bwd_lse(const void* logits, int dtype, const int* labels, const int* frame_lens,
@@ -560,5 +682,19 @@
                                         long long workspace_bytes, const float* row_lse, int n_parts, void* stream) {
     PK_CHECK_ARG(row_lse != nullptr, "row_lse is null");
     return rnnt_loss_impl(logits, dtype, labels, frame_lens, label_lens, B, T, U1, V, ldv, ld_labels, grad_scale, costs, dlogits,
-                          dlogits_colsum, workspace, workspace_bytes, row_lse, n_parts, stream);
-}
+                          dlogits_colsum, workspace, workspace_bytes, row_lse, n_parts, nullptr, nullptr, nullptr, 0, nullptr, stream);
+}
+
+extern "C" int pk_rnnt_loss_fwd_bwd_compact(const void* logits, int dtype, const int* labels, const int* frame_lens,
+                                            const int* label_lens, int B, int T, int U1, int V, int ldv, int ld_labels,
+                                            const float* grad_scale, float* costs, void* dz_c, float* dlogits_colsum, void* workspace,
+                                            long long workspace_bytes, const float* row_lse, int n_parts, const void* h, int H,
+                                            void* h_c, int* row_map, int* row_count, void* stream) {
+    PK_CHECK_ARG(dtype == PK_BF16, "the compacted gradient is bf16 only");
+    PK_CHECK_ARG(dz_c != nullptr && row_map != nullptr && row_count != nullptr && h != nullptr && h_c != nullptr, "null pointer");
+    PK_CHECK_ARG(H > 0 && H % 8 == 0 && H / 8 <= pk::GRAD_THREADS, "H must be a multiple of 8, <= 2048");
+    PK_CHECK_ARG(dz_c != logits, "dz_c must not alias the logits");
+    PK_CHECK_ARG((reinterpret_cast<uintptr_t>(h) & 15) == 0 && (reinterpret_cast<uintptr_t>(h_c) & 15) == 0, "h / h_c not 16B aligned");
+    return rnnt_loss_impl(logits, dtype, labels, frame_lens, label_lens, B, T, U1, V, ldv, ld_labels, grad_scale, costs, dz_c,
+                          dlogits_colsum, workspace, workspace_bytes, row_lse, n_parts, row_map, row_count, h, H, h_c, stream);
+}
diff --git a/pika_b200/engine.py b/pika_b200/engine.py
--- a/pika_b200/engine.py
+++ b/pika_b200/engine.py
@@ -665,6 +665,9 @@
 _FUSED_LSE = True
 
 
+_COMPACT_GRAD = True
+
+
 EVENT_TAPS = None
 
 
@@ -713,22 +716,26 @@
     return logits, state
 
 
-def _joint_backward(dlogits, st, model, need_enc=True, need_pred=True, db2=None):
+def _joint_backward(dlogits, st, model, need_enc=True, need_pred=True, db2=None, compact=None):
     B, T, U1, H, V, ldv = st["dims"]
     R = B * T * U1
     fc1, fcg, fc2 = model.fc1, model.fc_gate, model.fc2
     dl_parts = [p.view(R, ldv) for p in stage_act(dlogits)]
     dl_v = [p[:, :V] for p in dl_parts]
     dh = _new((R, H), like=dlogits)
-    gemm_parts([dl_v], [st["w2"]], dh, b_mn=True)
-    gemm_parts([dl_v], [st["h_parts"]], grad_of(fc2.weight), a_mn=True, b_mn=True)
+    h_parts, row_map, rows = st.get("h_parts"), None, None
+    if compact is not None:
+        h_c, row_map, rows = compact
+        h_parts = [h_c]
+    gemm_parts([dl_v], [st["w2"]], dh, b_mn=True, a_rows_dev=rows)
+    gemm_parts([dl_v], [h_parts], grad_of(fc2.weight), a_mn=True, b_mn=True, a_rows_dev=rows)
     if db2 is None:
         db2 = torch.empty(ldv, dtype=torch.float32, device=dlogits.device)
         K.colsum(dlogits.view(R, ldv), db2)
     grad_of(fc2.bias).copy_(db2[:V])
     dex = _new((B * T, 2 * H), like=dlogits)
     dpy = _new((B * U1, 2 * H), like=dlogits)
-    K.joint_gate_bwd(st["ex"], st["py"], dh, dex, dpy, B, T, U1, H)
+    K.joint_gate_bwd(st["ex"], st["py"], dh, dex, dpy, B, T, U1, H, dh_map=row_map)
     del dh
     dex_parts, dpy_parts = stage_act(dex), stage_act(dpy)
     g1, gg = grad_of(fc1.weight), grad_of(fcg.weight)
@@ -784,10 +791,20 @@
             costs, _ = K.rnnt_loss_fwd_bwd(logits, labels, frame_lens, label_lens, V=V, want_grad=False, row_lse=st.pop("row_lse"))
             return costs
         db2 = torch.empty(logits.shape[-1], dtype=torch.float32, device=logits.device)
-        with _Tap("rnnt_loss"):
-            costs, _ = K.rnnt_loss_fwd_bwd(logits, labels, frame_lens, label_lens, V=V, dlogits=logits, colsum=db2,
-                                           row_lse=st.pop("row_lse"))
-        d_enc, d_pred = _joint_backward(logits, st, model, db2=db2)
+        compact = None
+        if _COMPACT_GRAD and logits.dtype == torch.bfloat16 and len(st["w2"]) == 1 and len(st["h_parts"]) == 1:
+            with _Tap("rnnt_loss"):
+                costs, dz_c, h_c, row_map, rows = K.rnnt_loss_compact(logits, labels, frame_lens, label_lens, st["h_parts"][0], V=V,
+                                                                      colsum=db2, row_lse=st.pop("row_lse"))
+            logits, compact = dz_c, (h_c, row_map, rows)
+            del dz_c, h_c
+            st.pop("h_parts")
+        else:
+            with _Tap("rnnt_loss"):
+                costs, _ = K.rnnt_loss_fwd_bwd(logits, labels, frame_lens, label_lens, V=V, dlogits=logits, colsum=db2,
+                                               row_lse=st.pop("row_lse"))
+        d_enc, d_pred = _joint_backward(logits, st, model, db2=db2, compact=compact)
+        del compact
         del logits, st
         ctx.save_for_backward(d_enc, d_pred)
         ctx.model = model
diff --git a/pika_b200/kernels.py b/pika_b200/kernels.py
--- a/pika_b200/kernels.py
+++ b/pika_b200/kernels.py
@@ -36,7 +36,7 @@
 
 def gemm(a, b, c, a_mn=False, b_mn=False, a_sel=(SEL_ZB0, SEL_ZB1), b_sel=(SEL_ZB0, SEL_ZB1), kz_count=1,
          a_row_off=None, b_row_off=None, alpha=1.0, bias=None, act=ACT_NONE, drop_p=0.0, drop_seed=0,
-         aux=None, aux_mode=AUX_NONE, aux_scale=1.0, accumulate=False, block_n=0, k_splits=0, row_lse=None):
+         aux=None, aux_mode=AUX_NONE, aux_scale=1.0, accumulate=False, block_n=0, k_splits=0, row_lse=None, a_rows_dev=None):
     a = a if isinstance(a, (list, tuple)) else [a]
     b = b if isinstance(b, (list, tuple)) else [b]
     assert len(a) == len(b) and 1 <= len(a) <= _lib.MAX_PAIRS
@@ -77,6 +77,9 @@
         assert row_lse.dtype == torch.float32 and row_lse.is_contiguous() and c.dim() == 2
         assert tuple(row_lse.shape) == (row_lse_parts(c.shape[-2], c.shape[-1], block_n), c.shape[-2], 2)
         d.row_lse = row_lse.data_ptr()
+    if a_rows_dev is not None:
+        assert a_rows_dev.dtype == torch.int32 and a_rows_dev.is_cuda
+        d.a_rows_dev = a_rows_dev.data_ptr()
     check(lib.pk_gemm_bf16(d, _stream()), "pk_gemm_bf16")
     return c
 
@@ -112,6 +115,32 @@
     return costs, dlogits
 
 
+def rnnt_loss_compact(logits, labels, frame_lens, label_lens, h, V=None, colsum=None, row_lse=None):
+    B, T, U1, ldv = logits.shape
+    V = ldv if V is None else V
+    R, H = B * T * U1, h.shape[-1]
+    assert logits.is_contiguous() and logits.dtype == torch.bfloat16 and labels.dtype == torch.int32 and labels.dim() == 2
+    assert frame_lens.dtype == torch.int32 and label_lens.dtype == torch.int32
+    assert h.is_contiguous() and h.dtype == torch.bfloat16 and h.numel() == R * H
+    ws_bytes = int(lib.pk_rnnt_loss_workspace_bytes(B, T, U1))
+    if colsum is not None:
+        ws_bytes += int(lib.pk_rnnt_loss_colsum_workspace_bytes(B, T, U1, ldv))
+    dev = logits.device
+    ws = torch.empty(ws_bytes, dtype=torch.uint8, device=dev)
+    costs = torch.empty(B, dtype=torch.float32, device=dev)
+    dz_c = torch.empty(R, ldv, dtype=torch.bfloat16, device=dev)
+    h_c = torch.empty(R, H, dtype=torch.bfloat16, device=dev)
+    row_map = torch.empty(R, dtype=torch.int32, device=dev)
+    row_count = torch.empty(1, dtype=torch.int32, device=dev)
+    if row_lse is not None:
+        assert row_lse.dtype == torch.float32 and row_lse.is_contiguous() and tuple(row_lse.shape[1:]) == (R, 2)
+    check(lib.pk_rnnt_loss_fwd_bwd_compact(_P(logits), PK_BF16, _P(labels), _P(frame_lens), _P(label_lens), B, T, U1, V, ldv,
+                                           max(labels.stride(0), 1), None, _P(costs), _P(dz_c), _P(colsum), _P(ws), ws_bytes,
+                                           _P(row_lse), int(row_lse.shape[0]) if row_lse is not None else 0, _P(h), H, _P(h_c),
+                                           _P(row_map), _P(row_count), _stream()), "pk_rnnt_loss_fwd_bwd_compact")
+    return costs, dz_c, h_c, row_map, row_count
+
+
 
 
 def cast_split(src, hi, lo=None, cols_pad=None, scale=1.0):
@@ -259,8 +288,8 @@
     check(lib.pk_joint_gate_fwd(_P(ex), _P(py), _P(h), _dt(ex), B, T, U1, H, h.stride(0), _stream()), "pk_joint_gate_fwd")
 
 
-def joint_gate_bwd(ex, py, dh, dex, dpy, B, T, U1, H):
-    check(lib.pk_joint_gate_bwd(_P(ex), _P(py), _P(dh), _P(dex), _P(dpy), _dt(ex), B, T, U1, H, _stream()), "pk_joint_gate_bwd")
+def joint_gate_bwd(ex, py, dh, dex, dpy, B, T, U1, H, dh_map=None):
+    check(lib.pk_joint_gate_bwd(_P(ex), _P(py), _P(dh), _P(dh_map), _P(dex), _P(dpy), _dt(ex), B, T, U1, H, _stream()), "pk_joint_gate_bwd")
 
 
 def lstm_cell_fwd(gx, gh, c_prev, c_out, h_out, gates_save, B, H):
```

New measurement: 283.8 (median of 6 runs). 1.04x the previous value.
